# manlito/densepoints

Measured on AMD Instinct MI355X. Metric: Mpatches/sec (NCC eval+refine), higher is better.
Workload: dtype u8 texels, fp64 geometry, int32 moments; 1 GPU; cfg3_32view_4k: 32 views 3840x2160, 262144 expansion candidates/GPU/step (65536 refined seed parents x 4 directions), n=11, Nelder-Mead + InitRelatedImages + NCC filter (parity mode); views=32, width=3840, height=2160, cell=11, batch_per_gpu=262144, parallelism=dp1 (candidate shards, no data-path collective)

## Files before the change

### densepoints_amd/_native.py

```python
from __future__ import annotations

import ctypes
import os

import numpy as np

_HERE = os.path.dirname(os.path.abspath(__file__))
LIB_PATH = os.path.join(_HERE, "lib", os.environ.get("DP_LIB_VARIANT") or "libdensepoints.so")

PATCH_DTYPE = np.dtype(
    [
        ("pos", "<f4", 3),
        ("normal", "<f4", 3),
        ("ref", "<u4"),
        ("seq", "<u4"),
        ("vis", "<u8", 2),
        ("cand", "<u8", 2),
        ("score", "<f4"),
        ("evals", "<u4"),
        ("rgb", "u1", 3),
        ("flags", "u1"),
        ("parent", "<u4"),
    ],
    align=True,
)
assert PATCH_DTYPE.itemsize == 80

DP_OK = 0
DP_E_ARG = -1
DP_E_HIP = -2
DP_E_OOM = -3
DP_E_DEGENERATE = -4
DP_E_STATE = -5
DP_E_NODEVICE = -6

MODE_EVAL, MODE_FILTER, MODE_NM, MODE_SEED, MODE_EXPAND = range(5)
MODE_FAST_EVAL, MODE_FAST_REFINE = 5, 6
PATCH_ACCEPTED = 1
PATCH_DEGENERATE = 2


class DpOptions(ctypes.Structure):
    _fields_ = [
        ("seed_cell_size", ctypes.c_int32),
        ("expand_cell_size", ctypes.c_int32),
        ("grid_scale", ctypes.c_int32),
        ("max_patches_per_cell", ctypes.c_int32),
        ("min_visible", ctypes.c_int32),
        ("min_expand_visible", ctypes.c_int32),
        ("nm_max_evals", ctypes.c_int32),
        ("reserved0", ctypes.c_int32),
        ("ncc_threshold", ctypes.c_double),
        ("visible_angle", ctypes.c_double),
        ("candidate_angle", ctypes.c_double),
        ("nm_step", ctypes.c_double * 3),
        ("nm_eps", ctypes.c_double),
        ("ncc_denom_min", ctypes.c_double),
        ("max_pops", ctypes.c_int64),
    ]


class DpImage(ctypes.Structure):
    _fields_ = [
        ("width", ctypes.c_int32),
        ("height", ctypes.c_int32),
        ("stride", ctypes.c_int32),
        ("reserved", ctypes.c_int32),
        ("bgr", ctypes.c_void_p),
    ]


class DpDensifyStats(ctypes.Structure):
    _fields_ = [
        ("seeds_in", ctypes.c_int64),
        ("seed_patches", ctypes.c_int64),
        ("patches", ctypes.c_int64),
        ("pops", ctypes.c_int64),
        ("candidates", ctypes.c_int64),
        ("evals", ctypes.c_int64),
        ("generations", ctypes.c_int32),
        ("stalls", ctypes.c_int32),
        ("refine_ms", ctypes.c_double),
        ("total_ms", ctypes.c_double),
    ]


class DpGeneration(ctypes.Structure):
    _fields_ = [
        ("items", ctypes.c_int64),
        ("head", ctypes.c_int64),
        ("per_item", ctypes.c_int32),
        ("cell", ctypes.c_int32),
        ("seq0", ctypes.c_uint32),
        ("index", ctypes.c_int32),
    ]


class DpIterateStats(ctypes.Structure):
    _fields_ = [
        ("offered", ctypes.c_int64),
        ("reinserted", ctypes.c_int64),
        ("patches", ctypes.c_int64),
        ("filtered_out", ctypes.c_int64),
        ("candidates", ctypes.c_int64),
        ("evals", ctypes.c_int64),
        ("generations", ctypes.c_int32),
        ("reserved", ctypes.c_int32),
        ("refine_ms", ctypes.c_double),
        ("filter_ms", ctypes.c_double),
        ("total_ms", ctypes.c_double),
    ]


class DpFilterOptions(ctypes.Structure):
    _fields_ = [
        ("passes", ctypes.c_int32),
        ("reserved", ctypes.c_int32),
        ("min_neighbor_frac", ctypes.c_double),
    ]


FILTER_VISIBILITY, FILTER_NEIGHBORS = 1, 2


class DpRenderOptions(ctypes.Structure):
    _fields_ = [
        ("splat_scale", ctypes.c_float),
        ("max_radius_px", ctypes.c_int32),
        ("flags", ctypes.c_int32),
    ]


class DpRenderStats(ctypes.Structure):
    _fields_ = [
        ("patches", ctypes.c_int64),
        ("pairs", ctypes.c_int64),
        ("pixel_tests", ctypes.c_int64),
        ("covered_pixels", ctypes.c_int64),
        ("render_ms", ctypes.c_double),
    ]


RENDER_ALL_FACING = 1


class DpFuseOptions(ctypes.Structure):
    _fields_ = [
        ("depth_tol", ctypes.c_float),
        ("min_views", ctypes.c_int32),
        ("min_normal_cos", ctypes.c_float),
        ("flags", ctypes.c_int32),
    ]


class DpFuseStats(ctypes.Structure):
    _fields_ = [
        ("depth_pixels", ctypes.c_int64),
        ("matched_pairs", ctypes.c_int64),
        ("consistent_pairs", ctypes.c_int64),
        ("fusable", ctypes.c_int64),
        ("emitted", ctypes.c_int64),
        ("fuse_ms", ctypes.c_double),
    ]


FUSE_NO_SUPPRESS = 1

FUSED_DTYPE = np.dtype(
    [
        ("pos", "<f4", 3),
        ("normal", "<f4", 3),
        ("rgb", "u1", 3),
        ("n_views", "u1"),
        ("view", "<i4"),
        ("x", "<i4"),
        ("y", "<i4"),
    ],
    align=True,
)
assert FUSED_DTYPE.itemsize == 40


class DpMaprefOptions(ctypes.Structure):
    _fields_ = [
        ("window", ctypes.c_int32),
        ("sweep", ctypes.c_int32),
        ("step_px", ctypes.c_float),
        ("reach", ctypes.c_int32 * 2),
        ("max_sources", ctypes.c_int32),
# ... 158 lines not shown


class DpSynthConfig(ctypes.Structure):
    _fields_ = [
        ("n_views", ctypes.c_int32),
        ("width", ctypes.c_int32),
        ("height", ctypes.c_int32),
        ("kind", ctypes.c_int32),
        ("seed", ctypes.c_uint64),
        ("spread_deg", ctypes.c_double),
        ("seed_stride_px", ctypes.c_double),
        ("depth_noise", ctypes.c_double),
    ]


class DpMatcherOptions(ctypes.Structure):

    _fields_ = [
        ("n_features", ctypes.c_int32),
        ("n_levels", ctypes.c_int32),
        ("scale_factor", ctypes.c_double),
        ("edge_threshold", ctypes.c_int32),
        ("fast_threshold", ctypes.c_int32),
        ("cell_size", ctypes.c_int32),
        ("max_keypoints_per_cell", ctypes.c_int32),
        ("epipolar_matching", ctypes.c_int32),
        ("max_epipolar_distance", ctypes.c_float),
        ("nn_match_ratio", ctypes.c_float),
        ("matcher_type", ctypes.c_int32),
        ("detector_type", ctypes.c_int32),
        ("akaze_threshold", ctypes.c_float),
    ]


class DpSeedStats(ctypes.Structure):
    _fields_ = [
        ("keypoints_detected", ctypes.c_int64),
        ("keypoints", ctypes.c_int64),
        ("pairs", ctypes.c_int64),
        ("ratio_matches", ctypes.c_int64),
        ("matches", ctypes.c_int64),
        ("points", ctypes.c_int64),
        ("detect_ms", ctypes.c_double),
        ("describe_ms", ctypes.c_double),
        ("match_ms", ctypes.c_double),
        ("triangulate_ms", ctypes.c_double),
        ("total_ms", ctypes.c_double),
    ]


class DpFastOptions(ctypes.Structure):
    _fields_ = [
        ("iters", ctypes.c_int32),
        ("margin", ctypes.c_int32),
        ("tile_budget", ctypes.c_int32),
        ("max_views", ctypes.c_int32),
        ("fd_step", ctypes.c_float),
        ("ls_step", ctypes.c_float),
        ("densify", ctypes.c_int32),
        ("gradient", ctypes.c_int32),
        ("filter_max_views", ctypes.c_int32),
    ]


class DpFastStats(ctypes.Structure):
    _fields_ = [("patches", ctypes.c_int64), ("evals", ctypes.c_int64), ("view_evals", ctypes.c_int64),
                ("staged_bytes", ctypes.c_int64), ("clipped_stagings", ctypes.c_int64)]


KEYPOINT_DTYPE = np.dtype(
    [("x", "<f4"), ("y", "<f4"), ("response", "<f4"), ("angle", "<f4"), ("octave", "<i4"), ("reserved", "<i4")]
)

_P = ctypes.c_void_p
_I = ctypes.c_int
_D = ctypes.c_double

SIGNATURES = [
    ("dp_default_options", None, [_P]),
    ("dp_abi_version", _I, []),
    ("dp_device_count", _I, []),
    ("dp_ctx_create", _I, [_P, _I, _P]),
    ("dp_ctx_destroy", _I, [_P]),
    ("dp_last_error", ctypes.c_char_p, [_P]),
    ("dp_set_options", _I, [_P, _P]),
    ("dp_set_views", _I, [_P, _I, _P, _P]),
    ("dp_set_views_device", _I, [_P, _I, _P, _P, _P, _P, _P]),
    ("dp_build_pyramid", _I, [_P, _I]),
    ("dp_set_level", _I, [_P, _I]),
    ("dp_level_info", _I, [_P, _I, _I, _P, _P, _P]),
    ("dp_read_level", _I, [_P, _I, _I, _P]),
    ("dp_view_geometry", _I, [_P, _P, _P, _P, _P]),
    ("dp_seeds_to_patches", _I, [_P, _P, _I, _P]),
    ("dp_eval_batch", _I, [_P, _P, _I, _I, _P]),
    ("dp_refine_batch", _I, [_P, _P, _I, _I, _I, _P]),
    ("dp_refine_batch_device", _I, [_P, _P, _I, _I, _I, _P, _P]),
    ("dp_expand_batch", _I, [_P, _P, _I, _P, _P]),
    ("dp_expand_batch_device", _I, [_P, _P, _I, _P, _P, _P]),
    ("dp_densify", _I, [_P, _P, _I, _P, _P, _P]),
    ("dp_densify_begin", _I, [_P, _P, _I, _P]),
    ("dp_densify_commit", _I, [_P, _P, _P, _P, ctypes.c_int64]),
    ("dp_densify_result", _I, [_P, _P, _P, _P]),
    ("dp_densify_run", _I, [_P, _P, ctypes.c_int32]),
    ("dp_densify_run_until", _I, [_P, _P, ctypes.c_int32, ctypes.c_int64, _P]),
    ("dp_densify_owners", _I, [_P, _P, _I, _I, _P, _P]),
    ("dp_densify_partition_stats", _I, [_P, _P]),
    ("dp_densify_refine_items", _I, [_P, _P, _P, ctypes.c_int64, _P, _P]),
    ("dp_densify_partition_async", _I, [_P, _P, _I, _I, _P, _P, _P]),
    ("dp_densify_refine_share_async", _I, [_P, _P, _P, ctypes.c_int64, _P, ctypes.c_int64, _P]),
    ("dp_densify_commit_gathered_device", _I, [_P, _P, _P, ctypes.c_int64, _I, _P, _P]),
    ("dp_densify_resume", _I, [_P, _P, ctypes.c_int64, _P, _P]),
    ("dp_densify_resume_device", _I, [_P, _P, ctypes.c_int64, _P, _P, _P]),
    ("dp_densify_store_device", _I, [_P, _P, _P]),
    ("dp_densify_iterate", _I, [_P, _P, _I, _I, _P, _P, _P, _P, _P]),
    ("dp_default_filter_options", None, [_P]),
    ("dp_filter_patches", _I, [_P, _P, ctypes.c_int64, _P, _P]),
    ("dp_filter_patches_device", _I, [_P, _P, ctypes.c_int64, _P, _P, _P]),
    ("dp_default_render_options", None, [_P]),
    ("dp_render_maps", _I, [_P, _P, ctypes.c_int64, _P, _P, _I, _P, _P, _P, _P, _P, _P]),
    ("dp_render_maps_device", _I, [_P, _P, ctypes.c_int64, _P, _P, _I, _P, _P, _P, _P, _P, _P, _P]),
    ("dp_default_fuse_options", None, [_P]),
    ("dp_fuse_maps", _I, [_P, _P, _I, _P, _P, _P, _P, _P, _P]),
    ("dp_fuse_maps_device", _I, [_P, _P, _I, _P, _P, _P, _P, ctypes.c_int64, _P, _P, _P]),
    ("dp_default_mapref_options", None, [_P]),
    ("dp_refine_maps", _I, [_P, _P, _I, _P, _P, _P, _P, _P, _P, _P, _P, _P]),
    ("dp_refine_maps_device", _I, [_P, _P, _I, _P, _P, _P, _P, _P, _P, _P, _P, _P, _P]),
    ("dp_default_tsdf_options", None, [_P]),
    ("dp_tsdf_integrate", _I, [_P, _P, _I, _P, _P, _P, _P, _P, _P]),
    ("dp_tsdf_integrate_device", _I, [_P, _P, _I, _P, _P, _P, _P, _P, _P, _P]),
    ("dp_tsdf_mesh", _I, [_P, _P, _P, _P, _P, _P, _P, _P, _P, _P]),
    ("dp_tsdf_mesh_device", _I, [_P, _P, _P, _P, _P, _P, ctypes.c_int64, _P, _P, ctypes.c_int64, _P, _P, _P]),
    ("dp_default_mesh_clean_options", None, [_P]),
    ("dp_mesh_components", _I, [_P, _P, ctypes.c_int64, ctypes.c_int64, _P, _P, _P, _P, _P]),
    ("dp_mesh_components_device", _I, [_P, _P, ctypes.c_int64, ctypes.c_int64, _P, _P, _P, ctypes.c_int64, _P, _P, _P]),
    ("dp_mesh_clean", _I, [_P, _P, _P, ctypes.c_int64, _P, ctypes.c_int64, _P, _P, _P, _P, _P, _P, _P]),
    ("dp_mesh_clean_device", _I, [_P, _P, _P, ctypes.c_int64, _P, ctypes.c_int64, _P, ctypes.c_int64, _P, _P,
                                  ctypes.c_int64, _P, _P, _P, _P, _P]),
    ("dp_default_mesh_smooth_options", None, [_P]),
    ("dp_mesh_adjacency", _I, [_P, _P, ctypes.c_int64, ctypes.c_int64, _P, _P, _P, _P, _P, _P]),
    ("dp_mesh_adjacency_device", _I, [_P, _P, ctypes.c_int64, ctypes.c_int64, _P, _P, _P, ctypes.c_int64, _P, _P, _P,
                                      _P]),
    ("dp_mesh_smooth", _I, [_P, _P, _P, ctypes.c_int64, _P, ctypes.c_int64, _P, _P]),
    ("dp_mesh_smooth_device", _I, [_P, _P, _P, ctypes.c_int64, _P, ctypes.c_int64, _P, _P, _P]),
    ("dp_mesh_normals", _I, [_P, _P, ctypes.c_int64, _P, ctypes.c_int64, _P, _P]),
    ("dp_mesh_normals_device", _I, [_P, _P, ctypes.c_int64, _P, ctypes.c_int64, _P, _P, _P]),
    ("dp_default_mesh_decimate_options", None, [_P]),
    ("dp_mesh_decimate", _I, [_P, _P, _P, ctypes.c_int64, _P, ctypes.c_int64, _P, _P, _P, _P, _P, _P, _P]),
    ("dp_mesh_decimate_device", _I, [_P, _P, _P, ctypes.c_int64, _P, ctypes.c_int64, _P, ctypes.c_int64, _P, _P,
                                     ctypes.c_int64, _P, _P, _P, _P, _P]),
    ("dp_default_mesh_render_options", None, [_P]),
    ("dp_mesh_render", _I, [_P, _P, ctypes.c_int64, _P, ctypes.c_int64, _P, _I, _P, _P, _P, _P, _P]),
    ("dp_mesh_render_device", _I, [_P, _P, ctypes.c_int64, _P, ctypes.c_int64, _P, _I, _P, _P, _P, _P, _P, _P]),
    ("dp_last_kernel_ms", _I, [_P, _P]),
    ("dp_default_matcher_options", None, [_P]),
    ("dp_orb_pattern", _I, [_P]),
    ("dp_generate_seeds", _I, [_P, _P, _P, _P, _P]),
    ("dp_seed_keypoints", _I, [_P, _I, _P, _P, _P]),
    ("dp_seed_matches", _I, [_P, _I, _P, _P, _P, _P]),
    ("dp_knn_match", _I, [_P, _P, ctypes.c_int64, _P, ctypes.c_int64, _P, _P]),
    ("dp_knn_match_wide", _I, [_P, _P, ctypes.c_int64, _P, ctypes.c_int64, _I, _P, _P]),
    ("dp_seed_descriptor_bytes", _I, [_P]),
    ("dp_fundamental_matrix", _I, [_P, _P, _P]),
    ("dp_triangulate", _I, [_P, ctypes.c_int64, _P, _P, _P, _P]),
    ("dp_synth_default", None, [_P]),
    ("dp_synth_cameras", _I, [_P, _P]),
    ("dp_synth_render_host", _I, [_P, _P, _I, _P]),
    ("dp_synth_render_device", _I, [_P, _P, _P, _I, _P, _P]),
    ("dp_synth_seeds", ctypes.c_int64, [_P, _P, _P, ctypes.c_int64]),
    ("dp_synth_surface", _I, [_P, ctypes.c_int64, _P, _P, _P]),
    ("dp_default_fast_options", None, [_P]),
    ("dp_set_fast_options", _I, [_P, _P]),
    ("dp_build_gray", _I, [_P]),
    ("dp_read_gray", _I, [_P, _I, _P]),
    ("dp_fast_expand_batch", _I, [_P, _P, _I, _P, _P]),
    ("dp_fast_expand_batch_device", _I, [_P, _P, _I, _P, _P, _P]),
    ("dp_fast_last_stats", _I, [_P, _P]),
    ("dp_probe_sincos", None, [_D, _P, _P]),
    ("dp_probe_acos", _D, [_D]),
    ("dp_probe_texture", _I, [_P, ctypes.c_int32, ctypes.c_int32, _P, _P, _I, _P]),
    ("dp_probe_ncc", _D, [ctypes.c_int32] * 6 + [_D]),
    ("dp_probe_math_device", _I, [_P, _I, _P]),
    ("dp_probe_texel_device", _I, [_P, _P, _P, _I, _P]),
    ("dp_probe_recip_f32_device", _I, [_P, _I, _P]),
    ("dp_probe_grad_q24_device", _I, [_P, _I, _P]),
    ("dp_probe_lds_unaligned_device", _I, [_P]),
    ("dp_debug_stamps", _I, [_P]),
    ("dp_probe_keep_gather", _I, [_P, _P, ctypes.c_int64, _P, _P, _P]),
    ("dp_probe_akaze_plane", _I, [_P, _I, _I, _I, _P, ctypes.c_int64, _P]),
    ("dp_probe_orb_level", _I, [_P, _I, _I, _I, _D, _P, ctypes.c_int64, _P]),
    ("dp_probe_seed_stages", _I, [_P, _I, _P, _P, _P, _I, _P, _P, _P, _P]),
    ("dp_probe_seed_t2q", _I, [_P, _I, _P, _P]),
]


def _load():
    if not os.path.exists(LIB_PATH):
        raise ImportError(
            f"densepoints_amd: HIP library {LIB_PATH} is missing; build it with "
            "`python -c 'import __graft_entry__ as g; g.build()'` (no CPU fallback exists)"
        )
    lib = ctypes.CDLL(LIB_PATH)
    for name, res, args in SIGNATURES:
        fn = getattr(lib, name)
        fn.restype = res
        fn.argtypes = args
    return lib


lib = _load()


class DensePointsError(RuntimeError):
    def __init__(self, code: int, msg: str):
        super().__init__(f"densepoints error {code}: {msg}")
        self.code = code


def check(rc: int, ctx=None) -> None:
    if rc != DP_OK:
        msg = lib.dp_last_error(ctx).decode() if ctx else ""
        raise DensePointsError(rc, msg)


def ptr(a) -> int | None:
    if a is None:
        return None
    return a.ctypes.data


def default_options() -> DpOptions:
    o = DpOptions()
    lib.dp_default_options(ctypes.byref(o))
    return o
```

### densepoints_amd/csrc/dp_capi.hip

```cpp
#include "dp_ctx.h"

#include <algorithm>
#include <cmath>
#include <cstdlib>
#include <cstring>
#include <new>
#include <string>
#include <vector>



static double det_cols(const double *a, const double *b, const double *c)
{
    return (a[0] * (b[1] * c[2] - b[2] * c[1]) - b[0] * (a[1] * c[2] - a[2] * c[1])) +
           c[0] * (a[1] * b[2] - a[2] * b[1]);
}

extern "C" int dp_view_geometry(const double P[12], double C[3], double K[9], double E[12],
                                double xaxis[3])
{
    double col[4][3];
    for (int c = 0; c < 4; ++c)
        for (int r = 0; r < 3; ++r)
            col[c][r] = P[r * 4 + c];
    const double cx = det_cols(col[1], col[2], col[3]);
    const double cy = -det_cols(col[0], col[2], col[3]);
    const double cz = det_cols(col[0], col[1], col[3]);
    const double cw = -det_cols(col[0], col[1], col[2]);
    if (cw == 0.0 || !std::isfinite(cw))
        return DP_E_ARG;
    const double Cc[3] = {cx / cw, cy / cw, cz / cw};
    const double *m0 = P, *m1 = P + 4, *m2 = P + 8;
    double q2[3], q1[3], q0[3], t[3];
    const double l2 = std::sqrt(dpg::dot3(m2, m2));
    for (int i = 0; i < 3; ++i)
        q2[i] = m2[i] / l2;
    const double p12 = dpg::dot3(m1, q2);
    for (int i = 0; i < 3; ++i)
        t[i] = m1[i] - p12 * q2[i];
    const double l1 = std::sqrt(dpg::dot3(t, t));
    for (int i = 0; i < 3; ++i)
        q1[i] = t[i] / l1;
    const double p02 = dpg::dot3(m0, q2), p01 = dpg::dot3(m0, q1);
    for (int i = 0; i < 3; ++i)
        t[i] = (m0[i] - p02 * q2[i]) - p01 * q1[i];
    const double l0 = std::sqrt(dpg::dot3(t, t));
    for (int i = 0; i < 3; ++i)
        q0[i] = t[i] / l0;
    if (C)
        std::memcpy(C, Cc, sizeof(Cc));
    if (xaxis)
        std::memcpy(xaxis, q0, sizeof(q0));
    if (K) {
        const double k22 = dpg::dot3(m2, q2);
        const double k[9] = {dpg::dot3(m0, q0) / k22, dpg::dot3(m0, q1) / k22, dpg::dot3(m0, q2) / k22,
                             0.0, dpg::dot3(m1, q1) / k22, dpg::dot3(m1, q2) / k22,
                             0.0, 0.0, 1.0};
        std::memcpy(K, k, sizeof(k));
    }
    if (E) {
        const double *R[3] = {q0, q1, q2};
        for (int r = 0; r < 3; ++r) {
            for (int c = 0; c < 3; ++c)
                E[r * 4 + c] = R[r][c];
            E[r * 4 + 3] = -dpg::dot3(R[r], Cc);
        }
    }
    return DP_OK;
}

int view_from_P(const double *P, int W, int H, int gs, dpg::ViewDev &v)
{
    std::memset(&v, 0, sizeof(v));
    std::memcpy(v.P, P, sizeof(v.P));
    double xa[3];
    int rc = dp_view_geometry(P, v.C, nullptr, nullptr, xa);
    if (rc != DP_OK)
        return rc;
    const double nx = std::sqrt(dpg::dot3(xa, xa));
    for (int i = 0; i < 3; ++i)
        v.xr[i] = xa[i] / nx;
    v.W = W;
    v.H = H;
    v.pitch = W;
    v.gw = W / gs;
    v.gh = H / gs;
    return DP_OK;
}


extern "C" void dp_default_options(dp_options *o)
{
    std::memset(o, 0, sizeof(*o));
    o->seed_cell_size = 16;
    o->expand_cell_size = 11;
    o->grid_scale = 8;
    o->max_patches_per_cell = 1;
    o->min_visible = 3;
    o->min_expand_visible = 2;
    o->nm_max_evals = 500;
    o->ncc_threshold = 0.6;
    o->visible_angle = 0.78;
    o->candidate_angle = 1.04;
    o->nm_step[0] = 0.02;
    o->nm_step[1] = 0.2;
    o->nm_step[2] = 0.2;
    o->nm_eps = 0.0001;
    o->ncc_denom_min = 0.1;
    o->max_pops = 10000000;
}

extern "C" int dp_abi_version(void) { return DP_ABI_VERSION; }

static int check_options(dp_ctx *c, const dp_options &o)
{
    if (o.seed_cell_size < 2 || o.seed_cell_size > DP_MAX_CELL || o.expand_cell_size < 2 ||
        o.expand_cell_size > DP_MAX_CELL)
        return fail(c, DP_E_ARG, "cell sizes must be in [2, 16]");
    if (o.grid_scale <= 0)
        return fail(c, DP_E_ARG, "grid_scale must be > 0");
    if (o.max_patches_per_cell < 1 || o.max_patches_per_cell > 64)
        return fail(c, DP_E_ARG, "max_patches_per_cell must be in [1, 64]");
    if (o.nm_max_evals < 1)
        return fail(c, DP_E_ARG, "nm_max_evals must be >= 1");
    return DP_OK;
}

extern "C" int dp_device_count(void)
{
    int n = 0;
    return hipGetDeviceCount(&n) == hipSuccess ? n : 0;
}

extern "C" int dp_ctx_create(const dp_options *opt, int device, dp_ctx **out)
{
    if (!out)
        return DP_E_ARG;
    *out = nullptr;
    int ndev = 0;
    if (hipGetDeviceCount(&ndev) != hipSuccess || ndev <= 0)
        return DP_E_NODEVICE;
    if (device < 0 || device >= ndev)
        return DP_E_ARG;
    dp_ctx *c = new (std::nothrow) dp_ctx();
    if (!c)
        return DP_E_OOM;
    c->device = device;
    {
        const char *e = getenv("DP_NO_LPT");
        c->lpt_off = e && e[0] == '1';
        const char *g = getenv("DP_GEN_CAP");
        c->gen_cap_test = g ? std::atoll(g) : 0;
    }
    if (opt)
        c->opt = *opt;
    else
        dp_default_options(&c->opt);
    dp_default_fast_options(&c->fopt);
    int rc = check_options(c, c->opt);
    if (rc != DP_OK) {
        delete c;
        return rc;
    }
    if (hipSetDevice(device) != hipSuccess || hipStreamCreateWithFlags(&c->stream, hipStreamNonBlocking) != hipSuccess ||
        c->d_work.reserve(1) != hipSuccess || c->d_evals.reserve(1) != hipSuccess ||
        c->e0.create() != hipSuccess || c->e1.create() != hipSuccess ||
        c->ej.create(hipEventDisableTiming) != hipSuccess || c->mbox.reserve(8) != hipSuccess ||
        hipMemset(c->mbox.p, 0, 8 * sizeof(unsigned long long)) != hipSuccess) {
        dp_ctx_destroy(c);
        return DP_E_HIP;
    }
    *out = c;
    return DP_OK;
}

static void free_pyramid(dp_ctx *c)
{
    for (uint32_t *p : c->pyr_pool)
        hipFree(p);
    c->pyr_pool.clear();
    if (c->planes.size() > 1)
        c->planes.resize(1);
    c->level = 0;
}

static void free_views(dp_ctx *c)
{
    free_pyramid(c);
    c->planes.clear();
    c->P0.clear();
    for (uint32_t *p : c->own_img)
        hipFree(p);
    c->own_img.clear();
    if (c->d_views)
        hipFree(c->d_views);
    c->d_views = nullptr;
    c->hv.clear();
    c->V = 0;
}

extern "C" int dp_ctx_destroy(dp_ctx *c)
{
    if (!c)
        return DP_OK;
    hipSetDevice(c->device);
    if (c->stream)
        hipStreamSynchronize(c->stream);
    free_views(c);
    const hipStream_t stream = c->stream;
    delete c;
    if (stream)
        hipStreamDestroy(stream);
    return DP_OK;
}

extern "C" const char *dp_last_error(const dp_ctx *c) { return c ? c->err.c_str() : "null context"; }

extern "C" int dp_set_options(dp_ctx *c, const dp_options *opt)
{
    if (!c || !opt)
        return DP_E_ARG;
    int rc = check_options(c, *opt);
    if (rc != DP_OK)
        return rc;
    c->opt = *opt;
    for (auto &v : c->hv) {
        v.gw = v.W / opt->grid_scale;
        v.gh = v.H / opt->grid_scale;
    }
    if (c->V) {
        hipSetDevice(c->device);
        DP_HIP(c, hipMemcpy(c->d_views, c->hv.data(), sizeof(dpg::ViewDev) * c->V, hipMemcpyHostToDevice));
    }
    return DP_OK;
}

static int upload_view_table(dp_ctx *c)
{
    int64_t off = 0;
    for (auto &v : c->hv) {
        v.grid_off = off;
        off += (int64_t)v.gw * v.gh;
    }
    c->grid_cells = off;
    uintptr_t lo = UINTPTR_MAX, hi = 0;
    bool fits = true;
    for (auto &v : c->hv) {
        const uintptr_t b = (uintptr_t)v.img;
        lo = b < lo ? b : lo;
        const uintptr_t e = b + (uintptr_t)v.pitch * (uintptr_t)v.H * 4u;
        hi = e > hi ? e : hi;
        fits = fits && (int64_t)v.pitch * 4 < (1 << 24) && v.H < (1 << 24);
    }
    const char *wide = getenv("DP_WIDE_ADDRESSING");
    c->narrow = fits && hi - lo <= 0xFFFFFFF0ull && !(wide && wide[0] == '1');
    c->img_base = (const char *)lo;
    for (auto &v : c->hv)
        v.img_off = c->narrow ? (uint32_t)((uintptr_t)v.img - lo) : 0u;
    DP_HIP(c, hipMalloc(&c->d_views, sizeof(dpg::ViewDev) * c->V));
    DP_HIP(c, hipMemcpy(c->d_views, c->hv.data(), sizeof(dpg::ViewDev) * c->V, hipMemcpyHostToDevice));
    return DP_OK;
}

static void record_level0(dp_ctx *c, const double *P)
{
    c->gray_ready = false;
    c->P0.assign(P, P + 12 * (size_t)c->V);
    c->planes.assign(1, std::vector<dpk::PyrPlane>(c->V));
    for (int v = 0; v < c->V; ++v)
        c->planes[0][v] = dpk::PyrPlane{(uint32_t *)c->hv[v].img, c->hv[v].W, c->hv[v].H, c->hv[v].pitch, 0};
    c->level = 0;
}

extern "C" int dp_set_views(dp_ctx *c, int V, const double *P, const dp_image *images)
{
    if (!c || V <= 0 || V > DP_MAX_VIEWS || !P || !images)
        return fail(c, DP_E_ARG, "dp_set_views: bad arguments (1 <= V <= 128)");
    hipSetDevice(c->device);
    DP_HIP(c, hipStreamSynchronize(c->stream));
    free_views(c);
    c->hv.resize(V);
    size_t total = 0;
    for (int v = 0; v < V; ++v) {
        const dp_image &im = images[v];
        if (im.width <= 0 || im.height <= 0 || !im.bgr)
            return fail(c, DP_E_ARG, "dp_set_views: empty image");
        total += (size_t)im.width * (size_t)im.height;
    }
    uint32_t *pool = nullptr;
    DP_HIP(c, hipMalloc(&pool, total * sizeof(uint32_t)));
    c->own_img.push_back(pool);
    std::vector<uint32_t> tmp;
    size_t at = 0;
    for (int v = 0; v < V; ++v) {
        const dp_image &im = images[v];
        if (view_from_P(P + 12 * v, im.width, im.height, c->opt.grid_scale, c->hv[v]) != DP_OK)
            return fail(c, DP_E_ARG, "dp_set_views: singular projection matrix");
        const size_t stride = im.stride ? (size_t)im.stride : (size_t)im.width * 3;
        tmp.resize((size_t)im.width * im.height);
        parallel_for(im.height, [&](int64_t y) {
            const uint8_t *row = im.bgr + (size_t)y * stride;
            uint32_t *o = tmp.data() + (size_t)y * im.width;
            for (int x = 0; x < im.width; ++x)
                o[x] = (uint32_t)row[3 * x] | ((uint32_t)row[3 * x + 1] << 8) |
                       ((uint32_t)row[3 * x + 2] << 16) | 0xFF000000u;
        });
        uint32_t *d = pool + at;
        at += tmp.size();
        DP_HIP(c, hipMemcpy(d, tmp.data(), tmp.size() * sizeof(uint32_t), hipMemcpyHostToDevice));
        c->hv[v].img = d;
    }
    c->V = V;
    record_level0(c, P);
    return upload_view_table(c);
}

extern "C" int dp_set_views_device(dp_ctx *c, int V, const double *P, const int32_t *W, const int32_t *H,
                                   const int32_t *pitch, const void *const *dev_bgra)
{
    if (!c || V <= 0 || V > DP_MAX_VIEWS || !P || !W || !H || !dev_bgra)
        return fail(c, DP_E_ARG, "dp_set_views_device: bad arguments");
    hipSetDevice(c->device);
    DP_HIP(c, hipStreamSynchronize(c->stream));
    free_views(c);
    c->hv.resize(V);
    for (int v = 0; v < V; ++v) {
        if (W[v] <= 0 || H[v] <= 0 || !dev_bgra[v])
            return fail(c, DP_E_ARG, "dp_set_views_device: empty image");
        if (view_from_P(P + 12 * v, W[v], H[v], c->opt.grid_scale, c->hv[v]) != DP_OK)
            return fail(c, DP_E_ARG, "dp_set_views_device: singular projection matrix");
        c->hv[v].pitch = pitch ? pitch[v] : W[v];
        c->hv[v].img = (const uint32_t *)dev_bgra[v];
    }
    c->V = V;
    record_level0(c, P);
    return upload_view_table(c);
}


extern "C" int dp_build_pyramid(dp_ctx *c, int levels)
{
    if (!c || levels < 1 || levels > DP_MAX_LEVELS)
        return fail(c, DP_E_ARG, "dp_build_pyramid: levels must be in [1, DP_MAX_LEVELS]");
    if (c->V <= 0 || c->planes.empty())
        return fail(c, DP_E_STATE, "dp_build_pyramid: no views set");
    c->gray_ready = false;
    hipSetDevice(c->device);
    DP_HIP(c, hipStreamSynchronize(c->stream));
    if (c->level != 0) {
        int rc = dp_set_level(c, 0);
        if (rc != DP_OK)
            return rc;
    }
    free_pyramid(c);
    const int V = c->V;
    dpk::PyrPlane *d_tab = nullptr;
    DP_HIP(c, hipMalloc(&d_tab, sizeof(dpk::PyrPlane) * 2 * V));
    int rc = DP_OK;
    for (int l = 1; l < levels && rc == DP_OK; ++l) {
        const std::vector<dpk::PyrPlane> &src = c->planes[l - 1];
        std::vector<dpk::PyrPlane> dst(V);
        size_t total = 0;
        int mw = 0, mh = 0;
        for (int v = 0; v < V; ++v) {
            dst[v].w = (src[v].w + 1) / 2;
            dst[v].h = (src[v].h + 1) / 2;
            dst[v].pitch = dst[v].w;
            total += (size_t)dst[v].w * (size_t)dst[v].h;
            mw = std::max(mw, dst[v].w);
            mh = std::max(mh, dst[v].h);
        }
        uint32_t *pool = nullptr;
        if (hipMalloc(&pool, total * sizeof(uint32_t)) != hipSuccess) {
            rc = fail(c, DP_E_OOM, "dp_build_pyramid: out of device memory");
            break;
        }
        c->pyr_pool.push_back(pool);
        size_t at = 0;
        for (int v = 0; v < V; ++v) {
            dst[v].img = pool + at;
            at += (size_t)dst[v].w * (size_t)dst[v].h;
        }
        hipError_t e = hipMemcpyAsync(d_tab, src.data(), sizeof(dpk::PyrPlane) * V, hipMemcpyHostToDevice, c->stream);
        if (e == hipSuccess)
            e = hipMemcpyAsync(d_tab + V, dst.data(), sizeof(dpk::PyrPlane) * V, hipMemcpyHostToDevice, c->stream);
        if (e == hipSuccess)
            e = dpk::launch_pyr_down(d_tab, d_tab + V, V, mw, mh, c->stream);
        if (e == hipSuccess)
            e = hipStreamSynchronize(c->stream);
        if (e != hipSuccess) {
            rc = fail(c, DP_E_HIP, std::string("dp_build_pyramid: ") + hipGetErrorString(e));
            break;
        }
        c->planes.push_back(std::move(dst));
    }
    hipFree(d_tab);
    return rc;
}

extern "C" int dp_set_level(dp_ctx *c, int level)
{
    if (!c)
        return DP_E_ARG;
    if (c->V <= 0 || c->planes.empty())
        return fail(c, DP_E_STATE, "dp_set_level: no views set");
    if (level < 0 || level >= (int)c->planes.size())
        return fail(c, DP_E_ARG, "dp_set_level: level not built (dp_build_pyramid)");
    hipSetDevice(c->device);
    DP_HIP(c, hipStreamSynchronize(c->stream));
    const double s = std::ldexp(1.0, -level);
    std::vector<dpg::ViewDev> hv(c->V);
// ... 46 lines not shown
        bgr_out[3 * i + 1] = (uint8_t)((tmp[i] >> 8) & 255u);
        bgr_out[3 * i + 2] = (uint8_t)((tmp[i] >> 16) & 255u);
    }
    return DP_OK;
}


extern "C" void dp_default_filter_options(dp_filter_options *fo)
{
    if (!fo)
        return;
    fo->passes = DP_FILTER_VISIBILITY | DP_FILTER_NEIGHBORS;
    fo->reserved = 0;
    fo->min_neighbor_frac = 0.25;
}

extern "C" int dp_filter_patches_device(dp_ctx *c, const dp_patch *d_patches, int64_t n, const dp_filter_options *fo,
                                        uint8_t *d_keep, void *stream)
{
    if (!c || n < 0 || (n > 0 && (!d_patches || !d_keep)) || n > 0xFFFFFFFFll)
        return fail(c, DP_E_ARG, "dp_filter_patches: bad arguments");
    if (c->V <= 0)
        return fail(c, DP_E_STATE, "dp_filter_patches: no views set");
    dp_filter_options o;
    dp_default_filter_options(&o);
    if (fo)
        o = *fo;
    if (n == 0)
        return DP_OK;
    hipSetDevice(c->device);
    hipStream_t s = stream ? (hipStream_t)stream : c->stream;
    DP_HIP(c, c->front.reserve((size_t)c->grid_cells + 1));
    DP_HIP(c, c->f_alive.reserve((size_t)n));
    DP_HIP(c, c->f_rho.reserve((size_t)n));
    dpk::FilterArgs a{};
    a.views = c->d_views;
    a.V = c->V;
    a.patches = d_patches;
    a.n = n;
    a.alive = c->f_alive.p;
    a.front = c->front.p;
    a.rho = c->f_rho.p;
    a.grid_scale = (double)c->opt.grid_scale;
    a.min_neighbor_frac = o.min_neighbor_frac;
    const size_t fb = sizeof(unsigned long long) * ((size_t)c->grid_cells + 1);
    DP_HIP(c, hipMemsetAsync(c->f_alive.p, 1, (size_t)n, s));
    DP_HIP(c, dpk::launch_filter_rho(a, s));
    if (o.passes & DP_FILTER_VISIBILITY) {
        DP_HIP(c, hipMemsetAsync(c->front.p, 0xFF, fb, s));
        DP_HIP(c, dpk::launch_filter_front(a, s));
        DP_HIP(c, dpk::launch_filter_visibility(a, d_keep, s));
        DP_HIP(c, hipMemcpyAsync(c->f_alive.p, d_keep, (size_t)n, hipMemcpyDeviceToDevice, s));
    }
    if (o.passes & DP_FILTER_NEIGHBORS) {
        DP_HIP(c, hipMemsetAsync(c->front.p, 0xFF, fb, s));
        DP_HIP(c, dpk::launch_filter_front(a, s));
        DP_HIP(c, dpk::launch_filter_neighbors(a, d_keep, s));
    } else if (!(o.passes & DP_FILTER_VISIBILITY)) {
        DP_HIP(c, hipMemsetAsync(d_keep, 1, (size_t)n, s));
    }
    return DP_OK;
}

extern "C" int dp_filter_patches(dp_ctx *c, const dp_patch *patches, int64_t n, const dp_filter_options *fo,
                                 uint8_t *keep_out)
{
    if (!c || n < 0 || (n > 0 && (!patches || !keep_out)))
        return fail(c, DP_E_ARG, "dp_filter_patches: bad arguments");
    if (n == 0)
        return DP_OK;
    hipSetDevice(c->device);
    DP_HIP(c, c->f_pat.reserve((size_t)n));
    DP_HIP(c, c->f_keep.reserve((size_t)n));
    DP_HIP(c, hipMemcpyAsync(c->f_pat.p, patches, sizeof(dp_patch) * (size_t)n, hipMemcpyHostToDevice, c->stream));
    const int rc = dp_filter_patches_device(c, c->f_pat.p, n, fo, c->f_keep.p, c->stream);
    if (rc != DP_OK)
        return rc;
    DP_HIP(c, hipMemcpyAsync(keep_out, c->f_keep.p, (size_t)n, hipMemcpyDeviceToHost, c->stream));
    DP_HIP(c, hipStreamSynchronize(c->stream));
    return DP_OK;
}


template <typename F>
static int staged_batch(dp_ctx *c, const dp_patch *in, size_t n_in, DevBuf<dp_patch> &up, DevBuf<dp_patch> &res,
                        size_t n_out, dp_patch *out, bool flags, uint8_t *accept_out, F launch)
{
    hipSetDevice(c->device);
    if (in)
        DP_HIP(c, up.reserve(n_in));
    DP_HIP(c, res.reserve(n_out));
    if (flags)
        DP_HIP(c, c->ok.reserve(n_out));
    if (in)
        DP_HIP(c, hipMemcpyAsync(up.p, in, sizeof(dp_patch) * n_in, hipMemcpyHostToDevice, c->stream));
    const int rc = launch();
    if (rc != DP_OK)
        return rc;
    DP_HIP(c, hipMemcpyAsync(out, res.p, sizeof(dp_patch) * n_out, hipMemcpyDeviceToHost, c->stream));
    if (accept_out)
        DP_HIP(c, hipMemcpyAsync(accept_out, c->ok.p, n_out, hipMemcpyDeviceToHost, c->stream));
    DP_HIP(c, hipStreamSynchronize(c->stream));
    return DP_OK;
}


int seeds_device(dp_ctx *c, const double *xyz, int64_t n, dp_patch *d_out, hipStream_t s)
{
    DP_HIP(c, c->seedx.reserve((size_t)(3 * n)));
    DP_HIP(c, hipMemcpyAsync(c->seedx.p, xyz, sizeof(double) * 3 * (size_t)n, hipMemcpyHostToDevice, s));
    DP_HIP(c, dpk::launch_seed_patches(c->d_views, c->V, c->seedx.p, n, c->opt.visible_angle,
                                       c->opt.candidate_angle, d_out, s));
    return DP_OK;
}

extern "C" int dp_seeds_to_patches(dp_ctx *c, const double *xyz, int n, dp_patch *out)
{
    if (!c || n < 0 || (n > 0 && (!xyz || !out)))
        return fail(c, DP_E_ARG, "dp_seeds_to_patches: bad arguments");
    if (!c->V)
        return fail(c, DP_E_STATE, "dp_seeds_to_patches: no views");
    if (n == 0)
        return DP_OK;
    return staged_batch(c, nullptr, 0, c->sconv, c->sconv, (size_t)n, out, false, nullptr,
                        [&] { return seeds_device(c, xyz, n, c->sconv.p, c->stream); });
}


dpk::RefineArgs refine_args(dp_ctx *c, const dpk::RefineJob &job)
{
    const int n = job.n;
    dpk::RefineArgs a{};
    a.views = c->d_views;
    a.V = c->V;
    a.cell = job.cell;
    a.mode = job.mode;
    a.n = n;
    a.opt = c->opt;
    a.patches = job.patches;
    a.accept = job.accept;
    a.work = c->d_work.p;
    a.evals = c->d_evals.p;
    a.parents = job.parents;
    a.parent0 = job.parent0;
    a.max_pops = job.max_pops;
    a.items = job.items;
    a.gen = job.gen;
    a.epi = job.epi;
    a.seq0 = job.seq0;
    a.claim_grid = c->grid.p;
    a.grid_scale = (double)c->opt.grid_scale;
    a.img_base = c->img_base;
    a.narrow = c->narrow ? 1 : 0;
    if (!c->lpt_off && n > 0) {
        if (c->lpt.reserve((size_t)n + 2 * dpk::kLptBuckets) == hipSuccess) {
            a.order = c->lpt.p;
            a.order_scratch = c->lpt.p + n;
        } else {
            (void)hipGetLastError();
        }
    }
    return a;
}

int densify_epi(const dp_ctx *c)
{
    return dpk::kEpiColor | (c->opt.max_patches_per_cell == 1 ? dpk::kEpiClaims : 0);
}

int launch_job(dp_ctx *c, const dpk::RefineJob &job, hipStream_t s)
{
    if (job.mode >= DP_MODE_FAST_EVAL)
        return dp_fast_launch(c, job, s);
    const dpk::RefineArgs a = refine_args(c, job);
    if (!job.parity_untimed)
        DP_HIP(c, hipEventRecord(c->e0, s));
    DP_HIP(c, dpk::launch_refine(a, s));
    if (!job.parity_untimed) {
        DP_HIP(c, hipEventRecord(c->e1, s));
        c->timed = true;
    }
    return DP_OK;
}

int check_refine(dp_ctx *c, int n, int cell, int mode)
{
    if (!c)
        return DP_E_ARG;
    if (!c->V)
        return fail(c, DP_E_STATE, "no views set");
    if (n < 0 || cell < 2 || cell > DP_MAX_CELL || mode < DP_MODE_EVAL || mode > DP_MODE_FAST_REFINE)
        return fail(c, DP_E_ARG, "refine: bad n/cell/mode");
    return DP_OK;
}

extern "C" int dp_refine_batch_device(dp_ctx *c, dp_patch *d_inout, int n, int cell, int mode,
                                      uint8_t *d_accept, void *stream)
{
    int rc = check_refine(c, n, cell, mode);
    if (rc != DP_OK)
        return rc;
    if (n == 0)
        return DP_OK;
    hipSetDevice(c->device);
    return launch_job(c, dpk::RefineJob{d_inout, d_accept, n, cell, mode}, stream ? (hipStream_t)stream : c->stream);
}

extern "C" int dp_refine_batch(dp_ctx *c, dp_patch *inout, int n, int cell, int mode, uint8_t *accept_out)
{
    int rc = check_refine(c, n, cell, mode);
    if (rc != DP_OK)
        return rc;
    if (n == 0)
        return DP_OK;
    if (!inout)
        return fail(c, DP_E_ARG, "refine: null patches");
    for (int i = 0; i < n; ++i) {
        const dp_patch &p = inout[i];
        const bool bad_hi = c->V <= 64 ? (p.vis[1] != 0 || (c->V < 64 && (p.vis[0] >> c->V))) : (c->V < 128 && (p.vis[1] >> (c->V - 64)));
        if (p.ref >= (uint32_t)c->V || bad_hi)
            return fail(c, DP_E_ARG, "refine: patch " + std::to_string(i) + " names a view outside the scene");
    }
    return staged_batch(c, inout, (size_t)n, c->pat, c->pat, (size_t)n, inout, true, accept_out, [&] {
        return dp_refine_batch_device(c, c->pat.p, n, cell, mode, c->ok.p, c->stream);
    });
}

static int expand_device(dp_ctx *c, const dp_patch *d_parents, int n, dp_patch *d_children, uint8_t *d_accept,
                         void *stream, int mode)
{
    hipSetDevice(c->device);
    dpk::RefineJob job{d_children, d_accept, 4 * n, c->opt.expand_cell_size, mode};
    job.parents = d_parents;
    return launch_job(c, job, stream ? (hipStream_t)stream : c->stream);
}

extern "C" int dp_expand_batch_device(dp_ctx *c, const dp_patch *d_parents, int n, dp_patch *d_children,
                                      uint8_t *d_accept, void *stream)
{
    int rc = check_refine(c, n, c ? c->opt.expand_cell_size : 11, DP_MODE_EXPAND);
    if (rc != DP_OK)
        return rc;
    if (n == 0)
        return DP_OK;
    if ((int64_t)n * 4 > INT32_MAX || !d_parents || !d_children)
        return fail(c, DP_E_ARG, "expand: bad arguments");
    return expand_device(c, d_parents, n, d_children, d_accept, stream, DP_MODE_EXPAND);
}

extern "C" int dp_expand_batch(dp_ctx *c, const dp_patch *parents, int n, dp_patch *children, uint8_t *accept_out)
{
    int rc = check_refine(c, n, c ? c->opt.expand_cell_size : 11, DP_MODE_EXPAND);
    if (rc != DP_OK)
        return rc;
    if (n == 0)
        return DP_OK;
    if (!parents || !children)
        return fail(c, DP_E_ARG, "expand: null arrays");
    return staged_batch(c, parents, (size_t)n, c->cand, c->pat, (size_t)4 * n, children, true, accept_out,
                        [&] { return dp_expand_batch_device(c, c->cand.p, n, c->pat.p, c->ok.p, c->stream); });
}

extern "C" int dp_fast_expand_batch_device(dp_ctx *c, const dp_patch *d_parents, int n, dp_patch *d_children,
                                           uint8_t *d_accept, void *stream)
{
    if (!c)
        return DP_E_ARG;
    if (!c->V)
        return fail(c, DP_E_STATE, "no views set");
    const int cell = c->opt.expand_cell_size;
    if (n < 0 || cell < 2 || cell > DP_MAX_CELL)
        return fail(c, DP_E_ARG, "fast expand: bad n/cell");
    if (n == 0)
        return DP_OK;
    if ((int64_t)n * 4 > INT32_MAX || !d_parents || !d_children)
        return fail(c, DP_E_ARG, "fast expand: bad arguments");
    return expand_device(c, d_parents, n, d_children, d_accept, stream, DP_MODE_FAST_REFINE);
}

extern "C" int dp_fast_expand_batch(dp_ctx *c, const dp_patch *parents, int n, dp_patch *children,
                                    uint8_t *accept_out)
{
    if (!c)
        return DP_E_ARG;
    if (n < 0)
        return fail(c, DP_E_ARG, "fast expand: bad n");
    if (n == 0)
        return DP_OK;
    if (!parents || !children)
        return fail(c, DP_E_ARG, "fast expand: null arrays");
    return staged_batch(c, parents, (size_t)n, c->cand, c->pat, (size_t)4 * n, children, true, accept_out,
                        [&] { return dp_fast_expand_batch_device(c, c->cand.p, n, c->pat.p, c->ok.p, c->stream); });
}

extern "C" int dp_eval_batch(dp_ctx *c, const dp_patch *in, int n, int cell, float *score_out)
{
    int rc = check_refine(c, n, cell, DP_MODE_EVAL);
    if (rc != DP_OK)
        return rc;
    if (n == 0)
        return DP_OK;
    if (!in || !score_out)
        return fail(c, DP_E_ARG, "eval: null arrays");
    std::vector<dp_patch> tmp(in, in + n);
    rc = dp_refine_batch(c, tmp.data(), n, cell, DP_MODE_EVAL, nullptr);
    if (rc != DP_OK)
        return rc;
    for (int i = 0; i < n; ++i)
        score_out[i] = tmp[i].score;
    return DP_OK;
}

extern "C" int dp_last_kernel_ms(dp_ctx *c, double *ms)
{
    if (!c || !ms)
        return DP_E_ARG;
    if (!c->timed)
        return fail(c, DP_E_STATE, "no kernel timed yet");
    DP_HIP(c, hipEventSynchronize(c->e1));
    float f = 0.f;
    DP_HIP(c, hipEventElapsedTime(&f, c->e0, c->e1));
    *ms = f;
    return DP_OK;
}
```

### densepoints_amd/csrc/dp_ctx.h

```cpp
#pragma once

#include "dp_buf.h"
#include "dp_internal.h"

#include <chrono>
#include <cmath>
#include <memory>
#include <string>
#include <thread>
#include <vector>

struct dp_seedgen;
void dp_seedgen_free(dp_seedgen *s);

namespace dpk {

template <typename F> inline void parallel_for(int64_t n, F f)
{
    unsigned hw = std::thread::hardware_concurrency();
    int64_t nt = hw ? (int64_t)(hw > 32 ? 32 : hw) : 4;
    if (nt > n)
        nt = n;
    if (nt <= 1) {
        for (int64_t i = 0; i < n; ++i)
            f(i);
        return;
    }
    std::vector<std::thread> th;
    for (int64_t t = 0; t < nt; ++t)
        th.emplace_back([=, &f]() {
            for (int64_t i = t; i < n; i += nt)
                f(i);
        });
    for (auto &x : th)
        x.join();
}

}

using dpk::DevBuf;
using dpk::DevMem;
using dpk::Event;
using dpk::HostBuf;
using dpk::parallel_for;

using dpk::StripedCounters;
using dpk::Timer;

namespace dpk {


struct RenderScratch {
    DevBuf<unsigned long long> count;
    DevBuf<RenderPair> pairs;
    DevBuf<RenderSlot> slots;
    DevBuf<int32_t> slot_of;
    DevBuf<unsigned char> out;
    Timer time;
};

struct FuseScratch {
    DevBuf<uint8_t> flag;
    DevBuf<unsigned long long> bcount, boff;
    StripedCounters count;
    DevBuf<FuseView> tab;
    DevBuf<unsigned char> in;
    DevBuf<dp_fused_point> pts;
    HostBuf<dp_fused_point> res;
    Timer time;
};

struct MaprefScratch {
    DevBuf<MaprefView> tab;
    StripedCounters count;
    DevBuf<unsigned char> io;
    Timer time;
};

struct TsdfScratch {
    DevBuf<TsdfView> tab;
    StripedCounters count;
    DevBuf<unsigned long long> bcount, boff;
    DevBuf<unsigned char> in, vol;
    DevBuf<uint32_t> flags, vbase;
    DevBuf<uint8_t> tcount;
    DevBuf<dp_mesh_vertex> verts;
    DevBuf<int32_t> tris;
    HostBuf<dp_mesh_vertex> hverts;
    HostBuf<int32_t> htris;
    Timer time[2];
};

struct CleanScratch {
    DevBuf<int32_t> parent, tcnt, vcnt, cnum, vmap, tmax;
    DevBuf<uint8_t> used, keptc;
    DevBuf<unsigned long long> keys, keys_sorted, bcount, boff;
    StripedCounters count;
    DevBuf<unsigned char> in;
    DevBuf<int32_t> maps, tris;
    DevBuf<dp_mesh_vertex> verts;
    DevBuf<dp_mesh_component> comps;
    HostBuf<int32_t> htris;
    HostBuf<dp_mesh_vertex> hverts;
    HostBuf<dp_mesh_component> hcomps;
    Timer time[3];
};

struct MeshSmoothScratch {
    DevBuf<unsigned long long> keys, keys_sorted, bcount, boff;
    DevBuf<int32_t> hpos, off, maxval;
    DevBuf<uint8_t> vflags;
    StripedCounters count;
    DevBuf<float> pos[2];
    DevBuf<uint32_t> ikeys, ikeys_sorted;
    DevBuf<int32_t> itris, itris_sorted;
    DevBuf<unsigned char> in;
    DevBuf<int32_t> csr;
    DevBuf<dp_mesh_vertex> verts;
    DevBuf<float> normals;
    HostBuf<int32_t> hcsr;
    HostBuf<uint8_t> hflags;
    HostBuf<dp_mesh_vertex> hverts;
    HostBuf<float> hnormals;
    Timer time[2];
};

struct MeshDecimateScratch {
    DevBuf<uint8_t> used, tkeep, surv;
    DevBuf<unsigned long long> vkeys, vkeys_sorted, tkeys, tkeys_sorted, bcount, boff;
    DevBuf<int32_t> vidx, vidx_sorted, cid, cstart, tval[2], cout, maxval;
    DevBuf<uint32_t> pkeys, pkeys_sorted;
    DevBuf<int32_t> ptris, ptris_sorted;
    StripedCounters count;
    DevBuf<unsigned char> in;
    DevBuf<int32_t> maps, tris;
    DevBuf<dp_mesh_vertex> verts;
    HostBuf<int32_t> htris;
    HostBuf<dp_mesh_vertex> hverts;
    Timer time;
};

struct MeshRenderScratch {
    DevBuf<unsigned long long> count;
    DevBuf<MeshRenderPair> pairs;
    DevBuf<MeshRenderSlot> slots;
    DevBuf<unsigned char> in, out;
    Timer time;
};

}

struct SeedgenFree {
    void operator()(dp_seedgen *s) const { dp_seedgen_free(s); }
};

struct dp_ctx {
    int device = 0;
    hipStream_t stream = nullptr;
    dp_options opt{};
    std::string err;
    int V = 0;
    std::vector<dpg::ViewDev> hv;
    dpg::ViewDev *d_views = nullptr;
    std::vector<uint32_t *> own_img;
    const char *img_base = nullptr;
    std::vector<double> P0;
    std::vector<std::vector<dpk::PyrPlane>> planes;
    std::vector<uint32_t *> pyr_pool;
    int level = 0;
    bool narrow = false;
    DevBuf<uint32_t> d_work;
    DevBuf<unsigned long long> d_evals;
    Event e0, e1;
    bool timed = false;
    int64_t grid_cells = 0;
    DevBuf<uint32_t> grid;
    DevBuf<uint32_t> cellmin;
    DevBuf<uint64_t> pend;
    DevBuf<uint8_t> granted;
    DevBuf<uint32_t> lpt;
    bool lpt_off = false;
    int64_t gen_cap_test = 0;
    DevBuf<dp_patch> pat, store, cand;
    DevBuf<uint8_t> ok, acc;
    DevBuf<unsigned char> scan_tmp;
    DevBuf<unsigned long long> front;
    DevBuf<uint8_t> f_alive, f_keep;
    DevBuf<double> f_rho;
    DevBuf<dp_patch> f_pat;
    DevBuf<unsigned long long> pix64;
    dpk::RenderScratch render;
    dpk::FuseScratch fuse;
    dpk::MaprefScratch mapref;
    dpk::TsdfScratch tsdf;
    dpk::CleanScratch clean;
    dpk::MeshSmoothScratch smooth;
    dpk::MeshDecimateScratch decimate;
    dpk::MeshRenderScratch meshrender;
    HostBuf<dp_patch> result;
    DevBuf<unsigned long long> itw;
    std::vector<Event> fev;
    DevBuf<dp_patch> seedp;
    DevBuf<double> seedx;
    DevBuf<dp_patch> sconv;
    DevBuf<int64_t> items;
    DevBuf<uint64_t> tkeys, okeys;
    DevBuf<int64_t> oiota, porder, olo;
    int64_t part_stats[4] = {0, 0, 0, 0};
    bool part_pending = false;
    DevBuf<unsigned long long> mbox;
    DevBuf<dpk::GenDev> gstate;
    DevBuf<uint32_t> bsum;
    int g_slot = 0;
    uint32_t *g_lpt_scratch = nullptr;
    std::vector<Event> gev;
    DevBuf<dp_patch> wcand;
    DevBuf<uint8_t> wok;
    Event ej;
    bool g_time_pending = false;
    int64_t g_np = 0;
    int64_t g_nseeds = 0;
    int64_t g_expected = -1;
    dp_densify_stats g_st{};
    std::chrono::steady_clock::time_point g_t0;
    std::unique_ptr<dp_seedgen, SeedgenFree> seeds;
    dp_fast_options fopt{4, 2, 6656, 8, 0.5f, 1.0f, 0, 0, 32};
    DevMem gray_pool;
    size_t gray_cap = 0;
    DevMem d_gray;
    bool gray_ready = false;
    DevBuf<unsigned long long> d_fstats;
    int gray_level = -1, gray_V = 0;
};

namespace dpk {

struct RefineJob {
    dp_patch *patches = nullptr;
    uint8_t *accept = nullptr;
    int n = 0;
    int cell = 0;
    int mode = 0;
    const dp_patch *parents = nullptr;
    int64_t parent0 = 0;
    const int64_t *items = nullptr;
    int64_t max_pops = INT64_MAX;
    const GenDev *gen = nullptr;
    int epi = 0;
    uint32_t seq0 = 0;
    bool parity_untimed = false;
};

}

int dp_fast_launch(dp_ctx *c, const dpk::RefineJob &job, hipStream_t s);

dpk::RefineArgs refine_args(dp_ctx *c, const dpk::RefineJob &job);
int launch_job(dp_ctx *c, const dpk::RefineJob &job, hipStream_t s);
int check_refine(dp_ctx *c, int n, int cell, int mode);
int seeds_device(dp_ctx *c, const double *xyz, int64_t n, dp_patch *d_out, hipStream_t s);
int densify_epi(const dp_ctx *c);
int view_from_P(const double *P, int W, int H, int gs, dpg::ViewDev &v);

static inline int fail(dp_ctx *c, int code, const std::string &msg)
{
    if (c)
        c->err = msg;
    return code;
}


static inline int check_view_list(dp_ctx *c, const char *who, const int32_t *views, int n_views, int cap)
{
    const std::string w(who);
    if (c->V <= 0)
        return fail(c, DP_E_STATE, w + ": no views set");
    if (!views || n_views < 1 || n_views > c->V || n_views > cap)
        return fail(c, DP_E_ARG,
                    w + (cap < DP_MAX_VIEWS ? ": n_views must be in 1..min(V, " + std::to_string(cap) + ")"
                                            : ": n_views must be in 1..V"));
    uint64_t seen[2] = {0, 0};
    for (int k = 0; k < n_views; ++k) {
        const int32_t v = views[k];
        if (v < 0 || v >= c->V || ((seen[v >> 6] >> (v & 63)) & 1ull))
            return fail(c, DP_E_ARG, w + ": view ids must be unique and < V");
        seen[v >> 6] |= 1ull << (v & 63);
    }
    return DP_OK;
}

static inline bool view_inverse(const dpg::ViewDev &v, dpk::ViewInv &t)
{
    const double *P = v.P;
    const double h[9] = {P[0], P[1], P[2], P[4], P[5], P[6], P[8], P[9], P[10]};
    for (int j = 0; j < 12; ++j)
        t.P[j] = P[j];
    t.det = dpg::adjugate3(h, t.A);
    return t.det != 0.0 && std::isfinite(t.det);
}

static inline size_t view_pixels(const dp_ctx *c, int32_t v) { return (size_t)c->hv[v].W * (size_t)c->hv[v].H; }

struct PlanePacker {
    size_t total = 0;
    size_t add(size_t bytes)
    {
        const size_t off = total;
        total += (bytes + 255) & ~(size_t)255;
        return off;
    }
};

#define DP_HIP(c, expr)                                                                      \
    do {                                                                                      \
        hipError_t _e = (expr);                                                               \
        if (_e != hipSuccess)                                                                 \
            return fail((c), _e == hipErrorOutOfMemory ? DP_E_OOM : DP_E_HIP,                 \
                        std::string(#expr) + ": " + hipGetErrorString(_e));                   \
    } while (0)
```

### densepoints_amd/csrc/dp_internal.h

```cpp
#pragma once

#include "../../include/densepoints.h"
#include "dp_geom.h"
#include "dp_devmath.h"
#include <hip/hip_runtime.h>

namespace dpk {

constexpr int kWave = 64;
constexpr int kWavesPerBlock = 4;
constexpr int kBlock = kWave * kWavesPerBlock;

struct GenDev;


__device__ __forceinline__ bool org_cell(const dpg::ViewDev &v, const float *pos, double gs, int64_t &cell)
{
    double u, w;
    dpg::project(v.P, pos[0], pos[1], pos[2], u, w);
    const int64_t row = dpg::grid_coord(w, gs), col = dpg::grid_coord(u, gs);
    if (col < 0 || col >= v.gw || row < 0 || row >= v.gh)
        return false;
    cell = v.grid_off + row * (int64_t)v.gw + col;
    return true;
}

__device__ __forceinline__ uint32_t wave_color(const dpg::ViewDev *views, int V, const float *pos, int lane)
{
    const float p0 = pos[0], p1 = pos[1], p2 = pos[2];
    uint32_t s0 = 0, s1 = 0, s2 = 0, nin = 0;
    for (int v = lane; v < V; v += 64) {
        const dpg::ViewDev &vw = views[v];
        double u, w;
        dpg::project(vw.P, p0, p1, p2, u, w);
        if (dpg::inside(u, w, vw.W, vw.H)) {
            const uint32_t px = vw.img[(size_t)(int)w * (size_t)vw.pitch + (size_t)(int)u];
            s0 += px & 255u;
            s1 += (px >> 8) & 255u;
            s2 += (px >> 16) & 255u;
            ++nin;
        }
    }
    for (int o = 32; o > 0; o >>= 1) {
        s0 += __shfl_xor(s0, o);
        s1 += __shfl_xor(s1, o);
        s2 += __shfl_xor(s2, o);
        nin += __shfl_xor(nin, o);
    }
    if (!nin)
        return 0u;
    const uint32_t c0 = (uint8_t)((double)s2 / (double)nin), c1 = (uint8_t)((double)s1 / (double)nin),
                   c2 = (uint8_t)((double)s0 / (double)nin);
    return c0 | c1 << 8 | c2 << 16;
}

__device__ __forceinline__ void wave_claims(const dpg::ViewDev *views, const float *pos, uint64_t vis0, uint64_t vis1,
                                            double gs, uint32_t *grid, uint32_t seq, int lane)
{
    int64_t cell;
    if (((vis0 >> lane) & 1ull) && org_cell(views[lane], pos, gs, cell))
        atomicMin(&grid[cell], seq);
    if (((vis1 >> lane) & 1ull) && org_cell(views[64 + lane], pos, gs, cell))
        atomicMin(&grid[cell], seq);
}

constexpr int kEpiColor = 1;
constexpr int kEpiClaims = 2;

[[maybe_unused]] static __device__ __noinline__ uint32_t refine_epilogue(const dpg::ViewDev *views, int V, float p0,
                                                                        float p1, float p2, uint64_t vis0,
                                                                        uint64_t vis1, int epi, double gs,
                                                                        uint32_t *grid, uint32_t seq, int lane)
{
    const float pf[3] = {p0, p1, p2};
    if (epi & kEpiClaims)
        wave_claims(views, pf, vis0, vis1, gs, grid, seq, lane);
    return (epi & kEpiColor) ? wave_color(views, V, pf, lane) : 0u;
}

struct RefineArgs {
    const dpg::ViewDev *views;
    int32_t V;
    int32_t cell;
    int32_t mode;
    int32_t n;
    dp_options opt;
    dp_patch *patches;
    uint8_t *accept;
    uint32_t *work;
    unsigned long long *evals;
    const dp_patch *parents;
    int64_t parent0;
    int64_t max_pops;
    const char *img_base;
    int32_t narrow;
    uint32_t *order;
    uint32_t *order_scratch;
    const int64_t *items;
    const GenDev *gen;
    int32_t epi;
    uint32_t seq0;
    uint32_t *claim_grid;
    double grid_scale;
};
constexpr int kLptBuckets = 129;

struct GenDev {
    int64_t np;
    int64_t head;
    int64_t items;
    int64_t ncand;
    int64_t cand_total;
    int64_t gens;
    int64_t accepted;
    int64_t nseeds;
    int64_t seed_patches;
    uint32_t seq0;
    int32_t per_item;
    int32_t stall;
    int32_t err;
};
static_assert(sizeof(GenDev) % 8 == 0, "GenDev is copied as 64-bit words");

struct BfsArgs {
    const dpg::ViewDev *views;
    int32_t V;
    int32_t k;
    const GenDev *cur;
    GenDev *nxt;
    const dp_patch *cand;
    const uint8_t *ok;
    uint8_t *acc;
    uint32_t *bsum;
    uint32_t *grid;
    double grid_scale;
    uint32_t *cellmin;
    uint64_t *pend;
    uint8_t *granted;
    dp_patch *store;
    int64_t store_cap;
    int64_t cand_cap;
    int64_t max_pops;
    unsigned long long *mbox;
    uint32_t *work;
    uint32_t *lpt_scratch;
    int32_t fused;
    int64_t yield_items;
};
constexpr int kBfsBlocks = 1024;

hipError_t launch_bfs_organize(const BfsArgs &a, hipStream_t s);
hipError_t launch_bfs_set_state(GenDev *dst, const GenDev &v, hipStream_t s);
hipError_t launch_keep_count(const uint8_t *keep, int64_t n, uint32_t *bsum, unsigned long long *total_out,
                             hipStream_t s);
hipError_t launch_keep_gather(const dp_patch *src, const uint8_t *keep, int64_t n, const uint32_t *bsum, dp_patch *dst,
                              int64_t dst_cap, hipStream_t s);
hipError_t launch_compact_slot(const dp_patch *cand, const uint8_t *acc, const int64_t *items, int64_t n, int per,
                               dp_patch *slot, hipStream_t s);
struct ScatterClaims {
    const dpg::ViewDev *views;
    uint32_t *grid;
    double grid_scale;
    const GenDev *gen;
};
hipError_t launch_scatter_slots(const dp_patch *recs, int64_t stride, int world, int64_t nc, dp_patch *cand,
                                uint8_t *ok, unsigned long long *exchanged, const ScatterClaims &sc, hipStream_t s);

struct PyrPlane {
    uint32_t *img;
    int32_t w, h, pitch, pad;
};

struct FilterArgs {
    const dpg::ViewDev *views;
    int32_t V;
    int32_t pad;
    const dp_patch *patches;
    int64_t n;
    const uint8_t *alive;
    unsigned long long *front;
    double *rho;
    double grid_scale;
    double min_neighbor_frac;
};

hipError_t launch_filter_rho(const FilterArgs &a, hipStream_t s);
hipError_t launch_filter_front(const FilterArgs &a, hipStream_t s);
hipError_t launch_filter_visibility(const FilterArgs &a, uint8_t *keep, hipStream_t s);
hipError_t launch_filter_neighbors(const FilterArgs &a, uint8_t *keep, hipStream_t s);


struct ViewInv {
    double P[12];
    double A[9], det;
};

struct RenderSlot {
    int32_t view, W, H, pad;
    int64_t zoff;
    float *depth;
    int32_t *index;
    float *normal;
    float *score;
};
struct RenderPair {
    double A[9], D, s, RR;
    int32_t x0, x1, y0, y1;
    int32_t slot, index;
};
constexpr int kRenderCounters = 4;
struct RenderArgs {
    const dpg::ViewDev *views;
    int32_t V;
    int32_t n_slots;
    const dp_patch *patches;
    const uint8_t *keep;
    const double *rho;
    int64_t n;
    const RenderSlot *slots;
    const int32_t *slot_of;
    uint64_t req[2];
    double splat_scale, max_radius;
    int32_t all_facing, pad;
    RenderPair *pairs;
    int64_t pair_cap;
    unsigned long long *zbuf;
    unsigned long long *count;
};
hipError_t launch_render_pairs(const RenderArgs &a, int64_t i0, int64_t i1, int chunk, hipStream_t s);
hipError_t launch_render_raster(const RenderArgs &a, int chunk, hipStream_t s);
hipError_t launch_render_resolve(const RenderArgs &a, int max_pixels, hipStream_t s);

struct MeshRenderSlot {
    int32_t view, W, H, pad;
    int64_t zoff;
    double m;
    float *depth;
    int32_t *index;
    float *normal;
};
struct MeshRenderPair {
    double r[9], D;
    int64_t first;
    int32_t x0, x1, y0, y1;
    int32_t slot, index;
};

struct FuseView {
    ViewInv inv;
    const float *depth;
    const float *normal;
    const uint32_t *img;
    int64_t poff;
    int32_t W, H, pitch, view;
};
constexpr int kFuseBlock = 256;
constexpr int kFuseCounters = 4;
constexpr int kFuseStripes = 64;
struct FuseArgs {
    const FuseView *tab;
    int32_t K, min_views, no_suppress, has_normals;
    double tol, cos2;
    unsigned long long *mask;
    uint8_t *flag;
    unsigned long long *bcount;
    const unsigned long long *boff;
    unsigned long long *count;
    dp_fused_point *out;
    int64_t cap;
};
hipError_t launch_fuse_mask(const FuseArgs &a, unsigned gx, hipStream_t s);
hipError_t launch_fuse_count(const FuseArgs &a, unsigned gx, hipStream_t s);
hipError_t launch_fuse_emit(const FuseArgs &a, unsigned gx, hipStream_t s);

constexpr int kMaprefMaxSources = 8;
constexpr int kMaprefCounters = 6;
constexpr int kMaprefStripes = 64;
struct MaprefView {
    ViewInv inv;
    double C[3], xr[3];
    const float *depth;
    const float *normal;
    float *odepth;
    float *onormal;
    float *oscore;
    int32_t *ochoice;
    const uint16_t *gray;
    int32_t W, H, gpitch, nsrc;
    int32_t src[kMaprefMaxSources];
};
struct MaprefArgs {
    const MaprefView *tab;
    int32_t K, window, sweep, nreach;
    int32_t reach[2], top_k, keep_unscored;
    double step, min_ncc, dmin;
    unsigned long long *count;
};
hipError_t launch_mapref(const MaprefArgs &a, unsigned gx, hipStream_t s);

struct TsdfView {
    double P[12];
    double g;
    const float *depth;
    const uint32_t *img;
    int32_t W, H, pitch, view;
};
constexpr int kTsdfRows = 4;
constexpr int kTsdfCounters = 4;
constexpr int kTsdfStripes = 64;
constexpr int kMeshBlock = 256;
struct TsdfVolume {
    double origin[3], voxel;
    int32_t nx, ny, nz;
};
struct TsdfArgs {
    const TsdfView *tab;
    int32_t K;
    TsdfVolume vol;
    double trunc;
    float *tsdf;
    int32_t *weight;
    uint32_t *rgb;
    unsigned long long *count;
};
hipError_t launch_tsdf_integrate(const TsdfArgs &a, hipStream_t s);
struct MeshArgs {
    TsdfVolume vol;
    int32_t min_weight;
    int64_t points;
    const float *tsdf;
    const int32_t *weight;
    const uint32_t *rgb;
    uint32_t *flags;
    uint8_t *tcount;
    uint32_t *vbase;
    unsigned long long *bcount;
    const unsigned long long *boff;
    unsigned long long *active;
    int64_t blocks;
    dp_mesh_vertex *verts;
    int32_t *tris;
    int64_t vcap, tcap;
};
hipError_t launch_mesh_count(const MeshArgs &a, hipStream_t s);
hipError_t launch_mesh_vcount(const MeshArgs &a, hipStream_t s);
hipError_t launch_mesh_vertices(const MeshArgs &a, hipStream_t s);
hipError_t launch_mesh_triangles(const MeshArgs &a, hipStream_t s);

hipError_t launch_refine(const RefineArgs &a, hipStream_t s);
hipError_t launch_pyr_down(const PyrPlane *d_src, const PyrPlane *d_dst, int V, int max_dw, int max_dh,
                           hipStream_t s);
int read_stamps(unsigned long long *out);
hipError_t launch_probe_texel(const unsigned long long *ta, const unsigned long long *tb, const uint32_t *fxy, int n,
                              int32_t *gray);
hipError_t launch_render(const dp_synth_config &cfg, const double *P, uint32_t *out, int v,
                         hipStream_t s);
hipError_t launch_seed_patches(const dpg::ViewDev *views, int V, const double *xyz, int64_t n, double vis_angle,
                               double cand_angle, dp_patch *out, hipStream_t s);
hipError_t launch_tile_keys(const dpg::ViewDev *views, const dp_patch *items, int64_t n, double tile, int64_t tx_max,
                            int64_t ty_max, uint64_t *key, int64_t *iota, unsigned long long *stats, hipStream_t s);
hipError_t launch_partition_stats(const uint64_t *key, int64_t n, int world, unsigned long long *stats, hipStream_t s);
hipError_t launch_gather_patches(const dp_patch *src, const int64_t *idx, int64_t n, dp_patch *dst, hipStream_t s);
}
```

### densepoints_amd/csrc/dp_refine.hip

```cpp
#include "dp_internal.h"
#include "dp_wave.h"

namespace dpk {
namespace {

#ifndef DP_TEX_PER_LANE
#define DP_TEX_PER_LANE 4
#endif

#ifndef DP_MAP_CHUNK
#define DP_MAP_CHUNK 24
#endif
constexpr int kMapChunk = DP_MAP_CHUNK;

struct WaveLds {
    double rowt[64][3];
    double colt[64][3];
    dpg::TexMap map[kMapChunk];
    uint64_t roi[kMapChunk];
    int32_t pitch[kMapChunk];
    double score[DP_MAX_VIEWS];
    int32_t mom[kMapChunk][3];
    double c12[12];
    double X[3], n[3];
    double sp[4][3];
    double y[4];
    double cs[3];
    double pt[3];
    double ylo, ynhi, ysave;
    uint64_t vis[2], cand[2];
    int32_t ref, m;
    uint32_t anchor[DP_TEX_PER_LANE * 32];
    uint8_t vlist[DP_MAX_VIEWS];
#ifdef DP_STAMPS
    unsigned long long stamp[8];
#endif
};

#ifdef DP_STAMPS
__device__ unsigned long long g_stamps[8];
#define STAMP_BEGIN unsigned long long _st = __builtin_amdgcn_s_memtime()
#define STAMP(L, cat)                                                    \
    do {                                                                 \
        const unsigned long long _n = __builtin_amdgcn_s_memtime();      \
        (L).stamp[cat] += _n - _st;                                      \
        _st = _n;                                                        \
    } while (0)
#else
#define STAMP_BEGIN
#define STAMP(L, cat)
#endif

__device__ __forceinline__ void decode_vis(WaveLds &L, uint64_t v0, uint64_t v1)
{
    const int lane = lane_id();
    const uint64_t below = (1ull << lane) - 1ull;
    const int c0 = __popcll(v0);
    if ((v0 >> lane) & 1ull)
        L.vlist[__popcll(v0 & below)] = (uint8_t)lane;
    if ((v1 >> lane) & 1ull)
        L.vlist[c0 + __popcll(v1 & below)] = (uint8_t)(64 + lane);
    L.vis[0] = v0;
    L.vis[1] = v1;
    L.m = c0 + __popcll(v1);
    wave_sync();
}

typedef const __attribute__((address_space(1))) uint32_t *gpix_t;
typedef const __attribute__((address_space(1))) unsigned long long *gpair_t;

template <bool kSafe>
__device__ __forceinline__ void texel_coord(const WaveLds &L, int rb, int px, int py, int32_t &ix, int32_t &iy)
{
    const double X0 = L.rowt[rb + py][0], Y0 = L.rowt[rb + py][1], W0 = L.rowt[rb + py][2];
    const double cX = L.colt[rb + px][0], cY = L.colt[rb + px][1], cW = L.colt[rb + px][2];
    double W = W0 + cW;
    if (kSafe)
        W = recip_safe(W);
    else
        W = (W != 0.0) ? 1.0 / W : 0.0;
    double X = (X0 + cX) * W;
    double Y = (Y0 + cY) * W;
    if (!kSafe) {
        X = X < 2147483647.0 ? X : 2147483647.0;
        X = X > -2147483648.0 ? X : -2147483648.0;
        Y = Y < 2147483647.0 ? Y : 2147483647.0;
        Y = Y > -2147483648.0 ? Y : -2147483648.0;
    }
    ix = rint_i32(X);
    iy = rint_i32(Y);
}

struct TexelLoad {
    unsigned long long a, b;
    uint32_t fx, fy;
};

__device__ __forceinline__ int32_t med3_i32(int32_t v, int32_t lo, int32_t hi)
{
    int32_t r;
    asm("v_med3_i32 %0, %1, %2, %3" : "=v"(r) : "v"(v), "v"(lo), "v"(hi));
    return r;
}

__device__ __forceinline__ TexelLoad texel_fetch(gpix_t roi, int pitch, int wm32, int hm32, int32_t ix, int32_t iy)
{
    const int32_t cx = med3_i32(ix, 0, wm32), cy = med3_i32(iy, 0, hm32);
    const uint32_t o0 = __umul24((uint32_t)cy >> 5, (uint32_t)pitch) + ((uint32_t)cx >> 5);
    TexelLoad t;
    t.a = *(gpair_t)(roi + o0);
    t.b = *(gpair_t)(roi + o0 + pitch);
    t.fx = (uint32_t)cx & 31u;
    t.fy = (uint32_t)cy & 31u;
    return t;
}

typedef const __attribute__((address_space(1))) char *gbyte_t;

template <bool kUniPitch>
__device__ __forceinline__ TexelLoad texel_fetch_n(gbyte_t base, gbyte_t base1, uint32_t roi, int pitch4, int wm32,
                                                   int hm32, int32_t ix, int32_t iy)
{
    const int32_t cx = med3_i32(ix, 0, wm32), cy = med3_i32(iy, 0, hm32);
    uint32_t xo, o0;
    asm("v_lshl_add_u32 %0, %1, 2, %2" : "=v"(xo) : "v"((uint32_t)cx >> 5), "v"(roi));
    asm("v_mad_u32_u24 %0, %1, %2, %3" : "=v"(o0) : "v"((uint32_t)cy >> 5), "v"(pitch4), "v"(xo));
    TexelLoad t;
    t.a = *(gpair_t)(base + o0);
    if (kUniPitch)
        t.b = *(gpair_t)(base1 + o0);
    else
        t.b = *(gpair_t)(base + (o0 + (uint32_t)pitch4));
    t.fx = (uint32_t)cx & 31u;
    t.fy = (uint32_t)cy & 31u;
    return t;
}

__device__ __forceinline__ uint32_t pk_mul_u16_sat(uint32_t a, uint32_t b)
{
    uint32_t r;
    asm("v_pk_mad_u16 %0, %1, %2, 0 op_sel_hi:[1,0,0] clamp" : "=v"(r) : "v"(a), "v"(b));
    return r;
}

__device__ __forceinline__ uint32_t pk_mul_u16(uint32_t a, uint32_t b)
{
    uint32_t r;
    asm("v_pk_mul_lo_u16 %0, %1, %2 op_sel_hi:[1,0]" : "=v"(r) : "v"(a), "v"(b));
    return r;
}

__device__ __forceinline__ uint32_t mad_hi16(uint32_t a, uint32_t b, uint32_t c)
{
    uint32_t r;
    asm("v_mad_u32_u16 %0, %1, %2, %3 op_sel:[1,0,0,0]" : "=v"(r) : "v"(a), "s"(b), "v"(c));
    return r;
}

__device__ __forceinline__ uint32_t texel_gray_hi(const TexelLoad &t)
{
    typedef unsigned short us2 __attribute__((ext_vector_type(2)));
    const uint32_t a0 = (uint32_t)t.a, b0 = (uint32_t)t.b;
    const uint32_t a1 = (uint32_t)(t.a >> 32), b1 = (uint32_t)(t.b >> 32);
    const uint32_t wx64 = 2048u + t.fx * 4194240u;
    const us2 w0 = __builtin_bit_cast(us2, pk_mul_u16_sat(wx64, 32u - t.fy));
    const us2 w1 = __builtin_bit_cast(us2, pk_mul_u16(wx64, t.fy));
    uint32_t ch[3];
#pragma unroll
    for (int k = 0; k < 3; ++k) {
        const uint32_t sel = 0x0c000c00u | (uint32_t)k | ((uint32_t)(4 + k) << 16);
        const us2 p0 = __builtin_bit_cast(us2, __builtin_amdgcn_perm(a1, a0, sel));
        const us2 p1 = __builtin_bit_cast(us2, __builtin_amdgcn_perm(b1, b0, sel));
        ch[k] = __builtin_amdgcn_udot2(p0, w0, __builtin_amdgcn_udot2(p1, w1, 32768u, false), false);
    }
    return mad_hi16(ch[0], 7472u, mad_hi16(ch[1], 38468u, mad_hi16(ch[2], 19596u, 32768u)));
}

__device__ __forceinline__ int texel_gray(const TexelLoad &t) { return (int)(texel_gray_hi(t) >> 16); }

__device__ __forceinline__ void fill_tables(WaveLds &L, int rb, const dpg::TexMap &tm, int r)
{
    typedef __attribute__((address_space(3))) double *lds_f64w_t;
    const double m0 = tm.m0, m1 = tm.m1, m2 = tm.m2, m3 = tm.m3, m4 = tm.m4, m5 = tm.m5;
    const double m6 = tm.m6, m7 = tm.m7, m8 = tm.m8;
    const double v = (double)r;
    const double r0 = m1 * v + m2, r1 = m4 * v + m5, r2 = m7 * v + m8;
    const double c0 = m0 * v, c1 = m3 * v, c2 = m6 * v;
    const uint32_t off = __umul24((uint32_t)(rb + r), (uint32_t)sizeof(double[3]));
    const lds_f64w_t R = (lds_f64w_t)(uintptr_t)((uint32_t)(uintptr_t)(__attribute__((address_space(3))) char *)&L.rowt[0][0] + off);
    const lds_f64w_t C = (lds_f64w_t)(uintptr_t)((uint32_t)(uintptr_t)(__attribute__((address_space(3))) char *)&L.colt[0][0] + off);
    R[0] = r0;
    R[1] = r1;
    R[2] = r2;
    C[0] = c0;
    C[1] = c1;
    C[2] = c2;
}

__device__ __forceinline__ int pick8(int j, uint64_t q)
{
    return (int)(int8_t)(uint8_t)(q >> (8 * j));
}

template <int G>
__device__ __forceinline__ int group_total(int v)
{
    constexpr int LP = kWave / G;
    static_assert(LP >= 8, "groups of at least 8 lanes");
    v += __builtin_amdgcn_update_dpp(0, v, 0x111, 0xf, 0xf, false);
    v += __builtin_amdgcn_update_dpp(0, v, 0x112, 0xf, 0xf, false);
    v += __builtin_amdgcn_update_dpp(0, v, 0x114, 0xf, 0xe, false);
    if (LP >= 16)
        v += __builtin_amdgcn_update_dpp(0, v, 0x118, 0xf, 0xc, false);
    if (LP >= 32)
        v += __builtin_amdgcn_update_dpp(0, v, 0x142, 0xa, 0xf, false);
    if (LP == 64)
        v += __builtin_amdgcn_update_dpp(0, v, 0x143, 0xc, 0xf, false);
    return v;
}

template <int G>
__device__ __forceinline__ void group_total3(int &a, int &b, int &c)
{
    constexpr int LP = kWave / G;
    if (LP < 32) {
        a = group_total<G>(a);
        b = group_total<G>(b);
        c = group_total<G>(c);
        return;
    }
    a = group_total<4>(a);
    b = group_total<4>(b);
    c = group_total<4>(c);
    asm volatile("s_nop 1\n\t"
                 "v_add_u32_dpp %0, %0, %0 row_bcast:15 row_mask:0xa bank_mask:0xf\n\t"
                 "v_add_u32_dpp %1, %1, %1 row_bcast:15 row_mask:0xa bank_mask:0xf\n\t"
                 "v_add_u32_dpp %2, %2, %2 row_bcast:15 row_mask:0xa bank_mask:0xf"
                 : "+v"(a), "+v"(b), "+v"(c));
    if (LP == 64)
        asm volatile("s_nop 1\n\t"
                     "v_add_u32_dpp %0, %0, %0 row_bcast:31 row_mask:0xc bank_mask:0xf\n\t"
                     "v_add_u32_dpp %1, %1, %1 row_bcast:31 row_mask:0xc bank_mask:0xf\n\t"
                     "v_add_u32_dpp %2, %2, %2 row_bcast:31 row_mask:0xc bank_mask:0xf"
                     : "+v"(a), "+v"(b), "+v"(c));
}

constexpr int kTexPerLane = DP_TEX_PER_LANE;

__host__ __device__ constexpr int pass_width(int cell)
{
    return cell * cell <= 8 * kTexPerLane    ? 8
           : cell * cell <= 16 * kTexPerLane ? 4
           : cell * cell <= 32 * kTexPerLane ? 2
           : cell * cell <= 64 * kTexPerLane ? 1
                                             : 0;
}

static_assert(kTexPerLane % 2 == 0, "texels are packed in u16 pairs");

template <int G>
struct TexDescT {
    uint32_t ra[kTexPerLane], ca[kTexPerLane];
    uint32_t sel[kTexPerLane / 2];
    uint32_t anc;
    __device__ __forceinline__ uint32_t row(int i) const { return ra[i]; }
    __device__ __forceinline__ uint32_t col(int i) const { return ca[i]; }
};

constexpr int kWideLP = 16;
template <>
struct TexDescT<2> {
    uint32_t rc[2 * kTexPerLane];
    uint32_t sel[kTexPerLane];
    uint32_t anc;
    __device__ __forceinline__ uint32_t row(int i) const { return rc[i] & 0xffffu; }
    __device__ __forceinline__ uint32_t col(int i) const { return rc[i] >> 16; }
};

template <int G>
__device__ __forceinline__ TexDescT<G> make_texdesc(const WaveLds &L, int cell)
{
    const int lane = lane_id();
    const int N = cell * cell;
    const uint32_t rb = lds_addr(&L.rowt[0][0]), cb = lds_addr(&L.colt[0][0]);
    TexDescT<G> td;
    if constexpr (G == 2) {
        static_assert(sizeof(WaveLds) * kWavesPerBlock <= 65536, "LDS addresses fit 16 bits");
        const int q16 = lane & ~(kWideLP - 1), g = lane & (kWideLP - 1), b = (lane / kWideLP) & 1;
#pragma unroll
        for (int e = 0; e < 2 * kTexPerLane; ++e) {
            const int par = e < kTexPerLane ? b : 1 - b;
            const int tl = g + kWideLP * (par + 2 * (e % kTexPerLane));
            const int t = tl < N ? tl : N - 1;
            const int py = t / cell, px = t - py * cell;
            const uint32_t ra = rb + (uint32_t)(q16 + py) * (uint32_t)sizeof(double[3]);
            const uint32_t ca = cb + (uint32_t)(q16 + px) * (uint32_t)sizeof(double[3]);
            td.rc[e] = ra | (ca << 16);
            asm volatile("" : "+v"(td.rc[e]));
        }
#pragma unroll
        for (int p = 0; p < kTexPerLane; ++p) {
            const int par = p < kTexPerLane / 2 ? b : 1 - b;
            const int i0 = 2 * (p % (kTexPerLane / 2));
            const bool l0 = g + kWideLP * (par + 2 * i0) < N, l1 = g + kWideLP * (par + 2 * (i0 + 1)) < N;
            td.sel[p] = 0x0c000c00u | (l0 ? 0x02u : 0x0cu) | ((l1 ? 0x06u : 0x0cu) << 16);
        }
        td.anc = lds_addr(&L.anchor[lane & 31]);
        asm volatile("" : "+v"(td.anc));
    } else {
        constexpr int LP = kWave / G;
        const int j = lane / LP, g = lane & (LP - 1);
#pragma unroll
        for (int i = 0; i < kTexPerLane; ++i) {
            const int tl = g + LP * i;
            const int t = tl < N ? tl : N - 1;
            const int py = t / cell, px = t - py * cell;
            td.ra[i] = rb + (uint32_t)(j * (64 / G) + py) * (uint32_t)sizeof(double[3]);
            td.ca[i] = cb + (uint32_t)(j * (64 / G) + px) * (uint32_t)sizeof(double[3]);
            asm volatile("" : "+v"(td.ra[i]), "+v"(td.ca[i]));
        }
#pragma unroll
        for (int p = 0; p < kTexPerLane / 2; ++p) {
            const bool l0 = g + LP * (2 * p) < N, l1 = g + LP * (2 * p + 1) < N;
            td.sel[p] = 0x0c000c00u | (l0 ? 0x02u : 0x0cu) | ((l1 ? 0x06u : 0x0cu) << 16);
        }
        td.anc = lds_addr(&L.anchor[g]);
        asm volatile("" : "+v"(td.anc));
    }
    return td;
}

template <int LP>
__device__ __forceinline__ int anchor_slot(int p, int g) { return p * LP + g; }

__device__ __forceinline__ void texel_coord_d(uint32_t ra, uint32_t ca, int32_t &ix, int32_t &iy)
{
    const lds_f64_t R = (lds_f64_t)(uintptr_t)ra;
    const lds_f64_t C = (lds_f64_t)(uintptr_t)ca;
    const double W = recip_safe(R[2] + C[2]);
    ix = rint_i32((R[0] + C[0]) * W);
    iy = rint_i32((R[1] + C[1]) * W);
}

template <int G, bool kAnchor, bool kNarrow, bool kUniPitch>
__device__ __forceinline__ void group_sample_safe(const RefineArgs &a, WaveLds &L, const TexDescT<G> &td, int j,
                                                  uint64_t roi, int pitch, int upitch, int wm32, int hm32, int &s,
                                                  int &ss, int &sx)
{
    typedef unsigned short us2 __attribute__((ext_vector_type(2)));
    TexelLoad tl[kTexPerLane];
    const gbyte_t base1 = (gbyte_t)a.img_base + (uint32_t)(upitch * 4);
#pragma unroll
    for (int i = 0; i < kTexPerLane; ++i) {
        int32_t ix, iy;
        texel_coord_d(td.row(i), td.col(i), ix, iy);
        if (kNarrow)
            tl[i] = texel_fetch_n<kUniPitch>((gbyte_t)a.img_base, base1, (uint32_t)roi, pitch * 4, wm32, hm32, ix, iy);
        else
            tl[i] = texel_fetch((gpix_t)roi, pitch, wm32, hm32, ix, iy);
        __builtin_amdgcn_sched_barrier(0);
    }
    constexpr int LP = kWave / G;
    const int g = lane_id() & (LP - 1);
    const us2 ones = {1, 1};
    uint32_t us = (uint32_t)s, uss = (uint32_t)ss, usx = (uint32_t)sx;
#pragma unroll
    for (int p = 0; p < kTexPerLane / 2; ++p) {
        const uint32_t r0 = texel_gray_hi(tl[2 * p]);
        const uint32_t r1 = texel_gray_hi(tl[2 * p + 1]);
        const uint32_t gg = __builtin_amdgcn_perm(r1, r0, td.sel[p]);
        uint32_t aa;
        const lds_u32_t ap = (lds_u32_t)(uintptr_t)(td.anc + 4u * (uint32_t)(p * LP));
        if (kAnchor) {
            aa = (G == 1) ? gg : (uint32_t)__builtin_amdgcn_ds_bpermute(g << 2, (int)gg);
            if (j == 0)
                *ap = gg;
        } else {
            aa = *ap;
        }
        const us2 vg = __builtin_bit_cast(us2, gg);
        us = __builtin_amdgcn_udot2(vg, ones, us, false);
        uss = __builtin_amdgcn_udot2(vg, vg, uss, false);
        usx = __builtin_amdgcn_udot2(vg, __builtin_bit_cast(us2, aa), usx, false);
    }
    s = (int)us;
    ss = (int)uss;
    sx = (int)usx;
}

__device__ __forceinline__ void group_sample_split(const RefineArgs &a, const TexDescT<2> &td, int j, uint64_t roi,
                                                   int pitch, int upitch, int wm32, int hm32, int &s, int &ss, int &sx)
{
    typedef unsigned short us2 __attribute__((ext_vector_type(2)));
    static_assert(kTexPerLane == 4, "two texel pairs per lane");
    constexpr int LP = kWave / 2;
    const bool hi = j != 0;
    const uint32_t rc0 = hi ? td.rc[2] : td.rc[0], rc1 = hi ? td.rc[3] : td.rc[1];
    const uint32_t ra0 = rc0 & 0xffffu, ca0 = rc0 >> 16, ra1 = rc1 & 0xffffu, ca1 = rc1 >> 16;
    const uint32_t sel = hi ? td.sel[1] : td.sel[0];
    const gbyte_t base1 = (gbyte_t)a.img_base + (uint32_t)(upitch * 4);
    int32_t ix, iy;
    texel_coord_d(ra0, ca0, ix, iy);
    const TexelLoad t0 = texel_fetch_n<true>((gbyte_t)a.img_base, base1, (uint32_t)roi, pitch * 4, wm32, hm32, ix, iy);
    __builtin_amdgcn_sched_barrier(0);
    texel_coord_d(ra1, ca1, ix, iy);
    const TexelLoad t1 = texel_fetch_n<true>((gbyte_t)a.img_base, base1, (uint32_t)roi, pitch * 4, wm32, hm32, ix, iy);
    __builtin_amdgcn_sched_barrier(0);
    const uint32_t gg = __builtin_amdgcn_perm(texel_gray_hi(t1), texel_gray_hi(t0), sel);
    const uint32_t aa = *(lds_u32_t)(uintptr_t)(td.anc + 4u * (uint32_t)LP * (uint32_t)j);
    const us2 vg = __builtin_bit_cast(us2, gg);
    const us2 ones = {1, 1};
    s = (int)__builtin_amdgcn_udot2(vg, ones, 0u, false);
    ss = (int)__builtin_amdgcn_udot2(vg, vg, 0u, false);
    sx = (int)__builtin_amdgcn_udot2(vg, __builtin_bit_cast(us2, aa), 0u, false);
}

struct Moments {
    int s, ss, sx;
};

template <int G, bool kAnchor, bool kWide = false>
__device__ __attribute__((noinline)) Moments group_sample_clamped(WaveLds &L, int cell, int j, bool act, gpix_t roi,
                                                                  int pitch, int wm32, int hm32)
{
    constexpr int LP = kWave / G;
    const int g = lane_id() & (LP - 1);
    const int N = cell * cell;
    const float inv_cell = 1.0f / (float)cell;
    Moments m = {0, 0, 0};
    for (int phase = 0; phase < (kAnchor ? 2 : 1); ++phase) {
        const bool mine = kAnchor ? ((j == 0) == (phase == 0)) && act : act;
        if (mine) {
            for (int i = 0, t = g; t < N; ++i, t += LP) {
                const int py = (int)(((float)t + 0.5f) * inv_cell);
                const int px = t - py * cell;
                int32_t ix, iy;
                texel_coord<false>(L, j * (64 / G), px, py, ix, iy);
                const int gv = texel_gray(texel_fetch(roi, pitch, wm32, hm32, ix, iy));
                m.s += gv;
                m.ss += gv * gv;
                uint16_t *ah = kWide ? (uint16_t *)&L.anchor[anchor_slot<2 * LP>(i >> 2, g + LP * (i & 1))] + ((i >> 1) & 1)
                                     : (uint16_t *)&L.anchor[anchor_slot<LP>(i >> 1, g)] + (i & 1);
                if (kAnchor && j == 0)
                    *ah = (uint16_t)gv;
                else
                    m.sx += (int)*ah * gv;
            }
        }
        if (kAnchor)
            wave_sync();
    }
    return m;
}

__device__ __forceinline__ void pair_moments(uint32_t gg, uint32_t aa, uint32_t &us, uint32_t &uss, uint32_t &usx)
{
    typedef unsigned short us2 __attribute__((ext_vector_type(2)));
    const us2 ones = {1, 1};
    const us2 vg = __builtin_bit_cast(us2, gg);
    us = __builtin_amdgcn_udot2(vg, ones, us, false);
    uss = __builtin_amdgcn_udot2(vg, vg, uss, false);
    usx = __builtin_amdgcn_udot2(vg, __builtin_bit_cast(us2, aa), usx, false);
}

template <bool kAnchor, bool kUniPitch>
__device__ __forceinline__ void group_sample_wide(const RefineArgs &a, const TexDescT<2> &td, int j, uint32_t roi,
                                                  int pitch, int upitch, int wm32, int hm32, int &s, int &ss, int &sx)
{
    static_assert(kTexPerLane == 4, "two texel pairs per batch");
    const gbyte_t base1 = (gbyte_t)a.img_base + (uint32_t)(upitch * 4);
    const int lane = lane_id();
    const bool odd = (lane & kWideLP) != 0;
    const uint32_t anc1 = odd ? td.anc - 4u * kWideLP : td.anc + 4u * kWideLP;
    uint32_t us = 0, uss = 0, usx = 0;
    uint32_t keep[kTexPerLane / 2];
#pragma unroll
    for (int b = 0; b < 2; ++b) {
        TexelLoad tl[kTexPerLane];
#pragma unroll
        for (int i = 0; i < kTexPerLane; ++i) {
            int32_t ix, iy;
            texel_coord_d(td.row(kTexPerLane * b + i), td.col(kTexPerLane * b + i), ix, iy);
            tl[i] = texel_fetch_n<kUniPitch>((gbyte_t)a.img_base, base1, roi, pitch * 4, wm32, hm32, ix, iy);
            __builtin_amdgcn_sched_barrier(0);
        }
#pragma unroll
        for (int p = 0; p < kTexPerLane / 2; ++p) {
            const uint32_t r0 = texel_gray_hi(tl[2 * p]);
            const uint32_t r1 = texel_gray_hi(tl[2 * p + 1]);
            const uint32_t gg = __builtin_amdgcn_perm(r1, r0, td.sel[(kTexPerLane / 2) * b + p]);
            if (kAnchor) {
                if (b == 0) {
                    keep[p] = gg;
                } else {
                    const int src = (lane & (kWideLP - 1)) << 2;
                    const uint32_t x0 = (uint32_t)__builtin_amdgcn_ds_bpermute(src, (int)keep[p]);
                    const uint32_t x1 = (uint32_t)__builtin_amdgcn_ds_bpermute(src, (int)gg);
                    pair_moments(keep[p], odd ? x1 : x0, us, uss, usx);
                    pair_moments(gg, odd ? x0 : x1, us, uss, usx);
                    if (j == 0) {
                        *(lds_u32_t)(uintptr_t)(td.anc + 4u * (uint32_t)(p * 32)) = keep[p];
                        *(lds_u32_t)(uintptr_t)(anc1 + 4u * (uint32_t)(p * 32)) = gg;
                    }
                }
            } else {
                const uint32_t aa = *(lds_u32_t)(uintptr_t)((b ? anc1 : td.anc) + 4u * (uint32_t)(p * 32));
                pair_moments(gg, aa, us, uss, usx);
            }
        }
        __builtin_amdgcn_sched_barrier(0);
    }
    s = (int)us;
    ss = (int)uss;
    sx = (int)usx;
}

template <bool kAnchor>
__device__ __forceinline__ void views_pass_wide(const RefineArgs &a, WaveLds &L, const TexDescT<2> &td, uint64_t q,
                                                int &sa, int &saa)
{
    constexpr int LP = kWideLP;
    const int lane = lane_id();
    const int cell = a.cell;
    const int j = (int)((uint32_t)lane / (uint32_t)LP);
    const int slot = pick8(j, q);
    {
        const int r = lane & (LP - 1);
        if (r < cell)
            fill_tables(L, lane & ~(LP - 1), L.map[slot], r);
    }
    const int wm32 = (L.map[slot].w - 1) * 32, hm32 = (L.map[slot].h - 1) * 32;
    const bool all_safe = __ballot(L.map[slot].safe == 0) == 0ull;
    const int pitch = L.pitch[slot];
    const int upitch = uni(pitch);
    const bool uni_pitch = __ballot(pitch != upitch) == 0ull;
    const uint32_t roi = (uint32_t)L.roi[slot];
    wave_sync();
    int s = 0, ss = 0, sx = 0;
    if (all_safe) {
        if (uni_pitch)
            group_sample_wide<kAnchor, true>(a, td, j, roi, pitch, upitch, wm32, hm32, s, ss, sx);
        else
            group_sample_wide<kAnchor, false>(a, td, j, roi, pitch, upitch, wm32, hm32, s, ss, sx);
    } else {
        const Moments mm = group_sample_clamped<kWave / LP, kAnchor, true>(L, cell, j, true, (gpix_t)(a.img_base + roi),
                                                                         pitch, wm32, hm32);
        s = mm.s;
        ss = mm.ss;
        sx = mm.sx;
    }
    group_total3<kWave / LP>(s, ss, sx);
    if (kAnchor) {
        sa = __builtin_amdgcn_readlane(s, LP - 1);
        saa = __builtin_amdgcn_readlane(ss, LP - 1);
    }
    if ((lane & (LP - 1)) == LP - 1 && !(kAnchor && j == 0)) {
        L.mom[slot][0] = s;
        L.mom[slot][1] = ss;
        L.mom[slot][2] = sx;
    }
    wave_sync();
}

template <int G, bool kAnchor, bool kSplit = false>
__device__ __forceinline__ void views_pass(const RefineArgs &a, WaveLds &L, const TexDescT<G> &td, int base, uint64_t q, int &sa, int &saa)
{
    static_assert(!kSplit || (G == 2 && !kAnchor), "split passes: G = 2, no anchor");
    constexpr int LP = kWave / G;
    const int lane = lane_id();
    const int cell = a.cell;
    static_assert(LP >= kTexPerLane, "cell <= LP");
    const int j = (int)((uint32_t)lane / (uint32_t)LP);
    const int slot = pick8(j, q);
    const bool act = slot >= 0;
    const int sl = act ? slot : pick8(0, q);
    {
        constexpr int FP = G == 2 ? kWideLP : LP;
        const int r = lane & (FP - 1);
        if (act && r < cell)
            fill_tables(L, lane & ~(FP - 1), L.map[slot], r);
    }
    const int wm32 = (L.map[sl].w - 1) * 32, hm32 = (L.map[sl].h - 1) * 32;
    const int safe = L.map[sl].safe;
    const bool all_safe = (__ballot(safe == 0) & __ballot(act)) == 0ull;
    const int pitch = L.pitch[sl];
    const int upitch = uni(pitch);
    const bool uni_pitch = __ballot(pitch != upitch) == 0ull;
    const uint64_t roi = L.roi[sl];
    wave_sync();
    int s = 0, ss = 0, sx = 0;
    if constexpr (kSplit) {
        if (all_safe) {
            group_sample_split(a, td, j, roi, pitch, upitch, wm32, hm32, s, ss, sx);
        } else {
            const gpix_t roip = (gpix_t)(a.img_base + (uint32_t)roi);
            const Moments mm = group_sample_clamped<G, false>(L, a.cell, j, act && j == 0, roip, pitch, wm32, hm32);
            s = mm.s;
            ss = mm.ss;
            sx = mm.sx;
        }
    } else if (all_safe) {
        if (a.narrow && uni_pitch)
            group_sample_safe<G, kAnchor, true, true>(a, L, td, j, roi, pitch, upitch, wm32, hm32, s, ss, sx);
        else if (a.narrow)
            group_sample_safe<G, kAnchor, true, false>(a, L, td, j, roi, pitch, upitch, wm32, hm32, s, ss, sx);
        else
            group_sample_safe<G, kAnchor, false, false>(a, L, td, j, roi, pitch, upitch, wm32, hm32, s, ss, sx);
    } else {
        const gpix_t roip = a.narrow ? (gpix_t)(a.img_base + (uint32_t)roi) : (gpix_t)roi;
        const Moments mm = group_sample_clamped<G, kAnchor>(L, a.cell, j, act, roip, pitch, wm32, hm32);
        s = mm.s;
        ss = mm.ss;
        sx = mm.sx;
    }
    if (kSplit)
        group_total3<1>(s, ss, sx);
    else
        group_total3<G>(s, ss, sx);
    if (kAnchor) {
        sa = __builtin_amdgcn_readlane(s, LP - 1);
        saa = __builtin_amdgcn_readlane(ss, LP - 1);
    }
    if (kSplit ? lane == kWave - 1 : ((lane & (LP - 1)) == LP - 1 && act && !(kAnchor && j == 0))) {
        L.mom[slot][0] = s;
        L.mom[slot][1] = ss;
        L.mom[slot][2] = sx;
    }
    wave_sync();
}

template <int G>
__device__ __forceinline__ void views_all(const RefineArgs &a, WaveLds &L, const TexDescT<G> &td, int base, uint64_t todo, bool anchor, int &sa, int &saa)
{
    bool first = anchor;
    if constexpr (G == 2) {
        while (a.narrow && __popcll(todo) + (first ? 1 : 0) >= 4) {
            uint64_t q = 0;
#pragma unroll
            for (int s = 0; s < 4; ++s) {
                if (s == 0 && first)
                    continue;
                q |= (uint64_t)__builtin_ctzll(todo) << (8 * s);
                todo &= todo - 1;
            }
            if (first)
                views_pass_wide<true>(a, L, td, q, sa, saa);
            else
                views_pass_wide<false>(a, L, td, q, sa, saa);
            first = false;
        }
    }
    while (todo || first) {
        uint64_t q = ~0ull;
        int i = 0;
        if (first) {
            q &= ~0xffull;
            i = 1;
        }
#pragma unroll
        for (int s = 0; s < G; ++s) {
            if (s >= i && todo) {
                const uint64_t b = (uint64_t)__builtin_ctzll(todo);
                todo &= todo - 1;
                q = (q & ~(0xffull << (8 * s))) | (b << (8 * s));
            }
        }
        bool split = false;
        if constexpr (G == 2) {
            if (!first && (q >> 8 & 0xffull) == 0xffull && a.narrow) {
                views_pass<2, false, true>(a, L, td, base, (q & ~0xff00ull) | ((q & 0xffull) << 8), sa, saa);
                split = true;
            }
        }
        if (first)
            views_pass<G, true>(a, L, td, base, q, sa, saa);
        else if (!split)
            views_pass<G, false>(a, L, td, base, q, sa, saa);
        first = false;
    }
}

__device__ __forceinline__ int quad_xor1(int v) { return __builtin_amdgcn_mov_dpp(v, 0xB1, 0xf, 0xf, true); }
__device__ __forceinline__ int quad_xor2(int v) { return __builtin_amdgcn_mov_dpp(v, 0x4E, 0xf, 0xf, true); }
template <int I>
__device__ __forceinline__ float quad_bcast(float v)
{
    return __int_as_float(__builtin_amdgcn_mov_dpp(__float_as_int(v), I * 0x55, 0xf, 0xf, true));
}

struct MapView {
    double P[12];
    int32_t W, H, pitch;
    uint32_t img_off;
    const uint32_t *img;
};

template <int kLanesLog2 = 2>
__device__ __forceinline__ MapView load_map_view(const RefineArgs &a, const WaveLds &L, int base, int m, int round0)
{
    const int slot = round0 + (lane_id() >> kLanesLog2);
    const int kk = base + slot;
    const bool act = slot < kMapChunk && kk < m;
    const dpg::ViewDev &vw = a.views[L.vlist[act ? kk : base]];
    MapView v;
#pragma unroll
    for (int i = 0; i < 12; ++i)
        v.P[i] = vw.P[i];
    v.W = vw.W;
    v.H = vw.H;
    v.pitch = vw.pitch;
    v.img_off = vw.img_off;
    v.img = vw.img;
    return v;
}

__device__ __forceinline__ uint64_t build_maps_quad(const MapView &vw, WaveLds &L, int base, int m, int round0,
                                                    int cell, bool narrow)
{
    const int lane = lane_id();
    const int k = lane >> 2, ci = lane & 3;
    const int slot = round0 + k;
    const int kk = base + slot;
    const bool act = slot < kMapChunk && kk < m;
    double u, w;
    dpg::project(vw.P, L.c12[3 * ci], L.c12[3 * ci + 1], L.c12[3 * ci + 2], u, w);
    const uint64_t insm = __ballot(act) & __ballot(u > 0.0) & __ballot(u < (double)vw.W) & __ballot(w > 0.0) &
                          __ballot(w < (double)vw.H);
    const bool all_in = ((insm >> (lane & ~3)) & 0xFull) == 0xFull;
    int cx = (int)ceil(u), cy = (int)ceil(w), lx = (int)floor(u), ly = (int)floor(w);
    cx = min(cx, quad_xor1(cx));
    cx = min(cx, quad_xor2(cx));
    cy = min(cy, quad_xor1(cy));
    cy = min(cy, quad_xor2(cy));
    lx = max(lx, quad_xor1(lx));
    lx = max(lx, quad_xor2(lx));
    ly = max(ly, quad_xor1(ly));
    ly = max(ly, quad_xor2(ly));
    const int tlx = min(vw.W, cx), tly = min(vw.H, cy), brx = max(0, lx), bry = max(0, ly);
    const float fx = (float)u, fy = (float)w;
    const float fx0 = quad_bcast<0>(fx), fx1 = quad_bcast<1>(fx), fx2 = quad_bcast<2>(fx), fx3 = quad_bcast<3>(fx);
    const float fy0 = quad_bcast<0>(fy), fy1 = quad_bcast<1>(fy), fy2 = quad_bcast<2>(fy), fy3 = quad_bcast<3>(fy);
    bool ok = false;
    const int rw = brx - tlx, rh = bry - tly;
    if (ci == 0 && all_in && rw > 0 && rh > 0) {
        const float ftx = (float)tlx, fty = (float)tly;
        const double x[4] = {(double)(fx0 - ftx), (double)(fx1 - ftx), (double)(fx2 - ftx), (double)(fx3 - ftx)};
        const double y[4] = {(double)(fy0 - fty), (double)(fy1 - fty), (double)(fy2 - fty), (double)(fy3 - fty)};
        dpg::TexMap tm;
        ok = dpg::quad_map(x, y, tlx, tly, rw, rh, cell, tm);
        if (ok) {
            tm.m6 *= 0.03125;
            tm.m7 *= 0.03125;
            tm.m8 *= 0.03125;
            L.map[slot] = tm;
            L.roi[slot] = narrow ? (uint64_t)(vw.img_off + ((uint32_t)tm.tly * (uint32_t)vw.pitch + (uint32_t)tm.tlx) * 4u)
                                 : (uint64_t)(uintptr_t)(vw.img + ((size_t)tm.tly * (size_t)vw.pitch + (size_t)tm.tlx));
            L.pitch[slot] = vw.pitch;
        }
    }
    const uint64_t okq = __ballot(ok);
    uint64_t bits = 0;
    for (int q = 0; q < 16; ++q)
        bits |= ((okq >> (4 * q)) & 1ull) << q;
    return bits << round0;
}

__device__ __forceinline__ uint64_t build_maps_pair(const MapView &vw, WaveLds &L, int base, int m, int round0,
                                                    int cell, bool narrow)
{
    const int lane = lane_id();
    const int k = lane >> 1, h = lane & 1;
    const int slot = round0 + k;
    const int kk = base + slot;
    const bool act = slot < kMapChunk && kk < m;
    double u0, w0, u1, w1;
    dpg::project(vw.P, L.c12[6 * h], L.c12[6 * h + 1], L.c12[6 * h + 2], u0, w0);
    dpg::project(vw.P, L.c12[6 * h + 3], L.c12[6 * h + 4], L.c12[6 * h + 5], u1, w1);
    const double dW = (double)vw.W, dH = (double)vw.H;
    const uint64_t insm = __ballot(act) & __ballot(u0 > 0.0) & __ballot(u0 < dW) & __ballot(w0 > 0.0) &
                          __ballot(w0 < dH) & __ballot(u1 > 0.0) & __ballot(u1 < dW) & __ballot(w1 > 0.0) &
                          __ballot(w1 < dH);
    const bool all_in = ((insm >> (lane & ~1)) & 0x3ull) == 0x3ull;
    int cx = min((int)ceil(u0), (int)ceil(u1)), cy = min((int)ceil(w0), (int)ceil(w1));
    int lx = max((int)floor(u0), (int)floor(u1)), ly = max((int)floor(w0), (int)floor(w1));
    cx = min(cx, quad_xor1(cx));
    cy = min(cy, quad_xor1(cy));
    lx = max(lx, quad_xor1(lx));
    ly = max(ly, quad_xor1(ly));
    const int tlx = min(vw.W, cx), tly = min(vw.H, cy), brx = max(0, lx), bry = max(0, ly);
    const float fx0 = (float)u0, fx1 = (float)u1, fy0 = (float)w0, fy1 = (float)w1;
    const float fx2 = __int_as_float(quad_xor1(__float_as_int(fx0))), fx3 = __int_as_float(quad_xor1(__float_as_int(fx1)));
    const float fy2 = __int_as_float(quad_xor1(__float_as_int(fy0))), fy3 = __int_as_float(quad_xor1(__float_as_int(fy1)));
    bool ok = false;
    const int rw = brx - tlx, rh = bry - tly;
    if (h == 0 && all_in && rw > 0 && rh > 0) {
        const float ftx = (float)tlx, fty = (float)tly;
        const double x[4] = {(double)(fx0 - ftx), (double)(fx1 - ftx), (double)(fx2 - ftx), (double)(fx3 - ftx)};
        const double y[4] = {(double)(fy0 - fty), (double)(fy1 - fty), (double)(fy2 - fty), (double)(fy3 - fty)};
        dpg::TexMap tm;
        ok = dpg::quad_map(x, y, tlx, tly, rw, rh, cell, tm);
        if (ok) {
            tm.m6 *= 0.03125;
            tm.m7 *= 0.03125;
            tm.m8 *= 0.03125;
            L.map[slot] = tm;
            L.roi[slot] = narrow ? (uint64_t)(vw.img_off + ((uint32_t)tm.tly * (uint32_t)vw.pitch + (uint32_t)tm.tlx) * 4u)
                                 : (uint64_t)(uintptr_t)(vw.img + ((size_t)tm.tly * (size_t)vw.pitch + (size_t)tm.tlx));
            L.pitch[slot] = vw.pitch;
        }
    }
    const uint64_t okq = __ballot(ok);
    uint64_t bits = 0;
    for (int q = 0; q < 32; ++q)
        bits |= ((okq >> (2 * q)) & 1ull) << q;
    return bits << round0;
}

__device__ __forceinline__ double wave_ncc_finish(int N, int Sa, int Saa, const WaveLds &L, bool scored,
                                                  double denom_min)
{
    static_assert(kMapChunk < kWave, "lane 63 is not a view lane");
    const int lane = lane_id();
    const bool anc = lane == kWave - 1;
    const int64_t n = N;
    const double dn = (double)n, dn2 = (double)(n * n);
    double sig = 0.0;
    int32_t Sb = 0;
    if (scored || anc) {
        Sb = anc ? Sa : L.mom[lane][0];
        const int32_t Sbb = anc ? Saa : L.mom[lane][1];
        sig = dpg::dvsqrt(dpg::dvdiv((double)(n * (int64_t)Sbb - (int64_t)Sb * Sb), dn2));
    }
    const double sa = readlane_f64(sig, kWave - 1);
    double r = -1.0;
    if (scored) {
        double den = sa * sig;
        den = (denom_min < den) ? den : denom_min;
        const double num = dpg::dvdiv((double)(n * (int64_t)L.mom[lane][2] - (int64_t)Sa * Sb), dn);
        r = dpg::dvdiv(dpg::dvdiv(num, den), dn);
    }
    return r;
}

template <int G>
__device__ __forceinline__ int wave_scores(const RefineArgs &a, WaveLds &L, const TexDescT<G> &td, const double *nn, const double *pp, bool &degen)
{
    const int lane = lane_id();
    STAMP_BEGIN;
    const int m = uni(L.m);
    const int nv = m - 1;
    const int cell = a.cell;
    const int N = cell * cell;
    {
        double c12[12];
        const double Xs[3] = {L.X[0], L.X[1], L.X[2]};
        const dpg::ViewDev &rv = a.views[uni(L.ref)];
        const bool l1 = (lane_id() & 1) != 0;
        double u, w;
        dpg::project(rv.P, l1 ? pp[0] + rv.xr[0] : pp[0], l1 ? pp[1] + rv.xr[1] : pp[1],
                     l1 ? pp[2] + rv.xr[2] : pp[2], u, w);
        const bool ok = dpg::window_corners_sc(rv, Xs, nn, readlane_f64(u, 0), readlane_f64(w, 0),
                                               readlane_f64(u, 1), readlane_f64(w, 1), cell, c12);
        degen = degen || !ok;
        if (!ok) {
            for (int k = lane; k < nv; k += kWave)
                L.score[k] = -1.0;
            wave_sync();
            return nv > 0 ? nv : 0;
        }
        for (int i = 0; i < 12; ++i)
            L.c12[i] = c12[i];
    }
    if (nv <= 0)
        return 0;
    wave_sync();
    int Sa = 0, Saa = 0;
    bool va = false;
    for (int base = 0; base < m; base += kMapChunk) {
        uint64_t okmask = 0;
        if (m - base > 16) {
            static_assert(kMapChunk <= 32, "a pair round covers the chunk");
            okmask = build_maps_pair(load_map_view<1>(a, L, base, m, 0), L, base, m, 0, cell, a.narrow != 0);
        } else {
            okmask = build_maps_quad(load_map_view(a, L, base, m, 0), L, base, m, 0, cell, a.narrow != 0);
        }
        wave_sync();
        STAMP(L, 0);
        if (base == 0)
            va = okmask & 1ull;
        const int kb = base == 0 ? 1 : base;
        const int ke = (base + kMapChunk < m) ? base + kMapChunk : m;
        const uint64_t valid = va ? okmask : 0ull;
        const uint64_t todo = valid & (((ke - base) >= 64 ? ~0ull : ((1ull << (ke - base)) - 1ull)) &
                                       ~((1ull << (kb - base)) - 1ull));
        const bool anc = base == 0 && va;
        views_all<G>(a, L, td, base, todo, anc, Sa, Saa);
        STAMP(L, 1);
        wave_sync();
        STAMP(L, 2);
        const int k = base + lane;
        const bool scored = k >= kb && k < ke && ((valid >> lane) & 1ull);
        const double sc = wave_ncc_finish(N, Sa, Saa, L, scored, DP_KARG(RefineArgs, double, opt.ncc_denom_min));
        if (k >= kb && k < ke)
            L.score[k - 1] = scored ? sc : -1.0;
        wave_sync();
        STAMP(L, 3);
    }
    return nv;
}

template <int G>
__device__ __forceinline__ double wave_objective(const RefineArgs &a, WaveLds &L, const TexDescT<G> &td, double x0, double x1, double x2, bool &degen)
{
    double nn[3], pp[3];
    {
        const double Xs[3] = {L.X[0], L.X[1], L.X[2]};
        const double ns[3] = {L.n[0], L.n[1], L.n[2]};
        double s, co;
        dpm::sincos((lane_id() & 1) ? x2 : x1, s, co);
        const double sa = readlane_f64(s, 0), ca = readlane_f64(co, 0);
        const double sb = readlane_f64(s, 1), cb = readlane_f64(co, 1);
        dpg::unparametrize_sc(a.views[uni(L.ref)].C, Xs, ns, x0, sa, ca, sb, cb, nn, pp);
    }
    const int nv = wave_scores<G>(a, L, td, nn, pp, degen);
    if (nv == 0)
        return 2.0;
    double sum = 0.0;
    for (int k = 0; k < nv; ++k)
        sum = sum + (1.0 - L.score[k]);
    return dpg::dvdiv(sum, (double)nv);
}

enum NmPhase { kInit = 0, kReflect = 1, kExpand = 2, kContract = 3, kShrink = 4 };

__device__ __forceinline__ double nm_uni(double v) { return uni_f64(v); }

__device__ __forceinline__ double pick_y(const double *yy, int i)
{
    return i == 0 ? yy[0] : (i == 1 ? yy[1] : (i == 2 ? yy[2] : yy[3]));
}

template <int G>
__device__ __forceinline__ int wave_nelder_mead(const RefineArgs &a, WaveLds &L, const TexDescT<G> &td, bool &degen)
{
    const double step[3] = {DP_KARG(RefineArgs, double, opt.nm_step[0]), DP_KARG(RefineArgs, double, opt.nm_step[1]),
                            DP_KARG(RefineArgs, double, opt.nm_step[2])};
    for (int i = 1; i <= 3; ++i) {
        for (int jj = 0; jj < 3; ++jj)
            L.sp[i][jj] = 0.0;
        L.sp[i][i - 1] += 0.5 * step[i - 1];
    }
    for (int jj = 0; jj < 3; ++jj)
        L.sp[0][jj] = 0.0 - 0.5 * step[jj];

    int fcount = 4, evals = 0, phase = kInit, vi = 0;
    int ilo = 0, ihi = 0, inhi = 0;
    for (;;) {
        double q0, q1, q2;
        if (phase == kInit || phase == kShrink) {
            q0 = L.sp[vi][0];
            q1 = L.sp[vi][1];
            q2 = L.sp[vi][2];
        } else {
            const double fac = phase == kReflect ? -1.0 : (phase == kExpand ? 2.0 : 0.5);
            const double alpha = phase == kReflect ? 2.0 / 3.0 : (phase == kExpand ? -1.0 / 3.0 : 0.5 / 3.0);
            const double beta = alpha - fac;
            q0 = L.cs[0] * alpha - L.sp[ihi][0] * beta;
            q1 = L.cs[1] * alpha - L.sp[ihi][1] * beta;
            q2 = L.cs[2] * alpha - L.sp[ihi][2] * beta;
            L.pt[0] = q0;
            L.pt[1] = q1;
            L.pt[2] = q2;
        }
        const double f = nm_uni(wave_objective<G>(a, L, td, q0, q1, q2, degen));
        ++evals;
        bool decide = false;
        if (phase == kInit) {
            L.y[vi] = f;
            if (++vi == 4) {
                for (int jj = 0; jj < 3; ++jj)
                    L.cs[jj] = ((L.sp[0][jj] + L.sp[1][jj]) + L.sp[2][jj]) + L.sp[3][jj];
                decide = true;
            }
        } else if (phase == kShrink) {
            L.y[vi] = f;
            ++vi;
            if (vi == ilo)
                ++vi;
            if (vi <= 3) {
                for (int jj = 0; jj < 3; ++jj)
                    L.sp[vi][jj] = 0.5 * (L.sp[vi][jj] + L.sp[ilo][jj]);
            } else {
                fcount += 3;
                for (int jj = 0; jj < 3; ++jj)
                    L.cs[jj] = ((L.sp[0][jj] + L.sp[1][jj]) + L.sp[2][jj]) + L.sp[3][jj];
                decide = true;
            }
        } else {
            if (f < nm_uni(L.y[ihi])) {
                L.y[ihi] = f;
                for (int jj = 0; jj < 3; ++jj)
                    L.cs[jj] += L.pt[jj] - L.sp[ihi][jj];
                for (int jj = 0; jj < 3; ++jj)
                    L.sp[ihi][jj] = L.pt[jj];
            }
            if (phase == kReflect) {
                if (f <= nm_uni(L.ylo)) {
                    phase = kExpand;
                } else if (f >= nm_uni(L.ynhi)) {
                    L.ysave = L.y[ihi];
                    phase = kContract;
                } else {
                    --fcount;
                    decide = true;
                }
            } else if (phase == kExpand) {
                decide = true;
            } else {
                if (f >= nm_uni(L.ysave)) {
                    vi = (ilo == 0) ? 1 : 0;
                    for (int jj = 0; jj < 3; ++jj)
                        L.sp[vi][jj] = 0.5 * (L.sp[vi][jj] + L.sp[ilo][jj]);
                    phase = kShrink;
                } else {
                    decide = true;
                }
            }
        }
        if (!decide)
            continue;
        ilo = 0;
        const double y0 = nm_uni(L.y[0]), y1 = nm_uni(L.y[1]), y2 = nm_uni(L.y[2]), y3 = nm_uni(L.y[3]);
        const double yy[4] = {y0, y1, y2, y3};
        if (y0 > y1) {
            ihi = 0;
            inhi = 1;
        } else {
            ihi = 1;
            inhi = 0;
        }
#pragma unroll
        for (int i = 0; i <= 3; ++i) {
            const double yv = yy[i];
            if (yv <= pick_y(yy, ilo))
                ilo = i;
            if (yv > pick_y(yy, ihi)) {
                inhi = ihi;
                ihi = i;
            } else if (yv > pick_y(yy, inhi) && i != ihi) {
                inhi = i;
            }
        }
        if (ilo == inhi || ilo == ihi) {
#pragma unroll
            for (int i = 0; i <= 3; ++i) {
                if (yy[i] == pick_y(yy, ilo) && i != ihi && i != inhi) {
                    ilo = i;
                    break;
                }
            }
        }
        const double err = fabs(pick_y(yy, ihi) - pick_y(yy, ilo));
        double range = 0.0;
        for (int jj = 0; jj < 3; ++jj) {
            double mn = nm_uni(L.sp[0][jj]), mx = mn;
            for (int i = 1; i <= 3; ++i) {
                const double v = nm_uni(L.sp[i][jj]);
                mn = (v < mn) ? v : mn;
                mx = (mx < v) ? v : mx;
            }
            const double rr = fabs(mx - mn);
            range = (range < rr) ? rr : range;
        }
        if (range <= DP_KARG(RefineArgs, double, opt.nm_eps) || err <= DP_KARG(RefineArgs, double, opt.nm_eps) ||
            fcount >= DP_KARG(RefineArgs, int32_t, opt.nm_max_evals))
            break;
        fcount += 2;
        L.ylo = L.y[ilo];
        L.ynhi = L.y[inhi];
        phase = kReflect;
    }
    double nn[3], pp[3];
    {
        const double Xs[3] = {L.X[0], L.X[1], L.X[2]};
        const double ns[3] = {L.n[0], L.n[1], L.n[2]};
        dpg::unparametrize(a.views[uni(L.ref)].C, Xs, ns, L.sp[ilo][0], L.sp[ilo][1], L.sp[ilo][2], nn, pp);
    }
    for (int i = 0; i < 3; ++i) {
        L.n[i] = (double)(float)nn[i];
        L.X[i] = (double)(float)pp[i];
    }
    wave_sync();
    return evals;
}

template <int G>
__device__ __forceinline__ bool wave_filter(const RefineArgs &a, WaveLds &L, const TexDescT<G> &td, float &score, bool &degen)
{
    const int lane = lane_id();
    int nv;
    {
        const double nn[3] = {L.n[0], L.n[1], L.n[2]};
        const double pp[3] = {L.X[0], L.X[1], L.X[2]};
        nv = wave_scores<G>(a, L, td, nn, pp, degen);
    }
    if (nv == 0) {
        score = -1.0f;
        return false;
    }
    double sum = 0.0;
    for (int k = 0; k < nv; ++k)
        sum = sum + L.score[k];
    score = (float)(sum / (double)nv);
    const uint64_t v0 = L.vis[0], v1 = L.vis[1];
    const uint64_t below = (1ull << lane) - 1ull;
    const double thr = DP_KARG(RefineArgs, double, opt.ncc_threshold);
    const int c0 = __popcll(v0);
    const bool in0 = (v0 >> lane) & 1ull;
    const int r0 = __popcll(v0 & below);
    const bool drop0 = in0 && r0 < nv && L.score[r0] < thr;
    const bool in1 = (v1 >> lane) & 1ull;
    const int r1 = c0 + __popcll(v1 & below);
    const bool drop1 = in1 && r1 < nv && L.score[r1] < thr;
    const uint64_t n0 = __ballot(in0 && !drop0);
    const uint64_t n1 = __ballot(in1 && !drop1);
    wave_sync();
    decode_vis(L, n0, n1);
    return uni(L.m) >= DP_KARG(RefineArgs, int32_t, opt.min_visible);
}

__device__ void wave_init_related(const RefineArgs &a, WaveLds &L)
{
    const int lane = lane_id();
    const int ref = uni(L.ref);
    const double X[3] = {L.X[0], L.X[1], L.X[2]};
    const double n[3] = {L.n[0], L.n[1], L.n[2]};
    int cls0 = 0, cls1 = 0;
    if (lane < a.V && lane != ref)
        cls0 = dpg::classify_view(a.views[lane], X, n, DP_KARG(RefineArgs, double, opt.visible_angle),
                                  DP_KARG(RefineArgs, double, opt.candidate_angle));
    if (64 + lane < a.V && 64 + lane != ref)
        cls1 = dpg::classify_view(a.views[64 + lane], X, n, DP_KARG(RefineArgs, double, opt.visible_angle),
                                  DP_KARG(RefineArgs, double, opt.candidate_angle));
    const uint64_t v0 = __ballot(cls0 == 1), v1 = __ballot(cls1 == 1);
    const uint64_t c0 = __ballot(cls0 == 2), c1 = __ballot(cls1 == 2);
    wave_sync();
    L.cand[0] = c0;
    L.cand[1] = c1;
    decode_vis(L, v0, v1);
}

__device__ void child_position(const RefineArgs &a, const dp_patch &par, int dir, float *out)
{
    const dpg::ViewDev &rv = a.views[par.ref];
    const double X[3] = {par.pos[0], par.pos[1], par.pos[2]};
    const double nrm[3] = {par.normal[0], par.normal[1], par.normal[2]};
    double yax[3];
    dpg::cross3(nrm, rv.xr, yax);
    double cu, cv, qu, qv;
    dpg::project(rv.P, X[0], X[1], X[2], cu, cv);
    dpg::project(rv.P, X[0] + rv.xr[0], X[1] + rv.xr[1], X[2] + rv.xr[2], qu, qv);
    const double du = qu - cu, dv = qv - cv;
    const double dx = sqrt(du * du + dv * dv);
    const double scale = (double)DP_KARG(RefineArgs, int32_t, opt.grid_scale) / dx;
    for (int i = 0; i < 3; ++i) {
        const double d = dir == 0 ? rv.xr[i] : dir == 1 ? -rv.xr[i] : dir == 2 ? yax[i] : -yax[i];
        out[i] = (float)(X[i] + scale * d);
    }
}

#ifndef DP_REFINE_WAVES_PER_EU
#define DP_REFINE_WAVES_PER_EU 5
#endif
#ifdef DP_REFINE_MAX_VGPR
#define DP_REFINE_BOUNDS                                                                                       \
    __launch_bounds__(kBlock) __attribute__((amdgpu_waves_per_eu(DP_REFINE_WAVES_PER_EU)))                   \
        __attribute__((amdgpu_num_vgpr(DP_REFINE_MAX_VGPR)))
#else
#define DP_REFINE_BOUNDS __launch_bounds__(kBlock) __attribute__((amdgpu_waves_per_eu(DP_REFINE_WAVES_PER_EU)))
#endif

template <int kMode, int G, bool kGen = false>
__global__ DP_REFINE_BOUNDS void refine_kernel(RefineArgs a)
{
    const int n = kGen ? (int)a.gen->ncand : a.n;
    const int64_t parent0 = kGen ? a.gen->head : a.parent0;
    if (kGen && (int64_t)blockIdx.x * kWavesPerBlock >= (int64_t)n)
        return;
    __shared__ WaveLds lds[kWavesPerBlock];
    WaveLds &L = lds[uni((int)(threadIdx.x / kWave))];
    const int lane = lane_id();
    unsigned long long wave_evals = 0;
#ifdef DP_STAMPS
    for (int c = 0; c < 8; ++c)
        L.stamp[c] = 0;
#endif
    const TexDescT<G> td = make_texdesc<G>(L, a.cell);
    const uint32_t gs = a.parents ? 4u : 1u;
    const int npos = a.order ? (int)(((uint32_t)n + gs - 1) / gs * gs) : n;
    for (;;) {
        uint32_t idx = (uint32_t)npos;
        if (lane == 0) {
            const uint32_t t = atomicAdd(a.work, 1u);
            if (t < (uint32_t)npos)
                idx = t;
        }
        idx = (uint32_t)uni((int)idx);
        if (idx >= (uint32_t)npos)
            break;
        if (a.order) {
            idx = (uint32_t)uni((int)(a.order[idx / gs] * gs + idx % gs));
            if (idx >= (uint32_t)n)
                continue;
        }
        dp_patch *out = a.patches + idx;
        bool live = true;
#ifdef DP_STAMPS
        const unsigned long long _t_patch = __builtin_amdgcn_s_memtime();
#endif
        {
            const dp_patch *src = out;
            float cpos[3] = {0.f, 0.f, 0.f};
            int64_t qi = 0;
            if (a.parents) {
                qi = parent0 + (a.items ? a.items[idx >> 2] : (int64_t)(idx >> 2));
                src = a.parents + qi;
                const int pm = __popcll(src->vis[0]) + __popcll(src->vis[1]);
                live = qi < a.max_pops && pm >= a.opt.min_expand_visible && src->ref < (uint32_t)a.V;
                if (live)
                    child_position(a, *src, (int)(idx & 3u), cpos);
            }
            const uint32_t ref = src->ref;
            const uint64_t v0 = src->vis[0], v1 = src->vis[1];
            const uint64_t m0 = a.V >= 64 ? ~0ull : ((1ull << a.V) - 1ull);
            const uint64_t m1 = a.V >= 128 ? ~0ull : (a.V <= 64 ? 0ull : ((1ull << (a.V - 64)) - 1ull));
            const bool bad = ref >= (uint32_t)a.V || (v0 & ~m0) || (v1 & ~m1);
            if (bad)
                live = false;
            if (lane == 0) {
                if (a.parents) {
                    *out = *src;
                    out->evals = 0;
                    out->flags = 0;
                    out->parent = (uint32_t)qi;
                    if (live) {
                        out->pos[0] = cpos[0];
                        out->pos[1] = cpos[1];
                        out->pos[2] = cpos[2];
                    }
                }
            }
            for (int i = 0; i < 3; ++i) {
                L.X[i] = (a.parents && live) ? (double)cpos[i] : (double)src->pos[i];
                L.n[i] = (double)src->normal[i];
            }
            L.ref = bad ? 0 : (int)ref;
            L.cand[0] = src->cand[0];
            L.cand[1] = src->cand[1];
            decode_vis(L, bad ? 0ull : v0, bad ? 0ull : v1);
        }

        bool degen = false, ok = false;
        int evals = 0;
        float score = 0.f;
        bool has_score = false;
        if (live) {
            switch (kMode) {
            case DP_MODE_EVAL: {
                const double nn[3] = {L.n[0], L.n[1], L.n[2]};
                const double pp[3] = {L.X[0], L.X[1], L.X[2]};
                const int nv = wave_scores<G>(a, L, td, nn, pp, degen);
                double sum = 0.0;
                for (int k = 0; k < nv; ++k)
                    sum = sum + L.score[k];
                score = nv ? (float)(sum / (double)nv) : -1.0f;
                has_score = true;
                evals = 1;
                ok = nv > 0;
                break;
            }
            case DP_MODE_FILTER:
                ok = wave_filter<G>(a, L, td, score, degen);
                has_score = true;
                evals = 1;
                break;
            case DP_MODE_NM:
                evals = wave_nelder_mead<G>(a, L, td, degen);
                ok = true;
                break;
            case DP_MODE_SEED:
                ok = wave_filter<G>(a, L, td, score, degen);
                has_score = true;
                evals = 1;
                if (ok)
                    evals += wave_nelder_mead<G>(a, L, td, degen);
                break;
            case DP_MODE_EXPAND:
            default:
                evals = wave_nelder_mead<G>(a, L, td, degen);
                wave_init_related(a, L);
                ok = wave_filter<G>(a, L, td, score, degen);
                has_score = true;
                evals += 1;
                break;
            }
        }
        wave_evals += (unsigned long long)evals;
#ifdef DP_STAMPS
        L.stamp[7] += __builtin_amdgcn_s_memtime() - _t_patch;
        L.stamp[6] += 1;
#endif
        uint32_t rgb = 0;
        const bool epi = ok && live && a.epi != 0;
        if (epi)
            rgb = refine_epilogue(a.views, a.V, (float)L.X[0], (float)L.X[1], (float)L.X[2], L.vis[0], L.vis[1], a.epi,
                                  a.grid_scale, a.claim_grid, (kGen ? a.gen->seq0 : a.seq0) + idx, lane);
        if (lane == 0) {
            if (epi && (a.epi & kEpiColor)) {
                out->rgb[0] = (uint8_t)rgb;
                out->rgb[1] = (uint8_t)(rgb >> 8);
                out->rgb[2] = (uint8_t)(rgb >> 16);
            }
            if (live) {
                for (int i = 0; i < 3; ++i) {
                    out->pos[i] = (float)L.X[i];
                    out->normal[i] = (float)L.n[i];
                }
                out->vis[0] = L.vis[0];
                out->vis[1] = L.vis[1];
                out->cand[0] = L.cand[0];
                out->cand[1] = L.cand[1];
                if (has_score)
                    out->score = score;
                out->evals += (uint32_t)evals;
            }
            out->flags = (uint8_t)((out->flags & ~DP_PATCH_ACCEPTED) | (ok ? DP_PATCH_ACCEPTED : 0u) |
                                   (degen ? DP_PATCH_DEGENERATE : 0u));
            if (a.accept)
                a.accept[idx] = ok ? 1 : 0;
        }
    }
    if (a.evals && lane == 0 && wave_evals)
        atomicAdd(a.evals, wave_evals);
#ifdef DP_STAMPS
    if (lane == 0)
        for (int c = 0; c < 8; ++c)
            atomicAdd(&g_stamps[c], L.stamp[c]);
#endif
}


__global__ void probe_texel_kernel(const unsigned long long *ta, const unsigned long long *tb, const uint32_t *fxy,
                                   int n, int32_t *gray)
{
    const int i = blockIdx.x * blockDim.x + threadIdx.x;
    if (i >= n)
        return;
    TexelLoad t;
    t.a = ta[i];
    t.b = tb[i];
    t.fx = fxy[i] & 31u;
    t.fy = (fxy[i] >> 5) & 31u;
    gray[i] = texel_gray(t);
}

}

hipError_t launch_probe_texel(const unsigned long long *ta, const unsigned long long *tb, const uint32_t *fxy, int n,
                              int32_t *gray)
{
    hipLaunchKernelGGL(probe_texel_kernel, dim3((n + 255) / 256), dim3(256), 0, 0, ta, tb, fxy, n, gray);
    return hipGetLastError();
}

int read_stamps(unsigned long long *out)
{
#ifdef DP_STAMPS
    if (hipMemcpyFromSymbol(out, HIP_SYMBOL(g_stamps), sizeof(unsigned long long) * 8) != hipSuccess)
        return -2;
    unsigned long long z[8] = {0, 0, 0, 0, 0, 0, 0, 0};
    hipMemcpyToSymbol(HIP_SYMBOL(g_stamps), z, sizeof(z));
    return 0;
#else
    (void)out;
    return -5;
#endif
}

__device__ __forceinline__ int lpt_key(const RefineArgs &a, int64_t parent0, int64_t g)
{
    const dp_patch &p = a.parents ? a.parents[parent0 + (a.items ? a.items[g] : g)] : a.patches[g];
    return kLptBuckets - 1 - (__popcll(p.vis[0]) + __popcll(p.vis[1]));
}

__device__ __forceinline__ int lpt_groups(const RefineArgs &a, int ng)
{
    return a.gen ? (int)((a.gen->ncand + 3) / 4) : ng;
}

__global__ void lpt_hist_kernel(RefineArgs a, int ng_host)
{
    __shared__ uint32_t h[kLptBuckets];
    const int ng = lpt_groups(a, ng_host);
    const int64_t parent0 = a.gen ? a.gen->head : a.parent0;
    for (int b = threadIdx.x; b < kLptBuckets; b += blockDim.x)
        h[b] = 0;
    __syncthreads();
    for (int g = blockIdx.x * blockDim.x + threadIdx.x; g < ng; g += gridDim.x * blockDim.x)
        atomicAdd(&h[lpt_key(a, parent0, g)], 1u);
    __syncthreads();
    for (int b = threadIdx.x; b < kLptBuckets; b += blockDim.x)
        if (h[b])
            atomicAdd(a.order_scratch + b, h[b]);
}

__global__ void lpt_scan_kernel(RefineArgs a)
{
    if (threadIdx.x != 0)
        return;
    uint32_t run = 0;
    for (int b = 0; b < kLptBuckets; ++b) {
        a.order_scratch[kLptBuckets + b] = run;
        run += a.order_scratch[b];
    }
}

__global__ void lpt_scatter_kernel(RefineArgs a, int ng_host)
{
    __shared__ uint32_t h[kLptBuckets];
    const int ng = lpt_groups(a, ng_host);
    const int64_t parent0 = a.gen ? a.gen->head : a.parent0;
    for (int t0 = blockIdx.x * blockDim.x; t0 < ng; t0 += gridDim.x * blockDim.x) {
        for (int b = threadIdx.x; b < kLptBuckets; b += blockDim.x)
            h[b] = 0;
        __syncthreads();
        const int g = t0 + threadIdx.x;
        int key = 0;
        uint32_t rank = 0;
        if (g < ng) {
            key = lpt_key(a, parent0, g);
            rank = atomicAdd(&h[key], 1u);
        }
        __syncthreads();
        for (int b = threadIdx.x; b < kLptBuckets; b += blockDim.x)
            if (h[b])
                h[b] = atomicAdd(a.order_scratch + kLptBuckets + b, h[b]);
        __syncthreads();
        if (g < ng)
            a.order[h[key] + rank] = (uint32_t)g;
        __syncthreads();
    }
}

hipError_t launch_refine(const RefineArgs &a, hipStream_t s)
{
    const bool gen = a.gen != nullptr;
    if (!gen && a.n <= 0)
        return hipSuccess;
    if (gen && (a.mode != DP_MODE_EXPAND || !a.parents))
        return hipErrorInvalidValue;
    int dev = 0;
    hipGetDevice(&dev);
    int cus = 256;
    hipDeviceGetAttribute(&cus, hipDeviceAttributeMultiprocessorCount, dev);
    const int64_t want = ((int64_t)a.n + kWavesPerBlock - 1) / kWavesPerBlock;
    const int64_t cap = (int64_t)cus * 8;
    const int grid = gen ? (int)cap : (int)(want < cap ? want : cap);
    hipError_t e = hipSuccess;
    if (!gen && (e = hipMemsetAsync(a.work, 0, sizeof(uint32_t), s)) != hipSuccess)
        return e;
    const int g = pass_width(a.cell);
    if (g <= 0)
        return hipErrorInvalidValue;
    if (a.order) {
        const int ng = a.parents ? (a.n + 3) / 4 : a.n;
        if (!gen && (e = hipMemsetAsync(a.order_scratch, 0, 2 * kLptBuckets * sizeof(uint32_t), s)) != hipSuccess)
            return e;
        const int gb = gen ? cus : (ng + 255) / 256;
        hipLaunchKernelGGL(lpt_hist_kernel, dim3(gb), dim3(256), 0, s, a, ng);
        hipLaunchKernelGGL(lpt_scan_kernel, dim3(1), dim3(64), 0, s, a);
        hipLaunchKernelGGL(lpt_scatter_kernel, dim3(gb), dim3(256), 0, s, a, ng);
    }
    if (gen) {
        switch (g) {
#define DP_LAUNCH_REFINE_GEN(GG)                                                                               \
    case GG:                                                                                                   \
        hipLaunchKernelGGL((refine_kernel<DP_MODE_EXPAND, GG, true>), dim3(grid), dim3(kBlock), 0, s, a);      \
        break;
            DP_LAUNCH_REFINE_GEN(8)
            DP_LAUNCH_REFINE_GEN(4)
            DP_LAUNCH_REFINE_GEN(2)
            DP_LAUNCH_REFINE_GEN(1)
#undef DP_LAUNCH_REFINE_GEN
        default:
            return hipErrorInvalidValue;
        }
        return hipGetLastError();
    }
    switch (a.mode * 16 + g) {
#define DP_LAUNCH_REFINE(M, GG)                                                                               \
    case M * 16 + GG:                                                                                          \
        hipLaunchKernelGGL((refine_kernel<M, GG>), dim3(grid), dim3(kBlock), 0, s, a);                         \
        break;
#define DP_LAUNCH_REFINE_G(M) DP_LAUNCH_REFINE(M, 8) DP_LAUNCH_REFINE(M, 4) DP_LAUNCH_REFINE(M, 2) DP_LAUNCH_REFINE(M, 1)
        DP_LAUNCH_REFINE_G(DP_MODE_EVAL)
        DP_LAUNCH_REFINE_G(DP_MODE_FILTER)
        DP_LAUNCH_REFINE_G(DP_MODE_NM)
        DP_LAUNCH_REFINE_G(DP_MODE_SEED)
        DP_LAUNCH_REFINE_G(DP_MODE_EXPAND)
#undef DP_LAUNCH_REFINE_G
#undef DP_LAUNCH_REFINE
    default:
        return hipErrorInvalidValue;
    }
    return hipGetLastError();
}

}
```

### densepoints_amd/pmvs.py

```python
from __future__ import annotations

import ctypes
import json
import os
from dataclasses import dataclass, field

import numpy as np

from . import _native as N
from ._native import FUSED_DTYPE, PATCH_DTYPE, check, lib, ptr

__all__ = [
    "Options",
    "FastOptions",
    "View",
    "Engine",
    "PMVS",
    "ncc_score",
    "read_scene_json",
    "write_ply",
    "write_pfm",
    "check_fuse_args",
    "check_mapref_args",
    "check_tsdf_args",
# ... 113 lines not shown
    buf = (ctypes.c_char * (n * PATCH_DTYPE.itemsize)).from_address(addr)
    view = np.frombuffer(buf, dtype=PATCH_DTYPE, count=n)
    return view.copy() if copy else view


def visible_list(mask) -> list[int]:
    out = []
    for w in range(2):
        m = int(mask[w])
        for b in range(64):
            if (m >> b) & 1:
                out.append(64 * w + b)
    return out


def mask_from_list(views) -> np.ndarray:
    m = np.zeros(2, dtype=np.uint64)
    for v in views:
        m[v >> 6] |= np.uint64(1) << np.uint64(v & 63)
    return m


class Engine:

    def __init__(self, options: Options | None = None, device: int = 0):
        self.options = options or Options()
        self._ctx = ctypes.c_void_p()
        copt = self.options.to_c()
        rc = lib.dp_ctx_create(ctypes.byref(copt), device, ctypes.byref(self._ctx))
        check(rc)
        self.views: list[View] = []
        self._keep = []
        self._V = 0
        self._level = 0

    @property
    def handle(self):
        return self._ctx

    def close(self):
        if self._ctx:
            lib.dp_ctx_destroy(self._ctx)
            self._ctx = ctypes.c_void_p()

    def __del__(self):
        try:
            self.close()
        except Exception:
            pass

    def __enter__(self):
        return self

    def __exit__(self, *exc):
        self.close()

    def _check(self, rc):
        check(rc, self._ctx)

    def set_options(self, options: Options):
        self.options = options
        copt = options.to_c()
        self._check(lib.dp_set_options(self._ctx, ctypes.byref(copt)))

    def set_views(self, views: list[View]):
        V = len(views)
        P = np.ascontiguousarray(np.stack([v.P for v in views]).reshape(V, 12))
        imgs = (N.DpImage * V)()
        for i, v in enumerate(views):
            im = v.image
            imgs[i].width = im.shape[1]
            imgs[i].height = im.shape[0]
            imgs[i].stride = im.strides[0]
            imgs[i].bgr = im.ctypes.data
        self._check(lib.dp_set_views(self._ctx, V, ptr(P), imgs))
        self.views = list(views)
        self._V, self._level = V, 0

    def set_views_device(self, P: np.ndarray, widths, heights, pitches, dev_ptrs):
        V = len(dev_ptrs)
        P = np.ascontiguousarray(np.asarray(P, dtype=np.float64).reshape(V, 12))
        w = np.asarray(widths, dtype=np.int32)
        h = np.asarray(heights, dtype=np.int32)
        pt = np.asarray(pitches, dtype=np.int32)
        arr = (ctypes.c_void_p * V)(*[int(p) for p in dev_ptrs])
        self._check(lib.dp_set_views_device(self._ctx, V, ptr(P), ptr(w), ptr(h), ptr(pt), arr))
        self._keep = [P, w, h, pt, arr]
        self._V, self._level = V, 0

    def build_pyramid(self, levels: int):
        self._check(lib.dp_build_pyramid(self._ctx, int(levels)))
        self._level = 0

    def set_level(self, level: int):
        self._check(lib.dp_set_level(self._ctx, int(level)))
        self._level = int(level)

    def level_info(self, level: int, view: int):
        w, h, d = ctypes.c_int32(), ctypes.c_int32(), ctypes.c_void_p()
        self._check(lib.dp_level_info(self._ctx, level, view, ctypes.byref(w), ctypes.byref(h), ctypes.byref(d)))
        return w.value, h.value, d.value

    def read_level(self, level: int, view: int) -> np.ndarray:
        w, h, _ = self.level_info(level, view)
        out = np.zeros((h, w, 3), dtype=np.uint8)
        self._check(lib.dp_read_level(self._ctx, level, view, ptr(out)))
        return out

    def filter_patches(self, patches: np.ndarray, passes: int = 3, min_neighbor_frac: float = 0.25) -> np.ndarray:
        patches = np.ascontiguousarray(patches)
        assert patches.dtype == PATCH_DTYPE
        fo = N.DpFilterOptions(passes, 0, min_neighbor_frac)
        keep = np.zeros(len(patches), dtype=np.uint8)
        self._check(lib.dp_filter_patches(self._ctx, ptr(patches), len(patches), ctypes.byref(fo), ptr(keep)))
        return keep

    def seeds_to_patches(self, xyz: np.ndarray) -> np.ndarray:
        xyz = np.ascontiguousarray(xyz, dtype=np.float64).reshape(-1, 3)
        out = empty_patches(len(xyz))
        self._check(lib.dp_seeds_to_patches(self._ctx, ptr(xyz), len(xyz), ptr(out)))
        return out

    def refine(self, patches: np.ndarray, cell: int, mode: int) -> np.ndarray:
        assert patches.dtype == PATCH_DTYPE and patches.flags.c_contiguous
        acc = np.zeros(len(patches), dtype=np.uint8)
        self._check(lib.dp_refine_batch(self._ctx, ptr(patches), len(patches), cell, mode, ptr(acc)))
        return acc

    def refine_device(self, d_patches: int, n: int, cell: int, mode: int, d_accept: int | None,
                      stream: int | None = None):
        self._check(lib.dp_refine_batch_device(self._ctx, ctypes.c_void_p(d_patches), n, cell, mode,
                                               ctypes.c_void_p(d_accept) if d_accept else None,
                                               ctypes.c_void_p(stream) if stream else None))

    def expand(self, parents: np.ndarray):
        parents = np.ascontiguousarray(parents)
        assert parents.dtype == PATCH_DTYPE
        kids = empty_patches(4 * len(parents))
        acc = np.zeros(4 * len(parents), dtype=np.uint8)
        self._check(lib.dp_expand_batch(self._ctx, ptr(parents), len(parents), ptr(kids), ptr(acc)))
        return kids, acc

    def expand_device(self, d_parents: int, n: int, d_children: int, d_accept: int | None,
                      stream: int | None = None):
        self._check(lib.dp_expand_batch_device(self._ctx, ctypes.c_void_p(d_parents), n,
                                               ctypes.c_void_p(d_children),
                                               ctypes.c_void_p(d_accept) if d_accept else None,
                                               ctypes.c_void_p(stream) if stream else None))

    def last_kernel_ms(self) -> float:
        ms = ctypes.c_double()
        self._check(lib.dp_last_kernel_ms(self._ctx, ctypes.byref(ms)))
        return ms.value

    def set_fast_options(self, fo: FastOptions):
        c = fo.to_c()
        self._check(lib.dp_set_fast_options(self._ctx, ctypes.byref(c)))

    def build_gray(self):
        self._check(lib.dp_build_gray(self._ctx))

    def read_gray(self, view: int) -> np.ndarray:
        vw = self.views[view] if self.views else None
        w, h, _ = self.level_info(0, view) if vw is None else (vw.width, vw.height, 0)
        out = np.zeros((h, w), dtype=np.float16)
        self._check(lib.dp_read_gray(self._ctx, view, ptr(out)))
        return out

    def probe_akaze_plane(self, view: int, level: int, which: int) -> np.ndarray:
        wh = np.zeros(2, dtype=np.int32)
        self._check(lib.dp_probe_akaze_plane(self._ctx, view, level, which, None, 0, ptr(wh)))
        out = np.zeros((int(wh[1]), int(wh[0])), dtype=np.float32)
        self._check(lib.dp_probe_akaze_plane(self._ctx, view, level, which, ptr(out), out.size, ptr(wh)))
        return out

    def probe_orb_level(self, view: int, level: int, n_levels: int, scale_factor: float = 1.2) -> np.ndarray:
        wh = np.zeros(2, dtype=np.int32)
        self._check(lib.dp_probe_orb_level(self._ctx, view, level, n_levels, scale_factor, None, 0, ptr(wh)))
        out = np.zeros((int(wh[1]), int(wh[0])), dtype=np.uint8)
        self._check(lib.dp_probe_orb_level(self._ctx, view, level, n_levels, scale_factor, ptr(out), out.size,
                                           ptr(wh)))
        return out

    def fast_refine(self, patches: np.ndarray, cell: int, mode: int = N.MODE_FAST_REFINE) -> np.ndarray:
        return self.refine(patches, cell, mode)

    def fast_expand(self, parents: np.ndarray):
        parents = np.ascontiguousarray(parents)
        assert parents.dtype == PATCH_DTYPE
        kids = empty_patches(4 * len(parents))
        acc = np.zeros(4 * len(parents), dtype=np.uint8)
        self._check(lib.dp_fast_expand_batch(self._ctx, ptr(parents), len(parents), ptr(kids), ptr(acc)))
        return kids, acc

    def fast_expand_device(self, d_parents: int, n: int, d_children: int, d_accept: int | None,
                           stream: int | None = None):
        self._check(lib.dp_fast_expand_batch_device(self._ctx, ctypes.c_void_p(d_parents), n,
                                                    ctypes.c_void_p(d_children),
                                                    ctypes.c_void_p(d_accept) if d_accept else None,
                                                    ctypes.c_void_p(stream) if stream else None))

    def fast_last_stats(self) -> dict:
        st = N.DpFastStats()
        self._check(lib.dp_fast_last_stats(self._ctx, ctypes.byref(st)))
        return {name: getattr(st, name) for name, _ in N.DpFastStats._fields_}

    def evaluate(self, patches: np.ndarray, cell: int) -> np.ndarray:
        out = np.zeros(len(patches), dtype=np.float32)
        self._check(lib.dp_eval_batch(self._ctx, ptr(patches), len(patches), cell, ptr(out)))
        return out

    def optimize(self, patches: np.ndarray, cell: int) -> np.ndarray:
        return self.refine(patches, cell, N.MODE_NM)

    def filter(self, patches: np.ndarray, cell: int) -> np.ndarray:
        return self.refine(patches, cell, N.MODE_FILTER)

    def densify(self, seeds_xyz: np.ndarray, copy: bool = True):
        seeds = np.ascontiguousarray(seeds_xyz, dtype=np.float64).reshape(-1, 3)
        out = ctypes.c_void_p()
        n = ctypes.c_int64()
        st = N.DpDensifyStats()
        self._check(lib.dp_densify(self._ctx, ptr(seeds), len(seeds), ctypes.byref(out), ctypes.byref(n),
                                   ctypes.byref(st)))
        stats = {name: getattr(st, name) for name, _ in N.DpDensifyStats._fields_}
        return result_array(out.value, n.value, copy), stats

    def densify_begin(self, seeds_xyz: np.ndarray) -> N.DpGeneration:
        seeds = np.ascontiguousarray(seeds_xyz, dtype=np.float64).reshape(-1, 3)
        g = N.DpGeneration()
        self._check(lib.dp_densify_begin(self._ctx, ptr(seeds), len(seeds), ctypes.byref(g)))
        return g

    def densify_commit(self, gen: N.DpGeneration, cand: np.ndarray, acc: np.ndarray) -> N.DpGeneration:
        cand = np.ascontiguousarray(cand, dtype=PATCH_DTYPE)
        acc = np.ascontiguousarray(acc, dtype=np.uint8)
        self._check(lib.dp_densify_commit(self._ctx, ctypes.byref(gen), ptr(cand), ptr(acc), len(cand)))
        return gen

    def densify_run(self, gen: N.DpGeneration, max_generations: int = 1 << 30) -> N.DpGeneration:
        self._check(lib.dp_densify_run(self._ctx, ctypes.byref(gen), int(min(max_generations, 2**31 - 1))))
        return gen

    def densify_run_until(self, gen: N.DpGeneration, yield_items: int, max_generations: int = 1 << 30):
        ev = ctypes.c_int64()
        self._check(lib.dp_densify_run_until(self._ctx, ctypes.byref(gen), int(min(max_generations, 2**31 - 1)),
                                             int(yield_items), ctypes.byref(ev)))
        return gen, int(ev.value)

    def densify_owners(self, gen: N.DpGeneration, world: int, tile_px: int = 64):
        own = np.zeros(gen.items, dtype=np.int32)
        fb = ctypes.c_int32()
        self._check(lib.dp_densify_owners(self._ctx, ctypes.byref(gen), world, tile_px, ptr(own), ctypes.byref(fb)))
        return own, bool(fb.value)

    def densify_partition_stats(self) -> dict:
        st = np.zeros(4, dtype=np.int64)
        self._check(lib.dp_densify_partition_stats(self._ctx, ptr(st)))
        return {"items": int(st[0]), "world": int(st[1]), "tiles": int(st[2]), "split_items": int(st[3])}

    def densify_refine_items(self, gen: N.DpGeneration, items: np.ndarray):
        items = np.ascontiguousarray(items, dtype=np.int64)
        n = len(items) * gen.per_item
        cand = empty_patches(n)
        acc = np.zeros(n, dtype=np.uint8)
        self._check(lib.dp_densify_refine_items(self._ctx, ctypes.byref(gen), ptr(items), len(items), ptr(cand),
                                                ptr(acc)))
        return cand, acc

    def densify_partition_async(self, gen: N.DpGeneration, world: int, tile_px: int = 64,
                                stream: int | None = None):
        d_order = ctypes.c_void_p()
        counts = np.zeros(world, dtype=np.int64)
        self._check(lib.dp_densify_partition_async(self._ctx, ctypes.byref(gen), world, tile_px,
                                                   ctypes.c_void_p(stream) if stream else None,
                                                   ctypes.byref(d_order), ptr(counts)))
        return int(d_order.value or 0), counts

    def densify_refine_share_async(self, gen: N.DpGeneration, d_items: int, n: int, d_slot: int, stride: int,
                                   stream: int | None = None) -> None:
        self._check(lib.dp_densify_refine_share_async(self._ctx, ctypes.byref(gen), ctypes.c_void_p(d_items), n,
                                                      ctypes.c_void_p(d_slot), stride,
                                                      ctypes.c_void_p(stream) if stream else None))

    def densify_commit_gathered_device(self, gen: N.DpGeneration, d_recs: int, stride: int, world: int,
                                       stream: int | None = None) -> int:
        ex = ctypes.c_int64()
        self._check(lib.dp_densify_commit_gathered_device(self._ctx, ctypes.byref(gen), ctypes.c_void_p(d_recs), stride,
                                                          world, ctypes.c_void_p(stream) if stream else None,
                                                          ctypes.byref(ex)))
        return int(ex.value)

    def densify_result(self, copy: bool = True):
        out = ctypes.c_void_p()
        n = ctypes.c_int64()
        st = N.DpDensifyStats()
        self._check(lib.dp_densify_result(self._ctx, ctypes.byref(out), ctypes.byref(n), ctypes.byref(st)))
        stats = {name: getattr(st, name) for name, _ in N.DpDensifyStats._fields_}
        return result_array(out.value, n.value, copy), stats


    def densify_resume(self, patches: np.ndarray, keep: np.ndarray | None = None) -> N.DpGeneration:
        patches = np.ascontiguousarray(patches)
        assert patches.dtype == PATCH_DTYPE
        if keep is not None:
            keep = np.ascontiguousarray(keep, dtype=np.uint8)
# ... 1083 lines not shown
```

### include/densepoints.h

```cpp
#ifndef DENSEPOINTS_H
#define DENSEPOINTS_H

#include <stddef.h>
#include <stdint.h>

#ifdef __cplusplus
extern "C" {
#endif

#define DP_ABI_VERSION 2

#define DP_OK 0
#define DP_E_ARG (-1)
#define DP_E_HIP (-2)
#define DP_E_OOM (-3)
#define DP_E_DEGENERATE (-4)
#define DP_E_STATE (-5)
#define DP_E_NODEVICE (-6)

#define DP_MAX_VIEWS 128
#define DP_MAX_CELL 16
#define DP_MAX_LEVELS 8

typedef struct dp_options {
// ... 331 lines not shown
} dp_mesh_normals_stats;

void dp_default_mesh_smooth_options(dp_mesh_smooth_options *mso);
int dp_mesh_adjacency(dp_ctx *ctx, const int32_t *triangles, int64_t n_triangles, int64_t n_vertices,
                      const int32_t **offsets, const int32_t **neighbours, const int32_t **edge_triangles,
                      const uint8_t **vertex_flags, int64_t *n_entries, dp_mesh_adjacency_stats *stats);
int dp_mesh_adjacency_device(dp_ctx *ctx, const int32_t *d_triangles, int64_t n_triangles, int64_t n_vertices,
                             int32_t *d_offsets, int32_t *d_neighbours, int32_t *d_edge_triangles, int64_t entry_cap,
                             uint8_t *d_vertex_flags, int64_t *n_entries, dp_mesh_adjacency_stats *stats, void *stream);
int dp_mesh_smooth(dp_ctx *ctx, const dp_mesh_smooth_options *mso, const dp_mesh_vertex *vertices, int64_t n_vertices,
                   const int32_t *triangles, int64_t n_triangles, const dp_mesh_vertex **vertices_out,
                   dp_mesh_smooth_stats *stats);
int dp_mesh_smooth_device(dp_ctx *ctx, const dp_mesh_smooth_options *mso, const dp_mesh_vertex *d_vertices,
                          int64_t n_vertices, const int32_t *d_triangles, int64_t n_triangles,
                          dp_mesh_vertex *d_vertices_out, dp_mesh_smooth_stats *stats, void *stream);
int dp_mesh_normals(dp_ctx *ctx, const dp_mesh_vertex *vertices, int64_t n_vertices, const int32_t *triangles,
                    int64_t n_triangles, const float **normals, dp_mesh_normals_stats *stats);
int dp_mesh_normals_device(dp_ctx *ctx, const dp_mesh_vertex *d_vertices, int64_t n_vertices, const int32_t *d_triangles,
                           int64_t n_triangles, float *d_normals, dp_mesh_normals_stats *stats, void *stream);

#define DP_DECIMATE_MEAN 0
#define DP_DECIMATE_QUADRIC 1
#define DP_DECIMATE_DET_EPS 1e-6
typedef struct dp_mesh_decimate_options {
    float origin[3];
    float cell;
    int32_t mode;
    int32_t flags;
    int32_t reserved;
} dp_mesh_decimate_options;
typedef struct dp_mesh_decimate_stats {
    int64_t vertices_in, triangles_in, invalid_triangles, degenerate_triangles, unused_vertices,
        clamped_vertices, clusters, orphan_clusters, max_cluster, collapsed_triangles, duplicate_triangles,
        quadric_vertices, mean_vertices, vertices_out, triangles_out;
    double decimate_ms;
} dp_mesh_decimate_stats;

void dp_default_mesh_decimate_options(dp_mesh_decimate_options *mdo);
int dp_mesh_decimate(dp_ctx *ctx, const dp_mesh_decimate_options *opts, const dp_mesh_vertex *vertices,
                     int64_t n_vertices, const int32_t *triangles, int64_t n_triangles,
                     const dp_mesh_vertex **vertices_out, int64_t *n_vertices_out, const int32_t **triangles_out,
                     int64_t *n_triangles_out, int32_t *vertex_map, int32_t *triangle_map,
                     dp_mesh_decimate_stats *stats);
int dp_mesh_decimate_device(dp_ctx *ctx, const dp_mesh_decimate_options *opts, const dp_mesh_vertex *d_vertices,
                            int64_t n_vertices, const int32_t *d_triangles, int64_t n_triangles,
                            dp_mesh_vertex *d_vertices_out, int64_t vertex_cap, int64_t *n_vertices_out,
                            int32_t *d_triangles_out, int64_t triangle_cap, int64_t *n_triangles_out,
                            int32_t *d_vertex_map, int32_t *d_triangle_map, dp_mesh_decimate_stats *stats,
                            void *stream);

#define DP_MESH_RENDER_CULL_BACK 1
typedef struct dp_mesh_render_options {
    int32_t flags;
} dp_mesh_render_options;
typedef struct dp_mesh_render_stats {
    int64_t triangles, invalid_triangles, pairs, clipped_pairs, culled_pairs, pixel_tests, covered_pixels;
    double render_ms;
} dp_mesh_render_stats;

void dp_default_mesh_render_options(dp_mesh_render_options *mro);
int dp_mesh_render(dp_ctx *ctx, const dp_mesh_vertex *vertices, int64_t n_vertices, const int32_t *triangles,
                   int64_t n_triangles, const int32_t *views, int n_views, const dp_mesh_render_options *mro,
                   float *const *depth, int32_t *const *index, float *const *normal, dp_mesh_render_stats *stats);
int dp_mesh_render_device(dp_ctx *ctx, const dp_mesh_vertex *d_vertices, int64_t n_vertices,
                          const int32_t *d_triangles, int64_t n_triangles, const int32_t *views, int n_views,
                          const dp_mesh_render_options *mro, float *const *d_depth, int32_t *const *d_index,
                          float *const *d_normal, dp_mesh_render_stats *stats, void *stream);

typedef struct dp_matcher_options {
    int32_t n_features;
    int32_t n_levels;
    double scale_factor;
    int32_t edge_threshold;
    int32_t fast_threshold;
    int32_t cell_size;
    int32_t max_keypoints_per_cell;
    int32_t epipolar_matching;
    float max_epipolar_distance;
    float nn_match_ratio;
    int32_t matcher_type;
    int32_t detector_type;
    float akaze_threshold;
} dp_matcher_options;
#define DP_DETECTOR_AKAZE 0
#define DP_DETECTOR_ORB 1
#define DP_MATCHER_KNN 0
#define DP_MATCHER_FLANN 1

typedef struct dp_keypoint {
    float x, y;
    float response;
    float angle;
    int32_t octave;
    int32_t reserved;
} dp_keypoint;

typedef struct dp_seed_stats {
    int64_t keypoints_detected;
    int64_t keypoints;
    int64_t pairs;
    int64_t ratio_matches;
    int64_t matches;
    int64_t points;
    double detect_ms, describe_ms, match_ms, triangulate_ms, total_ms;
} dp_seed_stats;

void dp_default_matcher_options(dp_matcher_options *mo);
int dp_orb_pattern(int8_t *xy_out);
int dp_generate_seeds(dp_ctx *ctx, const dp_matcher_options *mo, const double **xyz_out, int64_t *n_out,
                      dp_seed_stats *stats);
int dp_seed_keypoints(dp_ctx *ctx, int view, const dp_keypoint **kp, const uint8_t **desc32, int64_t *n);
int dp_seed_descriptor_bytes(dp_ctx *ctx);
int dp_seed_matches(dp_ctx *ctx, int pair, int32_t *first, int32_t *second, const int32_t **query_to_train,
                    int64_t *nq);

int dp_knn_match(dp_ctx *ctx, const uint8_t *query, int64_t nq, const uint8_t *train, int64_t nt,
                 int32_t *idx2, int32_t *dist2);
int dp_knn_match_wide(dp_ctx *ctx, const uint8_t *query, int64_t nq, const uint8_t *train, int64_t nt,
                      int descriptor_bytes, int32_t *idx2, int32_t *dist2);
int dp_fundamental_matrix(const double P1[12], const double P2[12], double F[9]);
int dp_triangulate(dp_ctx *ctx, int64_t n_points, const int32_t *offsets, const double *P, const double *obs,
                   double *X);

typedef struct dp_fast_options {
    int32_t iters;
    int32_t margin;
    int32_t tile_budget;
    int32_t max_views;
    float fd_step;
    float ls_step;
    int32_t densify;
    int32_t gradient;
    int32_t filter_max_views;
} dp_fast_options;

void dp_default_fast_options(dp_fast_options *fo);
int dp_set_fast_options(dp_ctx *ctx, const dp_fast_options *fo);
int dp_build_gray(dp_ctx *ctx);
int dp_read_gray(dp_ctx *ctx, int view, uint16_t *fp16_out);
int dp_fast_expand_batch(dp_ctx *ctx, const dp_patch *parents, int n, dp_patch *children, uint8_t *accept_out);
typedef struct dp_fast_stats {
    int64_t patches;
    int64_t evals;
    int64_t view_evals;
    int64_t staged_bytes;
    int64_t clipped_stagings;
} dp_fast_stats;
int dp_fast_last_stats(dp_ctx *ctx, dp_fast_stats *out);
int dp_fast_expand_batch_device(dp_ctx *ctx, const dp_patch *d_parents, int n, dp_patch *d_children,
                                uint8_t *d_accept, void *stream);

int dp_last_kernel_ms(dp_ctx *ctx, double *ms);

typedef struct dp_synth_config {
    int32_t n_views;
    int32_t width, height;
    int32_t kind;
    uint64_t seed;
    double spread_deg;
    double seed_stride_px;
    double depth_noise;
} dp_synth_config;

void dp_synth_default(dp_synth_config *cfg);
int dp_synth_cameras(const dp_synth_config *cfg, double *P_out);
int dp_synth_render_host(const dp_synth_config *cfg, const double *P, int v, uint8_t *bgr_out);
int dp_synth_render_device(dp_ctx *ctx, const dp_synth_config *cfg, const double *P, int v,
                           void *d_bgra, void *stream);
int64_t dp_synth_seeds(const dp_synth_config *cfg, const double *P, double *xyz_out, int64_t cap);
int dp_synth_surface(const dp_synth_config *cfg, int64_t n, const double *xy, double *z_out, double *normal_out);

#ifdef __cplusplus
}
#endif
#endif
```

Baseline: 4.088 Mpatches/s.

## Specialise refine kernel for cell 11 with narrow addressing and uniform pitch

Adds compile-time specialisation of the refine kernel for an 11-pixel cell, narrow addressing and a pitch shared by all views. The pitch and second-row image base are read as kernel arguments (scalar registers) instead of being fetched from LDS per slot and checked with ballots, and the cell size becomes a constant for loop unrolling. The aim is fewer VGPRs, fewer branches and less per-pass overhead in the texel sampling paths. The cost is extra kernel instantiations and a larger binary, and the specialised path only applies when every view has the same pitch.

```diff
diff --git a/densepoints_amd/_native.py b/densepoints_amd/_native.py
--- a/densepoints_amd/_native.py
+++ b/densepoints_amd/_native.py
@@ -35,6 +35,7 @@
 DP_E_NODEVICE = -6
 
 MODE_EVAL, MODE_FILTER, MODE_NM, MODE_SEED, MODE_EXPAND = range(5)
+REFINE_GENERIC, REFINE_SPECIALISED = 0, 1
 MODE_FAST_EVAL, MODE_FAST_REFINE = 5, 6
 PATCH_ACCEPTED = 1
 PATCH_DEGENERATE = 2
@@ -499,6 +500,7 @@
     ("dp_mesh_render", _I, [_P, _P, ctypes.c_int64, _P, ctypes.c_int64, _P, _I, _P, _P, _P, _P, _P]),
     ("dp_mesh_render_device", _I, [_P, _P, ctypes.c_int64, _P, ctypes.c_int64, _P, _I, _P, _P, _P, _P, _P, _P]),
     ("dp_last_kernel_ms", _I, [_P, _P]),
+    ("dp_last_refine_instance", _I, [_P, _P]),
     ("dp_default_matcher_options", None, [_P]),
     ("dp_orb_pattern", _I, [_P]),
     ("dp_generate_seeds", _I, [_P, _P, _P, _P, _P]),
diff --git a/densepoints_amd/csrc/dp_capi.hip b/densepoints_amd/csrc/dp_capi.hip
--- a/densepoints_amd/csrc/dp_capi.hip
+++ b/densepoints_amd/csrc/dp_capi.hip
@@ -149,6 +149,8 @@
     {
         const char *e = getenv("DP_NO_LPT");
         c->lpt_off = e && e[0] == '1';
+        const char *ns = getenv("DP_NO_REFINE_SPEC");
+        c->spec_off = ns && ns[0] == '1';
         const char *g = getenv("DP_GEN_CAP");
         c->gen_cap_test = g ? std::atoll(g) : 0;
     }
@@ -257,6 +259,10 @@
     c->img_base = (const char *)lo;
     for (auto &v : c->hv)
         v.img_off = c->narrow ? (uint32_t)((uintptr_t)v.img - lo) : 0u;
+    c->uni_pitch = c->hv.empty() ? 0 : c->hv[0].pitch;
+    for (auto &v : c->hv)
+        if (v.pitch != c->uni_pitch)
+            c->uni_pitch = 0;
     DP_HIP(c, hipMalloc(&c->d_views, sizeof(dpg::ViewDev) * c->V));
     DP_HIP(c, hipMemcpy(c->d_views, c->hv.data(), sizeof(dpg::ViewDev) * c->V, hipMemcpyHostToDevice));
     return DP_OK;
@@ -609,6 +615,8 @@
     a.grid_scale = (double)c->opt.grid_scale;
     a.img_base = c->img_base;
     a.narrow = c->narrow ? 1 : 0;
+    a.pitch = (c->narrow && !c->spec_off) ? c->uni_pitch : 0;
+    a.img_base1 = c->img_base + 4 * (int64_t)a.pitch;
     if (!c->lpt_off && n > 0) {
         if (c->lpt.reserve((size_t)n + 2 * dpk::kLptBuckets) == hipSuccess) {
             a.order = c->lpt.p;
@@ -632,7 +640,7 @@
     const dpk::RefineArgs a = refine_args(c, job);
     if (!job.parity_untimed)
         DP_HIP(c, hipEventRecord(c->e0, s));
-    DP_HIP(c, dpk::launch_refine(a, s));
+    DP_HIP(c, dpk::launch_refine(a, s, &c->refine_instance));
     if (!job.parity_untimed) {
         DP_HIP(c, hipEventRecord(c->e1, s));
         c->timed = true;
@@ -768,6 +776,14 @@
     return DP_OK;
 }
 
+extern "C" int dp_last_refine_instance(const dp_ctx *c, int *instance)
+{
+    if (!c || !instance)
+        return DP_E_ARG;
+    *instance = c->refine_instance;
+    return DP_OK;
+}
+
 extern "C" int dp_last_kernel_ms(dp_ctx *c, double *ms)
 {
     if (!c || !ms)
diff --git a/densepoints_amd/csrc/dp_ctx.h b/densepoints_amd/csrc/dp_ctx.h
--- a/densepoints_amd/csrc/dp_ctx.h
+++ b/densepoints_amd/csrc/dp_ctx.h
@@ -169,6 +169,9 @@
     std::vector<uint32_t *> pyr_pool;
     int level = 0;
     bool narrow = false;
+    int32_t uni_pitch = 0;
+    bool spec_off = false;
+    int refine_instance = -1;
     DevBuf<uint32_t> d_work;
     DevBuf<unsigned long long> d_evals;
     Event e0, e1;
diff --git a/densepoints_amd/csrc/dp_internal.h b/densepoints_amd/csrc/dp_internal.h
--- a/densepoints_amd/csrc/dp_internal.h
+++ b/densepoints_amd/csrc/dp_internal.h
@@ -94,6 +94,8 @@
     int64_t max_pops;
     const char *img_base;
     int32_t narrow;
+    int32_t pitch;
+    const char *img_base1;
     uint32_t *order;
     uint32_t *order_scratch;
     const int64_t *items;
@@ -347,7 +349,9 @@
 hipError_t launch_mesh_vertices(const MeshArgs &a, hipStream_t s);
 hipError_t launch_mesh_triangles(const MeshArgs &a, hipStream_t s);
 
-hipError_t launch_refine(const RefineArgs &a, hipStream_t s);
+constexpr int kSpecCell = 11;
+constexpr int kRefineGeneric = 0, kRefineSpecialised = 1;
+hipError_t launch_refine(const RefineArgs &a, hipStream_t s, int *instance = nullptr);
 hipError_t launch_pyr_down(const PyrPlane *d_src, const PyrPlane *d_dst, int V, int max_dw, int max_dh,
                            hipStream_t s);
 int read_stamps(unsigned long long *out);
diff --git a/densepoints_amd/csrc/dp_refine.hip b/densepoints_amd/csrc/dp_refine.hip
--- a/densepoints_amd/csrc/dp_refine.hip
+++ b/densepoints_amd/csrc/dp_refine.hip
@@ -12,6 +12,16 @@
 #define DP_MAP_CHUNK 24
 #endif
 constexpr int kMapChunk = DP_MAP_CHUNK;
+
+template <int kCell = 0, bool kNarrow = false, bool kUniPitch = false>
+struct Spec {
+    static_assert(!kUniPitch || kNarrow, "the second row base exists in narrow addressing only");
+    static constexpr int cell = kCell;
+    static constexpr bool narrow = kNarrow, uni_pitch = kUniPitch;
+    static __device__ __forceinline__ int cell_of(const RefineArgs &a) { return kCell ? kCell : a.cell; }
+    static __device__ __forceinline__ bool narrow_of(const RefineArgs &a) { return kNarrow || a.narrow != 0; }
+    static __device__ __forceinline__ int pitch_of() { return DP_KARG(RefineArgs, int32_t, pitch); }
+};
 
 struct WaveLds {
     double rowt[64][3];
@@ -117,14 +127,17 @@
 
 typedef const __attribute__((address_space(1))) char *gbyte_t;
 
-template <bool kUniPitch>
+template <bool kUniPitch, bool kScalarPitch = false>
 __device__ __forceinline__ TexelLoad texel_fetch_n(gbyte_t base, gbyte_t base1, uint32_t roi, int pitch4, int wm32,
                                                    int hm32, int32_t ix, int32_t iy)
 {
     const int32_t cx = med3_i32(ix, 0, wm32), cy = med3_i32(iy, 0, hm32);
     uint32_t xo, o0;
     asm("v_lshl_add_u32 %0, %1, 2, %2" : "=v"(xo) : "v"((uint32_t)cx >> 5), "v"(roi));
-    asm("v_mad_u32_u24 %0, %1, %2, %3" : "=v"(o0) : "v"((uint32_t)cy >> 5), "v"(pitch4), "v"(xo));
+    if (kScalarPitch)
+        asm("v_mad_u32_u24 %0, %1, %2, %3" : "=v"(o0) : "v"((uint32_t)cy >> 5), "s"(pitch4), "v"(xo));
+    else
+        asm("v_mad_u32_u24 %0, %1, %2, %3" : "=v"(o0) : "v"((uint32_t)cy >> 5), "v"(pitch4), "v"(xo));
     TexelLoad t;
     t.a = *(gpair_t)(base + o0);
     if (kUniPitch)
@@ -134,6 +147,16 @@
     t.fx = (uint32_t)cx & 31u;
     t.fy = (uint32_t)cy & 31u;
     return t;
+}
+
+template <class S>
+__device__ __forceinline__ gbyte_t lower_row_base(const RefineArgs &a, int upitch)
+{
+    typedef const char *cbytes_t;
+    if constexpr (S::uni_pitch)
+        return (gbyte_t)DP_KARG(RefineArgs, cbytes_t, img_base1);
+    else
+        return (gbyte_t)a.img_base + (uint32_t)(upitch * 4);
 }
 
 __device__ __forceinline__ uint32_t pk_mul_u16_sat(uint32_t a, uint32_t b)
@@ -342,20 +365,21 @@
     iy = rint_i32((R[1] + C[1]) * W);
 }
 
-template <int G, bool kAnchor, bool kNarrow, bool kUniPitch>
+template <int G, bool kAnchor, bool kNarrow, bool kUniPitch, class S>
 __device__ __forceinline__ void group_sample_safe(const RefineArgs &a, WaveLds &L, const TexDescT<G> &td, int j,
                                                   uint64_t roi, int pitch, int upitch, int wm32, int hm32, int &s,
                                                   int &ss, int &sx)
 {
     typedef unsigned short us2 __attribute__((ext_vector_type(2)));
     TexelLoad tl[kTexPerLane];
-    const gbyte_t base1 = (gbyte_t)a.img_base + (uint32_t)(upitch * 4);
+    const gbyte_t base1 = lower_row_base<S>(a, upitch);
 #pragma unroll
     for (int i = 0; i < kTexPerLane; ++i) {
         int32_t ix, iy;
         texel_coord_d(td.row(i), td.col(i), ix, iy);
         if (kNarrow)
-            tl[i] = texel_fetch_n<kUniPitch>((gbyte_t)a.img_base, base1, (uint32_t)roi, pitch * 4, wm32, hm32, ix, iy);
+            tl[i] = texel_fetch_n<kUniPitch, S::uni_pitch>((gbyte_t)a.img_base, base1, (uint32_t)roi, pitch * 4, wm32,
+                                                           hm32, ix, iy);
         else
             tl[i] = texel_fetch((gpix_t)roi, pitch, wm32, hm32, ix, iy);
         __builtin_amdgcn_sched_barrier(0);
@@ -388,6 +412,7 @@
     sx = (int)usx;
 }
 
+template <class S>
 __device__ __forceinline__ void group_sample_split(const RefineArgs &a, const TexDescT<2> &td, int j, uint64_t roi,
                                                    int pitch, int upitch, int wm32, int hm32, int &s, int &ss, int &sx)
 {
@@ -398,13 +423,15 @@
     const uint32_t rc0 = hi ? td.rc[2] : td.rc[0], rc1 = hi ? td.rc[3] : td.rc[1];
     const uint32_t ra0 = rc0 & 0xffffu, ca0 = rc0 >> 16, ra1 = rc1 & 0xffffu, ca1 = rc1 >> 16;
     const uint32_t sel = hi ? td.sel[1] : td.sel[0];
-    const gbyte_t base1 = (gbyte_t)a.img_base + (uint32_t)(upitch * 4);
+    const gbyte_t base1 = lower_row_base<S>(a, upitch);
     int32_t ix, iy;
     texel_coord_d(ra0, ca0, ix, iy);
-    const TexelLoad t0 = texel_fetch_n<true>((gbyte_t)a.img_base, base1, (uint32_t)roi, pitch * 4, wm32, hm32, ix, iy);
+    const TexelLoad t0 = texel_fetch_n<true, S::uni_pitch>((gbyte_t)a.img_base, base1, (uint32_t)roi, pitch * 4, wm32,
+                                                           hm32, ix, iy);
     __builtin_amdgcn_sched_barrier(0);
     texel_coord_d(ra1, ca1, ix, iy);
-    const TexelLoad t1 = texel_fetch_n<true>((gbyte_t)a.img_base, base1, (uint32_t)roi, pitch * 4, wm32, hm32, ix, iy);
+    const TexelLoad t1 = texel_fetch_n<true, S::uni_pitch>((gbyte_t)a.img_base, base1, (uint32_t)roi, pitch * 4, wm32,
+                                                           hm32, ix, iy);
     __builtin_amdgcn_sched_barrier(0);
     const uint32_t gg = __builtin_amdgcn_perm(texel_gray_hi(t1), texel_gray_hi(t0), sel);
     const uint32_t aa = *(lds_u32_t)(uintptr_t)(td.anc + 4u * (uint32_t)LP * (uint32_t)j);
@@ -463,12 +490,12 @@
     usx = __builtin_amdgcn_udot2(vg, __builtin_bit_cast(us2, aa), usx, false);
 }
 
-template <bool kAnchor, bool kUniPitch>
+template <bool kAnchor, bool kUniPitch, class S>
 __device__ __forceinline__ void group_sample_wide(const RefineArgs &a, const TexDescT<2> &td, int j, uint32_t roi,
                                                   int pitch, int upitch, int wm32, int hm32, int &s, int &ss, int &sx)
 {
     static_assert(kTexPerLane == 4, "two texel pairs per batch");
-    const gbyte_t base1 = (gbyte_t)a.img_base + (uint32_t)(upitch * 4);
+    const gbyte_t base1 = lower_row_base<S>(a, upitch);
     const int lane = lane_id();
     const bool odd = (lane & kWideLP) != 0;
     const uint32_t anc1 = odd ? td.anc - 4u * kWideLP : td.anc + 4u * kWideLP;
@@ -481,7 +508,7 @@
         for (int i = 0; i < kTexPerLane; ++i) {
             int32_t ix, iy;
             texel_coord_d(td.row(kTexPerLane * b + i), td.col(kTexPerLane * b + i), ix, iy);
-            tl[i] = texel_fetch_n<kUniPitch>((gbyte_t)a.img_base, base1, roi, pitch * 4, wm32, hm32, ix, iy);
+            tl[i] = texel_fetch_n<kUniPitch, S::uni_pitch>((gbyte_t)a.img_base, base1, roi, pitch * 4, wm32, hm32, ix, iy);
             __builtin_amdgcn_sched_barrier(0);
         }
 #pragma unroll
@@ -515,13 +542,13 @@
     sx = (int)usx;
 }
 
-template <bool kAnchor>
+template <bool kAnchor, class S>
 __device__ __forceinline__ void views_pass_wide(const RefineArgs &a, WaveLds &L, const TexDescT<2> &td, uint64_t q,
                                                 int &sa, int &saa)
 {
     constexpr int LP = kWideLP;
     const int lane = lane_id();
-    const int cell = a.cell;
+    const int cell = S::cell_of(a);
     const int j = (int)((uint32_t)lane / (uint32_t)LP);
     const int slot = pick8(j, q);
     {
@@ -531,17 +558,23 @@
     }
     const int wm32 = (L.map[slot].w - 1) * 32, hm32 = (L.map[slot].h - 1) * 32;
     const bool all_safe = __ballot(L.map[slot].safe == 0) == 0ull;
-    const int pitch = L.pitch[slot];
-    const int upitch = uni(pitch);
-    const bool uni_pitch = __ballot(pitch != upitch) == 0ull;
+    int pitch, upitch;
+    bool uni_pitch = true;
+    if constexpr (S::uni_pitch) {
+        pitch = upitch = S::pitch_of();
+    } else {
+        pitch = L.pitch[slot];
+        upitch = uni(pitch);
+        uni_pitch = __ballot(pitch != upitch) == 0ull;
+    }
     const uint32_t roi = (uint32_t)L.roi[slot];
     wave_sync();
     int s = 0, ss = 0, sx = 0;
     if (all_safe) {
-        if (uni_pitch)
-            group_sample_wide<kAnchor, true>(a, td, j, roi, pitch, upitch, wm32, hm32, s, ss, sx);
-        else
-            group_sample_wide<kAnchor, false>(a, td, j, roi, pitch, upitch, wm32, hm32, s, ss, sx);
+        if (S::uni_pitch || uni_pitch)
+            group_sample_wide<kAnchor, true, S>(a, td, j, roi, pitch, upitch, wm32, hm32, s, ss, sx);
+        else if constexpr (!S::uni_pitch)
+            group_sample_wide<kAnchor, false, S>(a, td, j, roi, pitch, upitch, wm32, hm32, s, ss, sx);
     } else {
         const Moments mm = group_sample_clamped<kWave / LP, kAnchor, true>(L, cell, j, true, (gpix_t)(a.img_base + roi),
                                                                          pitch, wm32, hm32);
@@ -562,13 +595,13 @@
     wave_sync();
 }
 
-template <int G, bool kAnchor, bool kSplit = false>
+template <int G, bool kAnchor, bool kSplit, class S>
 __device__ __forceinline__ void views_pass(const RefineArgs &a, WaveLds &L, const TexDescT<G> &td, int base, uint64_t q, int &sa, int &saa)
 {
     static_assert(!kSplit || (G == 2 && !kAnchor), "split passes: G = 2, no anchor");
     constexpr int LP = kWave / G;
     const int lane = lane_id();
-    const int cell = a.cell;
+    const int cell = S::cell_of(a);
     static_assert(LP >= kTexPerLane, "cell <= LP");
     const int j = (int)((uint32_t)lane / (uint32_t)LP);
     const int slot = pick8(j, q);
@@ -583,32 +616,42 @@
     const int wm32 = (L.map[sl].w - 1) * 32, hm32 = (L.map[sl].h - 1) * 32;
     const int safe = L.map[sl].safe;
     const bool all_safe = (__ballot(safe == 0) & __ballot(act)) == 0ull;
-    const int pitch = L.pitch[sl];
-    const int upitch = uni(pitch);
-    const bool uni_pitch = __ballot(pitch != upitch) == 0ull;
+    int pitch, upitch;
+    bool uni_pitch = true;
+    if constexpr (S::uni_pitch) {
+        pitch = upitch = S::pitch_of();
+    } else {
+        pitch = L.pitch[sl];
+        upitch = uni(pitch);
+        uni_pitch = __ballot(pitch != upitch) == 0ull;
+    }
     const uint64_t roi = L.roi[sl];
     wave_sync();
     int s = 0, ss = 0, sx = 0;
     if constexpr (kSplit) {
         if (all_safe) {
-            group_sample_split(a, td, j, roi, pitch, upitch, wm32, hm32, s, ss, sx);
+            group_sample_split<S>(a, td, j, roi, pitch, upitch, wm32, hm32, s, ss, sx);
         } else {
             const gpix_t roip = (gpix_t)(a.img_base + (uint32_t)roi);
-            const Moments mm = group_sample_clamped<G, false>(L, a.cell, j, act && j == 0, roip, pitch, wm32, hm32);
+            const Moments mm = group_sample_clamped<G, false>(L, S::cell_of(a), j, act && j == 0, roip, pitch, wm32, hm32);
             s = mm.s;
             ss = mm.ss;
             sx = mm.sx;
         }
     } else if (all_safe) {
-        if (a.narrow && uni_pitch)
-            group_sample_safe<G, kAnchor, true, true>(a, L, td, j, roi, pitch, upitch, wm32, hm32, s, ss, sx);
-        else if (a.narrow)
-            group_sample_safe<G, kAnchor, true, false>(a, L, td, j, roi, pitch, upitch, wm32, hm32, s, ss, sx);
-        else
-            group_sample_safe<G, kAnchor, false, false>(a, L, td, j, roi, pitch, upitch, wm32, hm32, s, ss, sx);
+        if constexpr (S::uni_pitch) {
+            group_sample_safe<G, kAnchor, true, true, S>(a, L, td, j, roi, pitch, upitch, wm32, hm32, s, ss, sx);
+        } else {
+            if (a.narrow && uni_pitch)
+                group_sample_safe<G, kAnchor, true, true, S>(a, L, td, j, roi, pitch, upitch, wm32, hm32, s, ss, sx);
+            else if (a.narrow)
+                group_sample_safe<G, kAnchor, true, false, S>(a, L, td, j, roi, pitch, upitch, wm32, hm32, s, ss, sx);
+            else
+                group_sample_safe<G, kAnchor, false, false, S>(a, L, td, j, roi, pitch, upitch, wm32, hm32, s, ss, sx);
+        }
     } else {
-        const gpix_t roip = a.narrow ? (gpix_t)(a.img_base + (uint32_t)roi) : (gpix_t)roi;
-        const Moments mm = group_sample_clamped<G, kAnchor>(L, a.cell, j, act, roip, pitch, wm32, hm32);
+        const gpix_t roip = S::narrow_of(a) ? (gpix_t)(a.img_base + (uint32_t)roi) : (gpix_t)roi;
+        const Moments mm = group_sample_clamped<G, kAnchor>(L, S::cell_of(a), j, act, roip, pitch, wm32, hm32);
         s = mm.s;
         ss = mm.ss;
         sx = mm.sx;
@@ -629,12 +672,12 @@
     wave_sync();
 }
 
-template <int G>
+template <int G, class S>
 __device__ __forceinline__ void views_all(const RefineArgs &a, WaveLds &L, const TexDescT<G> &td, int base, uint64_t todo, bool anchor, int &sa, int &saa)
 {
     bool first = anchor;
     if constexpr (G == 2) {
-        while (a.narrow && __popcll(todo) + (first ? 1 : 0) >= 4) {
+        while (S::narrow_of(a) && __popcll(todo) + (first ? 1 : 0) >= 4) {
             uint64_t q = 0;
 #pragma unroll
             for (int s = 0; s < 4; ++s) {
@@ -644,9 +687,9 @@
                 todo &= todo - 1;
             }
             if (first)
-                views_pass_wide<true>(a, L, td, q, sa, saa);
+                views_pass_wide<true, S>(a, L, td, q, sa, saa);
             else
-                views_pass_wide<false>(a, L, td, q, sa, saa);
+                views_pass_wide<false, S>(a, L, td, q, sa, saa);
             first = false;
         }
     }
@@ -667,15 +710,15 @@
         }
         bool split = false;
         if constexpr (G == 2) {
-            if (!first && (q >> 8 & 0xffull) == 0xffull && a.narrow) {
-                views_pass<2, false, true>(a, L, td, base, (q & ~0xff00ull) | ((q & 0xffull) << 8), sa, saa);
+            if (!first && (q >> 8 & 0xffull) == 0xffull && S::narrow_of(a)) {
+                views_pass<2, false, true, S>(a, L, td, base, (q & ~0xff00ull) | ((q & 0xffull) << 8), sa, saa);
                 split = true;
             }
         }
         if (first)
-            views_pass<G, true>(a, L, td, base, q, sa, saa);
+            views_pass<G, true, false, S>(a, L, td, base, q, sa, saa);
         else if (!split)
-            views_pass<G, false>(a, L, td, base, q, sa, saa);
+            views_pass<G, false, false, S>(a, L, td, base, q, sa, saa);
         first = false;
     }
 }
@@ -714,6 +757,7 @@
     return v;
 }
 
+template <class S>
 __device__ __forceinline__ uint64_t build_maps_quad(const MapView &vw, WaveLds &L, int base, int m, int round0,
                                                     int cell, bool narrow)
 {
@@ -753,9 +797,14 @@
             tm.m7 *= 0.03125;
             tm.m8 *= 0.03125;
             L.map[slot] = tm;
-            L.roi[slot] = narrow ? (uint64_t)(vw.img_off + ((uint32_t)tm.tly * (uint32_t)vw.pitch + (uint32_t)tm.tlx) * 4u)
-                                 : (uint64_t)(uintptr_t)(vw.img + ((size_t)tm.tly * (size_t)vw.pitch + (size_t)tm.tlx));
-            L.pitch[slot] = vw.pitch;
+            if constexpr (S::uni_pitch) {
+                L.roi[slot] = (uint64_t)(vw.img_off + ((uint32_t)tm.tly * (uint32_t)S::pitch_of() + (uint32_t)tm.tlx) * 4u);
+            } else {
+                L.roi[slot] = (S::narrow || narrow)
+                                  ? (uint64_t)(vw.img_off + ((uint32_t)tm.tly * (uint32_t)vw.pitch + (uint32_t)tm.tlx) * 4u)
+                                  : (uint64_t)(uintptr_t)(vw.img + ((size_t)tm.tly * (size_t)vw.pitch + (size_t)tm.tlx));
+                L.pitch[slot] = vw.pitch;
+            }
         }
     }
     const uint64_t okq = __ballot(ok);
@@ -765,6 +814,7 @@
     return bits << round0;
 }
 
+template <class S>
 __device__ __forceinline__ uint64_t build_maps_pair(const MapView &vw, WaveLds &L, int base, int m, int round0,
                                                     int cell, bool narrow)
 {
@@ -804,9 +854,14 @@
             tm.m7 *= 0.03125;
             tm.m8 *= 0.03125;
             L.map[slot] = tm;
-            L.roi[slot] = narrow ? (uint64_t)(vw.img_off + ((uint32_t)tm.tly * (uint32_t)vw.pitch + (uint32_t)tm.tlx) * 4u)
-                                 : (uint64_t)(uintptr_t)(vw.img + ((size_t)tm.tly * (size_t)vw.pitch + (size_t)tm.tlx));
-            L.pitch[slot] = vw.pitch;
+            if constexpr (S::uni_pitch) {
+                L.roi[slot] = (uint64_t)(vw.img_off + ((uint32_t)tm.tly * (uint32_t)S::pitch_of() + (uint32_t)tm.tlx) * 4u);
+            } else {
+                L.roi[slot] = (S::narrow || narrow)
+                                  ? (uint64_t)(vw.img_off + ((uint32_t)tm.tly * (uint32_t)vw.pitch + (uint32_t)tm.tlx) * 4u)
+                                  : (uint64_t)(uintptr_t)(vw.img + ((size_t)tm.tly * (size_t)vw.pitch + (size_t)tm.tlx));
+                L.pitch[slot] = vw.pitch;
+            }
         }
     }
     const uint64_t okq = __ballot(ok);
@@ -842,14 +897,14 @@
     return r;
 }
 
-template <int G>
+template <int G, class S>
 __device__ __forceinline__ int wave_scores(const RefineArgs &a, WaveLds &L, const TexDescT<G> &td, const double *nn, const double *pp, bool &degen)
 {
     const int lane = lane_id();
     STAMP_BEGIN;
     const int m = uni(L.m);
     const int nv = m - 1;
-    const int cell = a.cell;
+    const int cell = S::cell_of(a);
     const int N = cell * cell;
     {
         double c12[12];
@@ -880,9 +935,9 @@
         uint64_t okmask = 0;
         if (m - base > 16) {
             static_assert(kMapChunk <= 32, "a pair round covers the chunk");
-            okmask = build_maps_pair(load_map_view<1>(a, L, base, m, 0), L, base, m, 0, cell, a.narrow != 0);
+            okmask = build_maps_pair<S>(load_map_view<1>(a, L, base, m, 0), L, base, m, 0, cell, a.narrow != 0);
         } else {
-            okmask = build_maps_quad(load_map_view(a, L, base, m, 0), L, base, m, 0, cell, a.narrow != 0);
+            okmask = build_maps_quad<S>(load_map_view(a, L, base, m, 0), L, base, m, 0, cell, a.narrow != 0);
         }
         wave_sync();
         STAMP(L, 0);
@@ -894,7 +949,7 @@
         const uint64_t todo = valid & (((ke - base) >= 64 ? ~0ull : ((1ull << (ke - base)) - 1ull)) &
                                        ~((1ull << (kb - base)) - 1ull));
         const bool anc = base == 0 && va;
-        views_all<G>(a, L, td, base, todo, anc, Sa, Saa);
+        views_all<G, S>(a, L, td, base, todo, anc, Sa, Saa);
         STAMP(L, 1);
         wave_sync();
         STAMP(L, 2);
@@ -909,7 +964,7 @@
     return nv;
 }
 
-template <int G>
+template <int G, class S>
 __device__ __forceinline__ double wave_objective(const RefineArgs &a, WaveLds &L, const TexDescT<G> &td, double x0, double x1, double x2, bool &degen)
 {
     double nn[3], pp[3];
@@ -922,7 +977,7 @@
         const double sb = readlane_f64(s, 1), cb = readlane_f64(co, 1);
         dpg::unparametrize_sc(a.views[uni(L.ref)].C, Xs, ns, x0, sa, ca, sb, cb, nn, pp);
     }
-    const int nv = wave_scores<G>(a, L, td, nn, pp, degen);
+    const int nv = wave_scores<G, S>(a, L, td, nn, pp, degen);
     if (nv == 0)
         return 2.0;
     double sum = 0.0;
@@ -940,7 +995,7 @@
     return i == 0 ? yy[0] : (i == 1 ? yy[1] : (i == 2 ? yy[2] : yy[3]));
 }
 
-template <int G>
+template <int G, class S>
 __device__ __forceinline__ int wave_nelder_mead(const RefineArgs &a, WaveLds &L, const TexDescT<G> &td, bool &degen)
 {
     const double step[3] = {DP_KARG(RefineArgs, double, opt.nm_step[0]), DP_KARG(RefineArgs, double, opt.nm_step[1]),
@@ -972,7 +1027,7 @@
             L.pt[1] = q1;
             L.pt[2] = q2;
         }
-        const double f = nm_uni(wave_objective<G>(a, L, td, q0, q1, q2, degen));
+        const double f = nm_uni(wave_objective<G, S>(a, L, td, q0, q1, q2, degen));
         ++evals;
         bool decide = false;
         if (phase == kInit) {
@@ -1094,7 +1149,7 @@
     return evals;
 }
 
-template <int G>
+template <int G, class S>
 __device__ __forceinline__ bool wave_filter(const RefineArgs &a, WaveLds &L, const TexDescT<G> &td, float &score, bool &degen)
 {
     const int lane = lane_id();
@@ -1102,7 +1157,7 @@
     {
         const double nn[3] = {L.n[0], L.n[1], L.n[2]};
         const double pp[3] = {L.X[0], L.X[1], L.X[2]};
-        nv = wave_scores<G>(a, L, td, nn, pp, degen);
+        nv = wave_scores<G, S>(a, L, td, nn, pp, degen);
     }
     if (nv == 0) {
         score = -1.0f;
@@ -1180,9 +1235,11 @@
 #define DP_REFINE_BOUNDS __launch_bounds__(kBlock) __attribute__((amdgpu_waves_per_eu(DP_REFINE_WAVES_PER_EU)))
 #endif
 
-template <int kMode, int G, bool kGen = false>
+template <int kMode, int G, bool kGen = false, int kCell = 0, bool kNarrow = false, bool kUniPitch = false>
 __global__ DP_REFINE_BOUNDS void refine_kernel(RefineArgs a)
 {
+    using S = Spec<kCell, kNarrow, kUniPitch>;
+    static_assert(kCell == 0 || pass_width(kCell) == G, "a compiled-in window runs at its own pass width");
     const int n = kGen ? (int)a.gen->ncand : a.n;
     const int64_t parent0 = kGen ? a.gen->head : a.parent0;
     if (kGen && (int64_t)blockIdx.x * kWavesPerBlock >= (int64_t)n)
@@ -1195,7 +1252,7 @@
     for (int c = 0; c < 8; ++c)
         L.stamp[c] = 0;
 #endif
-    const TexDescT<G> td = make_texdesc<G>(L, a.cell);
+    const TexDescT<G> td = make_texdesc<G>(L, S::cell_of(a));
     const uint32_t gs = a.parents ? 4u : 1u;
     const int npos = a.order ? (int)(((uint32_t)n + gs - 1) / gs * gs) : n;
     for (;;) {
@@ -1269,7 +1326,7 @@
             case DP_MODE_EVAL: {
                 const double nn[3] = {L.n[0], L.n[1], L.n[2]};
                 const double pp[3] = {L.X[0], L.X[1], L.X[2]};
-                const int nv = wave_scores<G>(a, L, td, nn, pp, degen);
+                const int nv = wave_scores<G, S>(a, L, td, nn, pp, degen);
                 double sum = 0.0;
                 for (int k = 0; k < nv; ++k)
                     sum = sum + L.score[k];
@@ -1280,26 +1337,26 @@
                 break;
             }
             case DP_MODE_FILTER:
-                ok = wave_filter<G>(a, L, td, score, degen);
+                ok = wave_filter<G, S>(a, L, td, score, degen);
                 has_score = true;
                 evals = 1;
                 break;
             case DP_MODE_NM:
-                evals = wave_nelder_mead<G>(a, L, td, degen);
+                evals = wave_nelder_mead<G, S>(a, L, td, degen);
                 ok = true;
                 break;
             case DP_MODE_SEED:
-                ok = wave_filter<G>(a, L, td, score, degen);
+                ok = wave_filter<G, S>(a, L, td, score, degen);
                 has_score = true;
                 evals = 1;
                 if (ok)
-                    evals += wave_nelder_mead<G>(a, L, td, degen);
+                    evals += wave_nelder_mead<G, S>(a, L, td, degen);
                 break;
             case DP_MODE_EXPAND:
             default:
-                evals = wave_nelder_mead<G>(a, L, td, degen);
+                evals = wave_nelder_mead<G, S>(a, L, td, degen);
                 wave_init_related(a, L);
-                ok = wave_filter<G>(a, L, td, score, degen);
+                ok = wave_filter<G, S>(a, L, td, score, degen);
                 has_score = true;
                 evals += 1;
                 break;
@@ -1452,7 +1509,7 @@
     }
 }
 
-hipError_t launch_refine(const RefineArgs &a, hipStream_t s)
+hipError_t launch_refine(const RefineArgs &a, hipStream_t s, int *instance)
 {
     const bool gen = a.gen != nullptr;
     if (!gen && a.n <= 0)
@@ -1472,6 +1529,11 @@
     const int g = pass_width(a.cell);
     if (g <= 0)
         return hipErrorInvalidValue;
+    constexpr int kSpecG = pass_width(kSpecCell);
+    const bool spec = a.cell == kSpecCell && a.narrow && a.pitch > 0 &&
+                      (a.mode == DP_MODE_EXPAND || a.mode == DP_MODE_NM);
+    if (instance)
+        *instance = spec ? kRefineSpecialised : kRefineGeneric;
     if (a.order) {
         const int ng = a.parents ? (a.n + 3) / 4 : a.n;
         if (!gen && (e = hipMemsetAsync(a.order_scratch, 0, 2 * kLptBuckets * sizeof(uint32_t), s)) != hipSuccess)
@@ -1480,6 +1542,11 @@
         hipLaunchKernelGGL(lpt_hist_kernel, dim3(gb), dim3(256), 0, s, a, ng);
         hipLaunchKernelGGL(lpt_scan_kernel, dim3(1), dim3(64), 0, s, a);
         hipLaunchKernelGGL(lpt_scatter_kernel, dim3(gb), dim3(256), 0, s, a, ng);
+    }
+    if (gen && spec) {
+        hipLaunchKernelGGL((refine_kernel<DP_MODE_EXPAND, kSpecG, true, kSpecCell, true, true>), dim3(grid), dim3(kBlock), 0,
+                           s, a);
+        return hipGetLastError();
     }
     if (gen) {
         switch (g) {
@@ -1495,6 +1562,15 @@
         default:
             return hipErrorInvalidValue;
         }
+        return hipGetLastError();
+    }
+    if (spec) {
+        if (a.mode == DP_MODE_EXPAND)
+            hipLaunchKernelGGL((refine_kernel<DP_MODE_EXPAND, kSpecG, false, kSpecCell, true, true>), dim3(grid),
+                               dim3(kBlock), 0, s, a);
+        else
+            hipLaunchKernelGGL((refine_kernel<DP_MODE_NM, kSpecG, false, kSpecCell, true, true>), dim3(grid), dim3(kBlock),
+                               0, s, a);
         return hipGetLastError();
     }
     switch (a.mode * 16 + g) {
diff --git a/densepoints_amd/pmvs.py b/densepoints_amd/pmvs.py
--- a/densepoints_amd/pmvs.py
+++ b/densepoints_amd/pmvs.py
@@ -289,6 +289,11 @@
         ms = ctypes.c_double()
         self._check(lib.dp_last_kernel_ms(self._ctx, ctypes.byref(ms)))
         return ms.value
+
+    def last_refine_instance(self) -> int:
+        inst = ctypes.c_int()
+        self._check(lib.dp_last_refine_instance(self._ctx, ctypes.byref(inst)))
+        return inst.value
 
     def set_fast_options(self, fo: FastOptions):
         c = fo.to_c()
diff --git a/include/densepoints.h b/include/densepoints.h
--- a/include/densepoints.h
+++ b/include/densepoints.h
@@ -507,6 +507,10 @@
 
 int dp_last_kernel_ms(dp_ctx *ctx, double *ms);
 
+#define DP_REFINE_GENERIC 0
+#define DP_REFINE_SPECIALISED 1
+int dp_last_refine_instance(const dp_ctx *ctx, int *instance);
+
 typedef struct dp_synth_config {
     int32_t n_views;
     int32_t width, height;
```

Result: no change. 4.125 Mpatches/s (median of 6 runs) (+0.9%).
